# SebastianBitsch/SRGAN-ST

Measured on AMD Instinct MI355X. Metric: HR images/sec (96px x4, B=16/GPU) G+D+ST-loss step, higher is better.
Workload: dtype f32; 1 GPU; srgan_x4_hr96_b16_G+D+ST-loss step: adv+mse+st, D updated every step (train.py:116-164; BASELINE metric); global_batch=16, hr=96, lr=24, parallelism=dp1, hip_graph=True, d_update_interval=1, d_sr_forward=run: all three discriminator forwards of train.py:136,155,158

## Files before the change

### include/srganst.h

```cpp
#ifndef SRGANST_H
#define SRGANST_H
#include <stdint.h>
#ifdef __cplusplus
extern "C" {
#endif

const char* sst_last_error(void);
int sst_version(void);
const char* sst_arch(void);
int sst_clear_error(void);
int sst_reload_env(void);

int sst_st_loss_workspace(int B, int H, int W, int64_t* partial_floats);
int sst_st_loss_fwd(const float* sr, const float* gt, float* loss, float* gS, float* partials,
                    unsigned* counter, int B, int H, int W, float sigma, float rho, int normalize,
                    void* stream);
int sst_st_loss_bwd(const float* sr, const float* gS, float* dsr, const float* scale_dev,
                    float scale_host, int accumulate, int B, int H, int W, float sigma, float rho,
                    void* stream);
int sst_st_maps_workspace(int B, int H, int W, int64_t* tile_floats);
int sst_st_maps(const float* x, const float* gt, float* Sx, float* Sgt, float* Fx, float* Fgt, float* d, float* tile_sums,
                int B, int H, int W, float sigma, float rho, int normalize, void* stream);
int sst_st_pixel_loss_fwd(const float* sr, const float* gt, float* loss, float* gS, float* partials, unsigned* counter,
                          float* pix_loss, float* pix_partials, int pix_mode, int B, int H, int W, float sigma, float rho,
                          int normalize, void* stream);
int sst_st_pixel_loss_bwd(const float* sr, const float* gt, const float* gS, float* dsr, const float* scale_dev, float scale_host,
                          float pix_weight, int pix_mode, int accumulate, int B, int H, int W, float sigma, float rho,
                          void* stream);

int64_t sst_conv_packed_floats(int Cout, int Cin, int ksize);
int sst_conv_pack(const float* w, float* wp, int Cout, int Cin, int ksize, int mode, void* stream);
int sst_conv_pack_multi(const void* jobs, int njobs, int total_blocks, void* stream);
int sst_conv_mtiles(int B, int Ho, int Wo);
int sst_conv_stat_tiles(int B, int H, int W, int Cin, int Cout, int ksize, int stride);
const char* sst_conv_kernel_name(int B, int H, int W, int Cin, int Cout, int ksize, int stride, int out_mode, int fused_in);
const char* sst_conv_wgrad_kernel_name(int B, int H, int W, int Cin, int Cout, int ksize, int stride, int njobs);
long sst_debug_big_tile_launches(void);
long sst_debug_band_launches(void);
long sst_debug_wgrad_band_launches(void);
int sst_debug_mfma_peak(float* out, int blocks, int iters, void* stream);
int sst_debug_bf16x3(const float* A, const float* B, float* C32, float* C3, int K, int mode, int blocks, void* stream);
int sst_debug_stamp(unsigned long long* out, int slot, void* stream);
int sst_conv_fwd(const float* x, const float* wp, float* y, float* y_pre, const float* bias,
                 const float* in_scale, const float* in_shift, const float* in_slope,
                 float in_slope_const, int in_act, const float* residual, float* stats,
                 float* stats_cnt, int out_mode, int B, int H, int W, int Cin, int Cout, int ksize,
                 int stride, void* stream);
int sst_conv_pipe_supported(int B, int H, int W, int Cin, int Cout, int ksize, int stride);
int sst_conv_pipe_stat_tiles(int B, int H, int W, int Cin, int Cout, int ksize, int stride);
int64_t sst_conv_pipe_ws_floats(int B, int H, int W, int Cin, int Cout, int ksize, int stride);
int sst_conv_pipe_groups_ok(int B, int H, int W, int Cin, int Cout, int ksize, int stride, int grp_images);
int sst_conv_pipe_fwd_grp(const float* x, const float* wp, float* y, const float* bias, const float* in_scale,
                          const float* in_shift, const float* in_slope, float in_slope_const, int in_act, float* stats,
                          float* stats_cnt, const float* epi_y, const float* epi_scale, const float* epi_shift,
                          const float* epi_slope, float epi_slope_const, int epi_act, float* epi_partial, float* ws, int B,
                          int H, int W, int Cin, int Cout, int ksize, int stride, int grp_images, void* stream);
int sst_conv_ns_supported(int B, int H, int W, int Cin, int Cout, int ksize, int stride, int out_mode);
int sst_conv_ns_fwd(const float* x, const float* wp, float* y, const float* bias, const float* in_scale,
                    const float* in_shift, const float* in_slope, float in_slope_const, int in_act, float* stats,
                    float* stats_cnt, const float* epi_y, const float* epi_scale, const float* epi_shift,
                    const float* epi_slope, float epi_slope_const, int epi_act, float* epi_partial, int B, int H, int W,
                    int Cin, int Cout, int ksize, int stride, int out_mode, int grp_images, void* stream);
int sst_conv_s2_dgrad_pipe_supported(int B, int H, int W, int Cin, int Cout);
int64_t sst_conv_s2_dgrad_pipe_ws_floats(int B, int H, int W, int Cin, int Cout);
int sst_conv_s2_dgrad_pipe_stat_tiles(int B, int H, int W, int Cin, int Cout);
int sst_conv_s2_dgrad_pipe_groups_ok(int B, int H, int W, int Cin, int Cout, int grp_images);
int sst_conv_s2_dgrad_pipe_bwdstats_grp(const float* dy, const float* wp, float* dx, float* ws, const float* epi_y,
                                    const float* epi_scale, const float* epi_shift, const float* epi_slope,
                                    float epi_slope_const, int epi_act, float* epi_partial, int B, int H, int W, int Cin,
                                    int Cout, int grp_images, void* stream);
int sst_conv_dgrad_bwdstats(const float* x, const float* wp, float* y, const float* residual, const float* epi_y,
                            const float* epi_scale, const float* epi_shift, const float* epi_slope,
                            float epi_slope_const, int epi_act, float* epi_partial, int B, int H, int W, int Cin,
                            int Cout, int ksize, void* stream);
int sst_conv_acc_supported(int B, int H, int W, int Cin, int Cout, int ksize, int stride);
int sst_conv_fwd_acc(const float* x, const float* in2, float* side_out, const float* ones, const float* wp, float* y,
                     const float* bias, const float* in_slope, float in_slope_const, int in_act, const double* in_acc,
                     const float* in_gamma, const float* in_beta, float in_n, float eps, float momentum, float* o_mean,
                     float* o_rstd, float* o_scale, float* o_shift, float* run_mean, float* run_var, double* st_acc,
                     int nrep, int B, int H, int W, int Cin, int Cout, int ksize, void* stream);
int sst_conv_dgrad_fused_acc(const float* g, const float* y2, const float* in_scale, const float* in_shift,
                             const float* in_slope, float in_slope_const, int in_act, float* dy_out, const float* wp,
                             float* out, const float* residual, const float* epi_y, const float* epi_scale,
                             const float* epi_shift, const float* epi_slope, float epi_slope_const, int epi_act,
                             const double* bw_in_acc, const float* mean, const float* rstd, const float* gamma, float n,
                             float* dgamma, float* dbeta, float* dslope, double* bw_st_acc, int nrep, int B, int H,
                             int W, int Cin, int Cout, int ksize, void* stream);
int sst_bn_finalize_acc(const double* acc, int nrep, int C, float n, const float* gamma, const float* beta,
                        float* run_mean, float* run_var, float* mean, float* rstd, float* scale, float* shift,
                        float eps, float momentum, void* stream);
int sst_conv_fwd_resin(const float* x, const float* y2, const float* ones, const float* bn_scale, const float* bn_shift,
                       float* h_out, const float* wp, float* y, const float* bias, float* stats, float* stats_cnt,
                       int B, int H, int W, int Cin, int Cout, int ksize, void* stream);
int sst_conv_dgrad_fused(const float* g, const float* y2, const float* cA, const float* cB, const float* cC,
                         const float* in_scale, const float* in_shift, const float* in_slope, float in_slope_const,
                         int in_act, float* dy_out, const float* wp, float* out, const float* residual,
                         const float* epi_y, const float* epi_scale, const float* epi_shift, const float* epi_slope,
                         float epi_slope_const, int epi_act, float* epi_partial, int B, int H, int W, int Cin, int Cout,
                         int ksize, void* stream);
int sst_conv_wgrad_chunks2(int B, int H, int W, int Cin, int Cout, int ksize, int stride, int njobs);
int sst_conv_wgrad_groups_ok(int B, int H, int W, int Cin, int Cout, int ksize, int stride, int grp_images);
int sst_conv_wgrad_grp(const float* x, const float* dy, float* slab, float* dw, const float* in_scale,
                   const float* in_shift, const float* in_slope, float in_slope_const, int in_act,
                   int B, int H, int W, int Cin, int Cout, int stride, int ksize, int accumulate,
                       int grp_images, void* stream);
int sst_conv_wgrad_pending_reduce(int B, int H, int W, int Cin, int Cout, int ksize, int stride, int has_in_scale, int in_act);
int sst_wgrad_reduce_multi(const void* jobs, int njobs, void* stream);
int sst_wgrad_c3_supported(int C, int ksize);
int64_t sst_wgrad_c3_slab_floats(int B, int H, int W, int C);
int sst_wgrad_c3(const float* big, const float* small, float* slab, float* dw, const float* in_slope,
                 float in_slope_const, int in_act, int kind, int B, int H, int W, int C, int accumulate,
                 void* stream);

int64_t sst_conv9_c3_packed_floats(int Cout_eff);
int sst_conv9_c3_pack(const float* w, float* wp, int Cout, int Cin, int mode, void* stream);
int sst_conv9_c3_fwd(const float* x, const float* wp, float* y, const float* bias, int B, int H, int W,
                     int Cout, void* stream);
int64_t sst_conv9_to3_packed_floats(int C);
int sst_conv9_to3_pack(const float* w, float* wp, int C, void* stream);
int sst_conv9_to3_fwd(const float* x, const float* wp, float* y, float* y_pre, const float* bias,
                      const float* in_slope, float in_slope_const, int in_act, int B, int H, int W, int C,
                      void* stream);

int64_t sst_conv_s2_dgrad_packed_floats(int Cout, int Cin);
int sst_conv_s2_dgrad_pack(const float* w, float* wp, int Cout, int Cin, void* stream);
int sst_conv_s2_dgrad(const float* dy, const float* wp, float* dx, int B, int H, int W, int Cin, int Cout,
                      void* stream);
int sst_conv_s2_dgrad_tiles(int B, int H, int W);
const char* sst_conv_s2_dgrad_kernel_name(int B, int H, int W, int Cin, int Cout, int fused);
int sst_conv_s2_dgrad_fused(const float* g, const float* y2, const float* cA, const float* cB, const float* cC,
                            const float* in_scale, const float* in_shift, const float* in_slope, float in_slope_const,
                            int in_act, float* dy_out, const float* wp, float* dx, const float* epi_y,
                            const float* epi_scale, const float* epi_shift, const float* epi_slope, float epi_slope_const,
                            int epi_act, float* epi_partial, int B, int H, int W, int Cin, int Cout, void* stream);

int sst_conv_wgrad_grouped(const void* jobs, int njobs, int B, int H, int W, int Cin, int Cout, int stride,
                           int ksize, int accumulate, void* stream);

int sst_bn_finalize_grp(const float* stats, const float* cnt, int ntiles, int C, int groups, const float* gamma,
                        const float* beta, float* run_mean, float* run_var, float* mean, float* rstd, float* scale,
                        float* shift, float eps, float momentum, void* stream);
int sst_bn_eval_affine(const float* gamma, const float* beta, const float* run_mean,
                       const float* run_var, float* scale, float* shift, int C, float eps, void* stream);
int sst_bn_residual(const float* y, const float* scale, const float* shift, const float* res,
                    const float* res_slope, float* out, int64_t R, int C, void* stream);
int sst_bwd_reduce_blocks(int64_t R, int C);
int sst_bwd_finalize(const float* partial, int nblk, int C, float n, const float* mean,
                     const float* rstd, const float* gamma, float* dgamma, float* dbeta, float* cA,
                     float* cB, float* cC, float* dslope, int accumulate, void* stream);
int sst_bwd_reduce_grp(const float* g, const float* g2, const float* y, const float* scale, const float* shift,
                       const float* slope, float slope_const, int act, float* partial, int64_t R, int C, int groups,
                       void* stream);
int sst_bwd_finalize_grp(const float* partial, int nblk, int C, float n, int groups, const float* mean, const float* rstd,
                         const float* gamma, float* dgamma, float* dbeta, float* cA, float* cB, float* cC, int accumulate,
                         void* stream);
int sst_bwd_apply_grp(const float* g, const float* g2, const float* y, const float* scale, const float* shift,
                      const float* slope, float slope_const, int act, const float* cA, const float* cB, const float* cC,
                      float* dy, int64_t R, int C, int groups, void* stream);
int sst_bwd_finalize_wide(const float* partial, int nblk, int C, float n, const float* mean, const float* rstd,
                          const float* gamma, float* dgamma, float* dbeta, float* cA, float* cB, float* cC,
                          float* dslope, int accumulate, float* scratch, unsigned* counter, void* stream);
int sst_act_bwd_partial_blocks(int64_t stored_rows);
int sst_act_bwd_partial(const float* g, const float* g2, const float* y, const float* slope, float slope_const,
                        float* dy, float* partial, int64_t R, int C, int unshuffle_H, int unshuffle_W, void* stream);
int sst_bwd_apply(const float* g, const float* g2, const float* y, const float* scale,
                  const float* shift, const float* slope, float slope_const, int act, const float* cA,
                  const float* cB, const float* cC, float* dy, int64_t R, int C, int unshuffle_H,
                  int unshuffle_W, void* stream);
int sst_add(const float* a, const float* b, float* out, int64_t n, void* stream);

int sst_transpose(const float* src, float* dst, int B, int C, int H, int W, int to_nchw, void* stream);
int sst_feat_loss_fwd(const float* x, const float* gt, const float* scale, const float* shift, float slope, int C,
                      float* loss, float* partials, unsigned* counter, int64_t n, int mode, void* stream);
int sst_feat_loss_bwd(const float* x, const float* gt, const float* scale, const float* shift, float slope, int C,
                      float* dx, const float* scale_dev, float scale_host, int accumulate, int64_t n, int mode,
                      void* stream);
int sst_transpose_affine(const float* src, float* dst, int B, int C, int H, int W, int to_nchw,
                         const float* scale, const float* shift, void* stream);
int sst_maxpool_relu_fwd(const float* y, float* out, int B, int H, int W, int C, void* stream);
int sst_maxpool_relu_bwd(const float* g, const float* y, float* dy, int B, int H, int W, int C, void* stream);
int sst_clamp_bwd_blocks(int B, int H, int W);
int sst_clamp_bwd(const float* g, const float* pre, float* out, float* partial, float* dbias,
                  int accumulate, int B, int C, int H, int W, void* stream);
int sst_pixel_loss_blocks(int64_t n);
int sst_pixel_loss_fwd(const float* x, const float* gt, float* loss, float* partials, unsigned* counter,
                       int64_t n, int mode, void* stream);
int sst_pixel_loss_bwd(const float* x, const float* gt, float* dx, const float* scale_dev,
                       float scale_host, int accumulate, int64_t n, int mode, void* stream);
int sst_bce_logits(const float* logits, float target, float* loss, float* dlogits,
                   const float* scale_dev, float scale_host, int n, void* stream);
int sst_bicubic(const float* x, float* y, const float* wy, const int* iy, const float* wx, const int* ix,
                int64_t planes, int H, int W, int oh, int ow, int Ty, int Tx, int round_grid, void* stream);
int sst_gather_batch(const uint8_t* src, int64_t N, const int* idx, int B, int H, int W, const float* lut, float* gt, float* lr,
                     const float* wy, const int* iy, const float* wx, const int* ix, int oh, int ow, int Ty, int Tx,
                     void* stream);
int sst_gather_crops(const uint8_t* arena, int64_t arena_bytes, const int64_t* table, int64_t N, const int* desc, int B, int S,
                     const float* lut, float* gt, float* lr, const float* wy, const int* iy, const float* wx, const int* ix,
                     int oh, int ow, int Ty, int Tx, int span, void* stream);
int sst_image_metrics_workspace(int B, int H, int W, int64_t* partial_doubles);
int sst_image_metrics(const float* sr, const float* hr, int B, int H, int W, double* out, uint8_t* sr_u8, uint8_t* hr_u8,
                      double* workspace, void* stream);
int sst_tile_gather(const uint8_t* src_u8, const float* src_f32, int64_t src_bytes, int H, int W, const int* desc, int B, int th,
                    int tw, int t, const float* lut, float* out, void* stream);
int sst_tile_scatter(const float* tiles, const int* rows, int B, int H, int W, int th, int tw, int scale, int t, float* canvas,
                     int accumulate, void* stream);
int sst_canvas_to_u8(const float* canvas, int H, int W, float scale, uint8_t* out, void* stream);
int sst_bb_blocks(int B, int H, int W);
int sst_bb_feature_dim(int mode);
int sst_bb_patches(const float* img, float* cand, float* cnrm, int B, int H, int W, int ncand_total, int cand_off,
                   int mode, const float* st_mats, void* stream);
int sst_bb_match_dist(const float* sr, const float* cand, const float* cnrm, int* ind, float* dsr, float* partials, int B,
                 int H, int W, int ncand, float alpha, float beta, int criterion_l2, int mode, const float* st_mats, int dist_l1,
                      void* stream);
int sst_bbg_patches(int H, int W, int k, int pad, int stride);
int sst_bbg_blocks(int B, int np);
int sst_bbg_unfold(const float* img, float* table, float* nrm, int B, int H, int W, int k, int pad, int stride, int nrows_total,
                   int row_off, void* stream);
int sst_bbg_match(const float* srf, const float* cand, const float* cnrm, int* ind, float* gfeat, float* partials, int B, int np,
                  int ncand, int D, float alpha, float beta, int criterion_l2, int dist_l1, void* stream);
int sst_bbg_fold(const float* gfeat, float* dsr, int B, int H, int W, int k, int pad, int stride, void* stream);
int sst_weighted_sum(const float* const* terms, const float* weights, int n, float* out, float* weighted,
                     void* stream);

int sst_linear_ksplit(int M, int N, int K);
int sst_linear_fwd(const float* x, const float* w, const float* bias, float* y, float* slab, int M, int N,
                   int K, void* stream);
int sst_linear_dgrad(const float* dy, const float* w, float* dx, int M, int N, int K, int nhwc_C,
                     int nhwc_HW, void* stream);
int sst_linear_wgrad(const float* dy, const float* x, float* dw, float* db, int M, int N, int K,
                     int accumulate, void* stream);
int sst_head_fwd(const float* h, const float* w, const float* b, float* y, int M, int N, int K, float slope,
                 void* stream);
int sst_head_bwd(const float* h, const float* w, const float* dy, float* dh, float* dw, float* db, int M,
                 int N, int K, float slope, int accumulate, void* stream);
int sst_flatten_act_grp(const float* y, const float* scale, const float* shift, float slope, int act,
                        float* flat, int B, int HW, int C, int grp_images, void* stream);

int sst_adam_flat(float* p, const float* g, float* m, float* v, int64_t n, const float* lr, float* steps,
                  int nsteps, double beta1, double beta2, double eps, double weight_decay, void* stream);

int sst_adam_flat_ema(float* p, const float* g, float* m, float* v, float* ema, int64_t n, const float* lr, float* steps,
                      int nsteps, double beta1, double beta2, double eps, double weight_decay, double ema_decay,
                      int ema_warmup, void* stream);

int sst_ema_flat(float* ema, const float* p, int64_t n, const float* steps, double ema_decay, int ema_warmup, void* stream);

#ifdef __cplusplus
}
#endif
#endif
```

### srgan-st_amd/csrc/conv_pipe.hip

```cpp
#include "conv_common.h"
#include <cstdlib>
#include <type_traits>
#include "conv_epilogue.h"

int sst_conv_band_rows(int B, int H, int W, int Cin, int Cout, int ksize, int stride);

namespace {

constexpr int PIPE_RING = 9;

struct PipeArgs {
  const float* x;
  const float* wp;
  float* y;
  const float* bias;
  const float* in_scale; const float* in_shift; const float* in_slope; float in_slope_const; int in_act;
  float* stats; float* stats_cnt;
  const float* epi_y; const float* epi_scale; const float* epi_shift; const float* epi_slope;
  float epi_slope_const; int epi_act; float* epi_partial;
  float* ws;
  int B, H, W, Cin, Cout, Ho, Wo;
  int R;
  int tiles_x, n_mt, nfc, total_tiles, ncb, ksplit, cb_per, units;
#ifdef SST_PIPE_ABLATE
  int dbg;
#endif
  int gB, grows;
};

template <int S, int TW, int MODE>
struct PipeGeom {
  static constexpr int TH = 32 / TW;
  static constexpr int NB = TW == 2 ? 3 : 1;
  static constexpr int KSPAN = MODE ? 2 : 3;
  static constexpr int PW = (TW - 1) * S + KSPAN;
  static constexpr int PR = (TH - 1) * S + KSPAN + NB;
  static constexpr int NP = PW * PR;
  static constexpr int NU = (NP + 15) / 16;
  static constexpr int PS = 20;
  static constexpr int WAVE_FLOATS = NP * PS;
  static constexpr int NACC = MODE ? 4 : 1;
  static constexpr int NPAIR = MODE ? 2 : 1;
  static constexpr int SCRATCH = NPAIR * 4 * 32 * 33;
};
constexpr int S2D_CLS[9] = {0, 1, 1, 2, 2, 3, 3, 3, 3};
constexpr int S2D_TAP[9] = {0, 0, 1, 0, 1, 0, 1, 2, 3};

struct Stage {
  int b0, rem0, ix0, c0;
  int gin;
  const float* w;
};

#define PIPE_GLOAD(dst, voff, sbase) \
  asm volatile("s_nop 4\n\tglobal_load_dwordx4 %0, %1, %2" : "=v"(dst) : "v"(voff), "s"(sbase))
#define PIPE_WAIT(reg, n) asm volatile("s_waitcnt vmcnt(%1)" : "+v"(reg) : "n"(n))

__device__ __forceinline__ float half_sum(float t) {
  auto ror = [](float x, auto ctrl) {
    return __builtin_bit_cast(float, __builtin_amdgcn_update_dpp(0, __builtin_bit_cast(int, x), decltype(ctrl)::value, 0xf, 0xf, false));
  };
  t += ror(t, std::integral_constant<int, 0x128>{});
  t += ror(t, std::integral_constant<int, 0x124>{});
  t += ror(t, std::integral_constant<int, 0x122>{});
  t += ror(t, std::integral_constant<int, 0x121>{});
  t += __shfl_xor(t, 16, 64);
  return t;
}

template <int TW, int MODE = 0>
__device__ __forceinline__ void pipe_epilogue(const PipeArgs& a, float v[4], int r0, int ox0, int c0, int mt, int lane, bool first,
                                              int cls = 0) {
  constexpr int TH = 32 / TW;
  const int px = lane & 31;
  const int r = r0 + px / TW, ox = ox0 + px % TW;
  const bool pix_ok = r < a.R && ox < a.Wo;
  size_t obase;
  if (MODE) {
    obase = ((size_t)(2 * r + (cls >> 1)) * (2 * a.Wo) + 2 * ox + (cls & 1)) * a.Cout + c0;
    if (pix_ok) *reinterpret_cast<f32x4*>(a.y + obase) = f32x4{v[0], v[1], v[2], v[3]};
  }
  if (!MODE && a.bias) {
    const f32x4 bv = *reinterpret_cast<const f32x4*>(a.bias + c0);
#pragma unroll
    for (int j = 0; j < 4; ++j) v[j] += bv[j];
  }
  if (!MODE) {
    obase = ((size_t)r * a.Wo + ox) * a.Cout + c0;
    if (pix_ok) *reinterpret_cast<f32x4*>(a.y + obase) = f32x4{v[0], v[1], v[2], v[3]};
  }
  if (!MODE && a.stats) {
    const int nvalid = min(TH, a.R - r0) * min(TW, a.Wo - ox0);
    f32x4 s1, m2;
#pragma unroll
    for (int j = 0; j < 4; ++j) s1[j] = half_sum(pix_ok ? v[j] : 0.f);
#pragma unroll
    for (int j = 0; j < 4; ++j) {
      const float mean = s1[j] / (float)nvalid;
      const float d = pix_ok ? (v[j] - mean) : 0.f;
      m2[j] = half_sum(d * d);
    }
    if (px == 0) {
      float* st = a.stats + (size_t)mt * 2 * a.Cout;
      *reinterpret_cast<f32x4*>(st + c0) = s1;
      *reinterpret_cast<f32x4*>(st + a.Cout + c0) = m2;
      if (first) a.stats_cnt[mt] = (float)nvalid;
    }
  }
  if (a.epi_partial) {
    const float eslope = a.epi_slope ? a.epi_slope[0] : a.epi_slope_const;
    f32x4 yv = {0.f, 0.f, 0.f, 0.f}, es = {1.f, 1.f, 1.f, 1.f}, eh = {0.f, 0.f, 0.f, 0.f};
    if (pix_ok) yv = *reinterpret_cast<const f32x4*>(a.epi_y + obase);
    if (a.epi_scale) {
      const int ge = a.gB ? (r0 / a.grows) * a.Cout : 0;
      es = *reinterpret_cast<const f32x4*>(a.epi_scale + ge + c0);
      eh = *reinterpret_cast<const f32x4*>(a.epi_shift + ge + c0);
    }
    f32x4 q[3];
#pragma unroll
    for (int j = 0; j < 4; ++j) {
      const float g = pix_ok ? v[j] : 0.f;
      const float z = a.epi_scale ? fmaf(yv[j], es[j], eh[j]) : yv[j];
      float gz = g, q2 = 0.f;
      if (a.epi_act) {
        q2 = g * fminf(z, 0.f);
        gz = z > 0.f ? g : g * eslope;
      }
      q[0][j] = half_sum(gz);
      q[1][j] = half_sum(gz * yv[j]);
      q[2][j] = half_sum(q2);
    }
    if (px == 0) {
      const size_t prow = MODE ? (size_t)mt * 4 + cls : (size_t)mt;
#pragma unroll
      for (int k = 0; k < 3; ++k) *reinterpret_cast<f32x4*>(a.epi_partial + (prow * 3 + k) * a.Cout + c0) = q[k];
    }
  }
}

template <int S, int TW, int MODE, bool MS>
__global__ __launch_bounds__(CONV_NT, (S == 1 && MODE == 0 ? 3 : 2)) void conv_pipe_kernel(PipeArgs a) {
  using G = PipeGeom<S, TW, MODE>;
  constexpr int NACC = G::NACC, NPAIR = G::NPAIR;
  constexpr int PW = G::PW, NP = G::NP, NU = G::NU, NB = G::NB;
  constexpr int PS = G::PS;
  __shared__ __attribute__((aligned(16))) float patch[4 * G::WAVE_FLOATS];
  __shared__ __attribute__((aligned(16))) float scratch[G::SCRATCH];
  const int tid = threadIdx.x, wave = __builtin_amdgcn_readfirstlane(tid >> 6), lane = tid & 63;
  const int li = lane & 31, lh = lane >> 5;
  const int nwg = gridDim.x;
  const int HV = a.H + 1;
  const float slope = a.in_slope ? a.in_slope[0] : a.in_slope_const;
  const int c4 = wave * 16 + (lane & 3) * 4;
  const int p0 = lane >> 2;
  float* const lds = patch + wave * G::WAVE_FLOATS;

  int q = blockIdx.x;
  if (q >= a.units) return;
  int mt, nf, r0, ox0, oy0, cb, cb_end;
  Stage cur, nxt;
  auto decode = [&](int qq, int& mt_, int& nf_, int& ksi_, int& r0_, int& ox0_, int& b0_, int& oy0_) {
    mt_ = qq % a.n_mt;
    const int rest = qq / a.n_mt;
    nf_ = rest % a.nfc;
    ksi_ = rest / a.nfc;
    const int ty = mt_ / a.tiles_x, tx = mt_ - ty * a.tiles_x;
    r0_ = ty * G::TH;
    ox0_ = tx * TW;
    b0_ = r0_ / a.Ho;
    oy0_ = r0_ - b0_ * a.Ho;
  };
  auto make_stage = [&](int b0_, int oy0_, int ox0_, int nf_, int cb_) {
    Stage s;
    s.b0 = b0_;
    s.rem0 = oy0_ * S;
    s.ix0 = ox0_ * S - (MODE ? 0 : 1);
    s.c0 = cb_ * CB;
    s.gin = a.gB ? (b0_ / a.gB) * a.Cin : 0;
    s.w = a.wp + ((size_t)(nf_ * a.ncb + cb_) * 9 * 8) * 256 + wave * 512;
    return s;
  };
  int ksi, b0;
  decode(q, mt, nf, ksi, r0, ox0, b0, oy0);
  cb = ksi * a.cb_per;
  cb_end = cb + a.cb_per;
  cur = make_stage(b0, oy0, ox0, nf, cb);

  constexpr int NS = NU + 2;
  f32x4 sv[NU];
  unsigned okmask = 0;
  f32x4 ssc, ssh;
  const float* sc_base = a.in_scale ? a.in_scale : a.x;
  const float* sh_base = a.in_scale ? a.in_shift : a.x;
  unsigned boffs[MS ? NU : 1];
  auto stage_load = [&](const Stage& s, bool same_tile) {
#ifdef SST_PIPE_ABLATE
    if (a.dbg & 4) return;
#endif
    if (MS && same_tile) {
#pragma unroll
      for (int u = 0; u < NU; ++u) {
        boffs[u] += CB * 4u;
        PIPE_GLOAD(sv[u], boffs[u], a.x);
      }
    } else {
      okmask = 0;
#pragma unroll
      for (int u = 0; u < NU; ++u) {
        const int p = p0 + 16 * u;
        const int pr = p / PW, pc = p - pr * PW;
        int rr = s.rem0 + pr, b = s.b0;
#pragma unroll
        for (int k = 0; k <= NB; ++k) {
          const bool wrap = rr >= HV;
          rr -= wrap ? HV : 0;
          b += wrap ? 1 : 0;
        }
        const int iy = MODE ? rr : rr - 1, ix = s.ix0 + pc;
        const bool ok = p < NP && (MODE ? rr < a.H : rr >= 1) && b < a.B && (unsigned)ix < (unsigned)a.W;
        const int off = ((b * a.H + iy) * a.W + ix) * a.Cin + s.c0 + c4;
        const unsigned boff = (ok ? (unsigned)off : (unsigned)c4) * 4u;
        if (MS) boffs[u] = boff;
        PIPE_GLOAD(sv[u], boff, a.x);
        okmask |= ok ? (1u << u) : 0u;
      }
    }
    const unsigned coff = (unsigned)(a.in_scale ? s.gin + s.c0 + c4 : c4) * 4u;
    PIPE_GLOAD(ssc, coff, sc_base);
    PIPE_GLOAD(ssh, coff, sh_base);
  };
  auto stage_store = [&]() {
#ifdef SST_PIPE_ABLATE
    if (a.dbg & 1) return;
#endif
#pragma unroll
    for (int u = 0; u < NU; ++u) {
      const int p = p0 + 16 * u;
      if (p >= NP) continue;
      f32x4 t = sv[u];
      if (a.in_scale) {
#pragma unroll
        for (int j = 0; j < 4; ++j) t[j] = fmaf(t[j], ssc[j], ssh[j]);
      }
      if (a.in_act == ACT_SLOPE) {
#pragma unroll
        for (int j = 0; j < 4; ++j) t[j] = t[j] > 0.f ? t[j] : t[j] * slope;
      }
      if (!((okmask >> u) & 1u)) t = f32x4{0.f, 0.f, 0.f, 0.f};
      *reinterpret_cast<f32x4*>(&lds[p * PS + (lane & 3) * 4]) = t;
    }
  };

  auto lane_base = [&](int oy0_) {
    const int tr = li / TW, tc = li - tr * TW;
    int cross = 0;
#pragma unroll
    for (int k = 1; k <= NB; ++k) cross += (oy0_ + tr >= k * a.Ho) ? 1 : 0;
    return ((S * tr + cross) * PW + tc * S) * PS + 4 * lh;
  };
  int a_base = lane_base(oy0);

  f32x4 ring[PIPE_RING];
  const unsigned wlane = lane * 16u;
#define PIPE_WCHUNK(dst, w, i) PIPE_GLOAD(dst, wlane, (w) + (((i) >> 1) * 8 + ((i) & 1)) * 256)

#pragma unroll
  for (int i = 0; i < PIPE_RING; ++i) PIPE_WCHUNK(ring[i], cur.w, i);
  stage_load(cur, false);
  asm volatile("s_waitcnt vmcnt(0)" ::: "memory");
  __builtin_amdgcn_sched_barrier(0);
  stage_store();

  f32x16 acc[NACC];
#pragma unroll
  for (int k = 0; k < NACC; ++k)
#pragma unroll
    for (int r = 0; r < 16; ++r) acc[k][r] = 0.f;

  for (;;) {
    const bool unit_end = cb + 1 == cb_end;
    int n_q = q, n_mt = mt, n_nf = nf, n_r0 = r0, n_ox0 = ox0, n_oy0 = oy0, n_cb = cb + 1, n_cb_end = cb_end;
    bool more = true;
    if (unit_end) {
      n_q = q + nwg;
      more = n_q < a.units;
      if (more) {
        int n_ksi, n_b0;
        decode(n_q, n_mt, n_nf, n_ksi, n_r0, n_ox0, n_b0, n_oy0);
        n_cb = n_ksi * a.cb_per;
        n_cb_end = n_cb + a.cb_per;
        nxt = make_stage(n_b0, n_oy0, n_ox0, n_nf, n_cb);
      } else {
        nxt = cur;
      }
    } else {
      nxt = cur;
      nxt.c0 += CB;
      nxt.w += (size_t)9 * 8 * 256;
    }

    {
      const float* ab = lds + a_base;
      f32x4 av = *reinterpret_cast<const f32x4*>(ab);
      __builtin_amdgcn_sched_barrier(0);
#pragma unroll
      for (int i = 0; i < 18; ++i) {
        f32x4 an = av;
        if (i + 1 < 18) {
          const int t = (i + 1) >> 1;
          const int ntx = MODE ? 1 + (S2D_CLS[t] & 1) : 3, tt = MODE ? S2D_TAP[t] : t;
          an = *reinterpret_cast<const f32x4*>(ab + ((tt / ntx) * PW + (tt % ntx)) * PS + ((i + 1) & 1) * 8);
        }
        if (i == 0 || i >= 10) PIPE_WAIT(ring[i % PIPE_RING], 8); else PIPE_WAIT(ring[i % PIPE_RING], 8 + NS);
        const f32x4 bv = ring[i % PIPE_RING];
        constexpr int dummy_ = 0;
        (void)dummy_;
        const int ai = MODE ? S2D_CLS[i >> 1] : 0;
#ifdef SST_PIPE_ABLATE
        if (!(a.dbg & 16))
#endif
#pragma unroll
        for (int j = 0; j < 4; ++j) acc[ai] = __builtin_amdgcn_mfma_f32_32x32x2f32(av[j], bv[j], acc[ai], 0, 0, 0);
#ifdef SST_PIPE_ABLATE
        if (a.dbg & 8) { PIPE_GLOAD(ring[i % PIPE_RING], wlane, a.wp); } else
#endif
        if (i + PIPE_RING < 18) PIPE_WCHUNK(ring[i % PIPE_RING], cur.w, i + PIPE_RING);
        else PIPE_WCHUNK(ring[i % PIPE_RING], nxt.w, i + PIPE_RING - 18);
        if (i == 0) stage_load(nxt, !unit_end);
        av = an;
        __builtin_amdgcn_sched_barrier(0);
      }
    }
#ifdef SST_PIPE_ABLATE
    if (unit_end && (a.dbg & 2)) {
      if (acc[0][0] == 12345.f) a.y[0] = acc[0][0];
      if (!more) return;
      a_base = lane_base(n_oy0);
    } else
#endif
    if (unit_end) {
      const int cl = 8 * wave + 4 * lh;
#pragma unroll
      for (int k0 = 0; k0 < NACC; k0 += NPAIR) {
        __syncthreads();
#pragma unroll
        for (int k = 0; k < NPAIR; ++k)
#pragma unroll
          for (int r = 0; r < 16; ++r) {
            const int row = (r & 3) + 8 * (r >> 2) + 4 * lh;
            scratch[((k * 4 + wave) * 32 + row) * 33 + li] = acc[k0 + k][r];
            acc[k0 + k][r] = 0.f;
          }
        __syncthreads();
#pragma unroll
        for (int k = 0; k < NPAIR; ++k) {
          float v[4];
#pragma unroll
          for (int j = 0; j < 4; ++j) {
            float t = scratch[((k * 4 + 0) * 32 + li) * 33 + cl + j];
            t += scratch[((k * 4 + 1) * 32 + li) * 33 + cl + j];
            t += scratch[((k * 4 + 2) * 32 + li) * 33 + cl + j];
            t += scratch[((k * 4 + 3) * 32 + li) * 33 + cl + j];
            v[j] = t;
          }
          if (a.ksplit > 1) {
            const int tile = nf * a.n_mt + mt;
            const int part = cb / a.cb_per;
            *reinterpret_cast<f32x4*>(a.ws + (((size_t)part * a.total_tiles + tile) * NACC + k0 + k) * 1024 + li * 32 + cl) =
                f32x4{v[0], v[1], v[2], v[3]};
          } else {
            pipe_epilogue<TW, MODE>(a, v, r0, ox0, nf * 32 + cl, mt, lane, nf == 0 && wave == 0, k0 + k);
          }
        }
      }
      if (!more) return;
      a_base = lane_base(n_oy0);
    }
    stage_store();
    q = n_q; mt = n_mt; nf = n_nf; r0 = n_r0; ox0 = n_ox0; oy0 = n_oy0; cb = n_cb; cb_end = n_cb_end;
    cur = nxt;
  }
}

template <int TW, int MODE>
__global__ __launch_bounds__(CONV_NT) void pipe_reduce_kernel(PipeArgs a) {
  constexpr int NACC = MODE ? 4 : 1;
  const int tid = threadIdx.x, wave = tid >> 6, lane = tid & 63;
  const int tile = blockIdx.x / NACC, cls = blockIdx.x - tile * NACC;
  const int nf = tile / a.n_mt, mt = tile - nf * a.n_mt;
  const int ty = mt / a.tiles_x, tx = mt - ty * a.tiles_x;
  const int li = lane & 31, cl = 8 * wave + 4 * (lane >> 5);
  const size_t slab = (size_t)a.total_tiles * NACC * 1024;
  const float* src = a.ws + ((size_t)tile * NACC + cls) * 1024 + li * 32 + cl;
  f32x4 s = *reinterpret_cast<const f32x4*>(src);
  for (int k = 1; k < a.ksplit; ++k) {
    const f32x4 t = *reinterpret_cast<const f32x4*>(src + k * slab);
#pragma unroll
    for (int j = 0; j < 4; ++j) s[j] += t[j];
  }
  float v[4] = {s[0], s[1], s[2], s[3]};
  pipe_epilogue<TW, MODE>(a, v, ty * (32 / TW), tx * TW, nf * 32 + cl, mt, lane, nf == 0 && wave == 0, cls);
}

struct PipePlan {
  int tw;
  int ksplit, n_mt, tiles_x, nfc, ncb;
};

PipePlan pipe_plan(int B, int H, int W, int Cin, int Cout, int ksize, int stride) {
  PipePlan pl{};
  if (ksize != 3 || (stride != 1 && stride != 2) || (Cin % 64) || (Cout % 32) || B <= 0) return pl;
  if (stride == 2 && ((H | W) & 1)) return pl;
  if (Cout <= 64 && sst_conv_band_rows(B, H, W, Cin, Cout, ksize, stride)) return pl;
  const int Ho = (H - 1) / stride + 1, Wo = (W - 1) / stride + 1;
  int tw = 0;
  if (Wo % 8 == 0 && Ho >= 3) tw = 8;
  else if (Wo % 4 == 0 && Ho >= 7) tw = 4;
  else if (Wo % 2 == 0 && Ho >= 5) tw = 2;
  if (!tw) return pl;
  const int th = 32 / tw;
  pl.tiles_x = Wo / tw;
  pl.n_mt = pl.tiles_x * ((B * Ho + th - 1) / th);
  pl.nfc = Cout / 32;
  pl.ncb = Cin / 64;
  const long tiles = (long)pl.n_mt * pl.nfc;
  int maxks = 1;
  while (maxks < 4 && pl.ncb % (maxks * 2) == 0) maxks *= 2;
  if (tiles * maxks < 256) return pl;
  int ks = 1;
  while (tiles * ks < 1024 && ks < maxks) ks *= 2;
  pl.ksplit = ks;
  pl.tw = tw;
  return pl;
}

constexpr int PIPE_CUS = 256;

}

SST_API int sst_conv_pipe_supported(int B, int H, int W, int Cin, int Cout, int ksize, int stride) {
  return pipe_plan(B, H, W, Cin, Cout, ksize, stride).tw;
}
SST_API int sst_conv_pipe_stat_tiles(int B, int H, int W, int Cin, int Cout, int ksize, int stride) {
  return pipe_plan(B, H, W, Cin, Cout, ksize, stride).n_mt;
}
SST_API int64_t sst_conv_pipe_ws_floats(int B, int H, int W, int Cin, int Cout, int ksize, int stride) {
  const PipePlan pl = pipe_plan(B, H, W, Cin, Cout, ksize, stride);
  return (pl.tw && pl.ksplit > 1) ? (int64_t)pl.ksplit * pl.n_mt * pl.nfc * 1024 : 0;
}

SST_API int sst_conv_pipe_groups_ok(int B, int H, int W, int Cin, int Cout, int ksize, int stride, int grp_images) {
  const PipePlan pl = pipe_plan(B, H, W, Cin, Cout, ksize, stride);
  if (!pl.tw || grp_images <= 0 || B % grp_images) return 0;
  const int Ho = (H - 1) / stride + 1;
  return (grp_images * Ho) % (32 / pl.tw) == 0;
}

SST_API int sst_conv_pipe_fwd_grp(const float* x, const float* wp, float* y, const float* bias, const float* in_scale,
                                  const float* in_shift, const float* in_slope, float in_slope_const, int in_act, float* stats,
                                  float* stats_cnt, const float* epi_y, const float* epi_scale, const float* epi_shift,
                                  const float* epi_slope, float epi_slope_const, int epi_act, float* epi_partial, float* ws, int B,
                                  int H, int W, int Cin, int Cout, int ksize, int stride, int grp_images, void* stream) {
  SST_REQUIRE(x && wp && y, "sst_conv_pipe_fwd: null pointer");
  const PipePlan pl = pipe_plan(B, H, W, Cin, Cout, ksize, stride);
  SST_REQUIRE(grp_images == 0 || grp_images == B || sst_conv_pipe_groups_ok(B, H, W, Cin, Cout, ksize, stride, grp_images),
              "sst_conv_pipe_fwd: coefficient groups of %d images do not end on tile boundaries (B=%d H=%d W=%d stride=%d)", grp_images, B,
              H, W, stride);
  SST_REQUIRE(pl.tw, "sst_conv_pipe_fwd: shape B=%d H=%d W=%d Cin=%d Cout=%d k=%d stride=%d is not taken by the pipelined kernel", B,
              H, W, Cin, Cout, ksize, stride);
  SST_REQUIRE((in_scale == nullptr) == (in_shift == nullptr), "sst_conv_pipe_fwd: in_scale/in_shift must come together");
  SST_REQUIRE(!stats || stats_cnt, "sst_conv_pipe_fwd: stats needs stats_cnt");
  SST_REQUIRE(!epi_partial || (epi_y && !stats && ((epi_scale == nullptr) == (epi_shift == nullptr))),
              "sst_conv_pipe_fwd: backward partials need epi_y and exclude forward stats");
  SST_REQUIRE(pl.ksplit == 1 || ws, "sst_conv_pipe_fwd: this shape splits K over workgroups and needs the workspace");
  SST_REQUIRE((int64_t)B * H * W * Cin < (1ll << 29), "sst_conv_pipe_fwd: input too large for 32-bit byte offsets");
  PipeArgs a;
  a.x = x; a.wp = wp; a.y = y; a.bias = bias; a.in_scale = in_scale; a.in_shift = in_shift; a.in_slope = in_slope;
  a.in_slope_const = in_slope_const; a.in_act = in_act; a.stats = stats; a.stats_cnt = stats_cnt;
  a.epi_y = epi_y; a.epi_scale = epi_scale; a.epi_shift = epi_shift; a.epi_slope = epi_slope; a.epi_slope_const = epi_slope_const;
  a.epi_act = epi_act; a.epi_partial = epi_partial; a.ws = ws;
  a.B = B; a.H = H; a.W = W; a.Cin = Cin; a.Cout = Cout;
  a.Ho = (H - 1) / stride + 1; a.Wo = (W - 1) / stride + 1; a.R = B * a.Ho;
  a.tiles_x = pl.tiles_x; a.n_mt = pl.n_mt; a.nfc = pl.nfc; a.total_tiles = pl.n_mt * pl.nfc; a.ncb = pl.ncb;
  a.ksplit = pl.ksplit; a.cb_per = pl.ncb / pl.ksplit; a.units = a.total_tiles * pl.ksplit;
  a.gB = (grp_images > 0 && grp_images < B) ? grp_images : 0;
  a.grows = a.gB * a.Ho;
#ifdef SST_PIPE_ABLATE
  a.dbg = sst_env("SST_PIPE_DBG") ? atoi(sst_env("SST_PIPE_DBG")) : 0;
#endif
  int wg_per_cu = stride == 1 ? 3 : 2;
  if (const char* e = sst_env("SST_PIPE_GPC")) {
    const int v = atoi(e);
    if (v >= 1 && v < wg_per_cu) wg_per_cu = v;
  }
  const int grid = a.units < wg_per_cu * PIPE_CUS ? a.units : wg_per_cu * PIPE_CUS;
  hipStream_t st = sst_stream(stream);
#define SST_PIPE_LAUNCH(S_, TW_)                                                                  \
  do {                                                                                            \
    if (a.cb_per > 1) conv_pipe_kernel<S_, TW_, 0, true><<<grid, CONV_NT, 0, st>>>(a);            \
    else conv_pipe_kernel<S_, TW_, 0, false><<<grid, CONV_NT, 0, st>>>(a);                        \
    SST_LAUNCH_CHECK("conv_pipe_kernel");                                                         \
    if (pl.ksplit > 1) {                                                                          \
      pipe_reduce_kernel<TW_, 0><<<a.total_tiles, CONV_NT, 0, st>>>(a);                           \
      SST_LAUNCH_CHECK("pipe_reduce_kernel");                                                     \
    }                                                                                             \
  } while (0)
  if (stride == 1) {
    if (pl.tw == 8) SST_PIPE_LAUNCH(1, 8); else if (pl.tw == 4) SST_PIPE_LAUNCH(1, 4); else SST_PIPE_LAUNCH(1, 2);
  } else {
    if (pl.tw == 8) SST_PIPE_LAUNCH(2, 8); else if (pl.tw == 4) SST_PIPE_LAUNCH(2, 4); else SST_PIPE_LAUNCH(2, 2);
  }
#undef SST_PIPE_LAUNCH
  return SST_OK;
}

int64_t sst_conv_s2_dgrad_pipe_section(int Cout, int Cin);

namespace {
PipePlan pipe_plan_s2d(int B, int H, int W, int Cin, int Cout) {
  PipePlan pl{};
  if (B <= 0 || H <= 0 || W <= 0 || ((H | W) & 1) || (Cout % 64) || (Cin % 32)) return pl;
  const int Hd = H / 2, Wd = W / 2;
  int tw = 0;
  if (Wd % 8 == 0 && Hd >= 3) tw = 8;
  else if (Wd % 4 == 0 && Hd >= 7) tw = 4;
  else if (Wd % 2 == 0 && Hd >= 5) tw = 2;
  if (!tw) return pl;
  const int th = 32 / tw;
  pl.tiles_x = Wd / tw;
  pl.n_mt = pl.tiles_x * ((B * Hd + th - 1) / th);
  pl.nfc = Cin / 32;
  pl.ncb = Cout / 64;
  const long tiles = (long)pl.n_mt * pl.nfc;
  int maxks = 1;
  while (maxks < 4 && pl.ncb % (maxks * 2) == 0) maxks *= 2;
  if (tiles * maxks < 256) return pl;
  int ks = 1;
  while (tiles * ks < 1024 && ks < maxks) ks *= 2;
  if (tw == 4 && ks > 1) return pl;
  pl.ksplit = ks;
  pl.tw = tw;
  return pl;
}
}

SST_API int sst_conv_s2_dgrad_pipe_supported(int B, int H, int W, int Cin, int Cout) { return pipe_plan_s2d(B, H, W, Cin, Cout).tw; }
SST_API int64_t sst_conv_s2_dgrad_pipe_ws_floats(int B, int H, int W, int Cin, int Cout) {
  const PipePlan pl = pipe_plan_s2d(B, H, W, Cin, Cout);
  return (pl.tw && pl.ksplit > 1) ? (int64_t)pl.ksplit * pl.n_mt * pl.nfc * 4 * 1024 : 0;
}
SST_API int sst_conv_s2_dgrad_pipe_stat_tiles(int B, int H, int W, int Cin, int Cout) { return pipe_plan_s2d(B, H, W, Cin, Cout).n_mt * 4; }
SST_API int sst_conv_s2_dgrad_pipe_groups_ok(int B, int H, int W, int Cin, int Cout, int grp_images) {
  const PipePlan pl = pipe_plan_s2d(B, H, W, Cin, Cout);
  if (!pl.tw || grp_images <= 0 || B % grp_images) return 0;
  return (grp_images * (H / 2)) % (32 / pl.tw) == 0;
}
SST_API int sst_conv_s2_dgrad_pipe_bwdstats_grp(const float* dy, const float* wp, float* dx, float* ws, const float* epi_y,
                                                const float* epi_scale, const float* epi_shift, const float* epi_slope,
                                                float epi_slope_const, int epi_act, float* epi_partial, int B, int H, int W, int Cin,
                                                int Cout, int grp_images, void* stream) {
  SST_REQUIRE(dy && wp && dx, "sst_conv_s2_dgrad_pipe: null pointer");
  SST_REQUIRE(grp_images == 0 || grp_images == B || !epi_partial || sst_conv_s2_dgrad_pipe_groups_ok(B, H, W, Cin, Cout, grp_images),
              "sst_conv_s2_dgrad_pipe: coefficient groups of %d images do not end on tile boundaries", grp_images);
  SST_REQUIRE(!epi_partial || (epi_y && ((epi_scale == nullptr) == (epi_shift == nullptr))), "sst_conv_s2_dgrad_pipe: backward partials need epi_y");
  const PipePlan pl = pipe_plan_s2d(B, H, W, Cin, Cout);
  SST_REQUIRE(pl.tw, "sst_conv_s2_dgrad_pipe: shape B=%d H=%d W=%d Cin=%d Cout=%d is not taken by the pipelined kernel", B, H, W, Cin, Cout);
  SST_REQUIRE(pl.ksplit == 1 || ws, "sst_conv_s2_dgrad_pipe: this shape splits K over workgroups and needs the workspace");
  SST_REQUIRE((int64_t)B * (H / 2) * (W / 2) * Cout < (1ll << 29), "sst_conv_s2_dgrad_pipe: input too large for 32-bit byte offsets");
  PipeArgs a{};
  a.x = dy; a.wp = wp + sst_conv_s2_dgrad_pipe_section(Cout, Cin); a.y = dx; a.ws = ws;
  a.in_act = ACT_NONE;
  a.epi_y = epi_y; a.epi_scale = epi_scale; a.epi_shift = epi_shift; a.epi_slope = epi_slope; a.epi_slope_const = epi_slope_const;
  a.epi_act = epi_act; a.epi_partial = epi_partial;
  a.B = B; a.H = H / 2; a.W = W / 2; a.Cin = Cout; a.Cout = Cin;
  a.Ho = a.H; a.Wo = a.W; a.R = B * a.Ho;
  a.tiles_x = pl.tiles_x; a.n_mt = pl.n_mt; a.nfc = pl.nfc; a.total_tiles = pl.n_mt * pl.nfc; a.ncb = pl.ncb;
  a.ksplit = pl.ksplit; a.cb_per = pl.ncb / pl.ksplit; a.units = a.total_tiles * pl.ksplit;
#ifdef SST_PIPE_ABLATE
  a.dbg = 0;
#endif
  a.gB = (grp_images > 0 && grp_images < B && epi_partial) ? grp_images : 0;
  a.grows = a.gB * a.Ho;
  const int grid = a.units < 2 * PIPE_CUS ? a.units : 2 * PIPE_CUS;
  hipStream_t st = sst_stream(stream);
#define SST_S2D_LAUNCH(TW_)                                                                       \
  do {                                                                                            \
    if (a.cb_per > 1) conv_pipe_kernel<1, TW_, 1, true><<<grid, CONV_NT, 0, st>>>(a);             \
    else conv_pipe_kernel<1, TW_, 1, false><<<grid, CONV_NT, 0, st>>>(a);                         \
    SST_LAUNCH_CHECK("conv_pipe_kernel (stride-2 data-gradient)");                                \
    if (pl.ksplit > 1) {                                                                          \
      pipe_reduce_kernel<TW_, 1><<<a.total_tiles * 4, CONV_NT, 0, st>>>(a);                       \
      SST_LAUNCH_CHECK("pipe_reduce_kernel (stride-2 data-gradient)");                            \
    }                                                                                             \
  } while (0)
  if (pl.tw == 8) SST_S2D_LAUNCH(8); else if (pl.tw == 4) SST_S2D_LAUNCH(4); else SST_S2D_LAUNCH(2);
#undef SST_S2D_LAUNCH
  return SST_OK;
}
```

### srgan-st_amd/csrc/conv_wgrad.hip

```cpp
#include "conv_common.h"
#include <cstring>
#include <cstdlib>

namespace {

constexpr int SUB = 64;
constexpr int WLD = 64 + 4;

struct WgJob {
  const float* x; const float* dy; float* slab; float* dw;
  const float* in_scale; const float* in_shift; const float* in_slope;
  float in_slope_const; int in_act;
};

constexpr int WG_TAB_MAX = 40;
struct WgJobTab { WgJob j[WG_TAB_MAX]; };

struct WgradArgs {
  int grouped;
  int nchunk;
  const float* x;
  const float* dy;
  float* slab;
  const float* in_scale;
// ... 78 lines not shown
            dv = *reinterpret_cast<const f32x4*>(src);
          } else {
#pragma unroll
            for (int j = 0; j < 4; ++j)
              if (co + j < a.Cout) dv[j] = src[j];
          }
        }
      }
      rx[u] = xv;
      rd[u] = dv;
      int ox = sox[u] + adv_x, oy = soy[u] + adv_y;
      if (ox >= a.Wo) { ox -= a.Wo; ++oy; }
      if (oy >= a.Ho) { oy -= a.Ho; ++sb[u]; if (oy >= a.Ho) { sb[u] += oy / a.Ho; oy %= a.Ho; } }
      sox[u] = ox;
      soy[u] = oy;
    }
  };
  f32x4 sc4 = {1.f, 1.f, 1.f, 1.f}, sh4 = {0.f, 0.f, 0.f, 0.f};
  {
    const int c = ci0 + (tid & 15) * 4;
    if (a.in_scale) {
#pragma unroll
      for (int j = 0; j < 4; ++j)
        if (c + j < a.Cin) {
          sc4[j] = a.in_scale[c + j];
          sh4[j] = a.in_shift[c + j];
        }
    }
  }
  auto stage_store = [&]() {
#pragma unroll
    for (int u = 0; u < 4; ++u) {
      const int q = tid + u * CONV_NT;
      const int p = q >> 4, c4 = (q & 15) * 4;
      f32x4 xv = rx[u];
      if ((rvalid >> u) & 1u) {
        const int c = ci0 + c4;
        if (a.in_scale) {
#pragma unroll
          for (int j = 0; j < 4; ++j) xv[j] = fmaf(xv[j], sc4[j], sh4[j]);
        }
        if (a.in_act == ACT_SLOPE) {
#pragma unroll
          for (int j = 0; j < 4; ++j) xv[j] = xv[j] > 0.f ? xv[j] : xv[j] * slope;
        }
        if (!VEC) {
#pragma unroll
          for (int j = 0; j < 4; ++j)
            if (c + j >= a.Cin) xv[j] = 0.f;
        }
      } else {
        xv = f32x4{0.f, 0.f, 0.f, 0.f};
      }
      *reinterpret_cast<f32x4*>(&sX[p * WLD + c4]) = xv;
      *reinterpret_cast<f32x4*>(&sD[p * WLD + c4]) = rd[u];
    }
  };
  if (m_begin < m_end) stage_load(m_begin);
  for (int64_t m0 = m_begin; m0 < m_end; m0 += SUB) {
    __syncthreads();
    stage_store();
    __syncthreads();
    if (m0 + SUB < m_end) stage_load(m0 + SUB);
    if (!(a.dbg & 2)) {
      float av = sD[lh * WLD + wco + li], bv = sX[lh * WLD + wci + li];
#pragma unroll
      for (int kk = 0; kk < SUB / 2; ++kk) {
        const int kn = (kk + 1 < SUB / 2) ? kk + 1 : kk;
        const float an = sD[(2 * kn + lh) * WLD + wco + li];
        const float bn = sX[(2 * kn + lh) * WLD + wci + li];
        acc = __builtin_amdgcn_mfma_f32_32x32x2f32(av, bv, acc, 0, 0, 0);
        av = an;
        bv = bn;
      }
    }
  }
  if (a.dbg & 4) {
    if (acc[0] == 12345.f) a.slab[0] = 1.f;
    return;
  }
  float* out = a.slab + ((size_t)chunk * gridDim.y + tap) * a.Cout * a.Cin;
  const int ci = ci0 + wci + li;
#pragma unroll
  for (int r = 0; r < 16; ++r) {
    const int co = co0 + wco + (r & 3) + 8 * (r >> 2) + 4 * lh;
    if (co < a.Cout && ci < a.Cin) out[(size_t)co * a.Cin + ci] = acc[r];
  }
}

constexpr int WB_XS = 10, WB_DS = 3;

template <int XS>
__global__ __launch_bounds__(CONV_NT, (XS > 7 ? 1 : 2)) void conv_wgrad_band_kernel(WgradArgs a, WgJobTab tab) {
  extern __shared__ __attribute__((aligned(16))) float wlds[];
  int chunk = blockIdx.x;
  if (a.grouped) {
    const int job = blockIdx.x / a.nchunk;
    chunk = blockIdx.x - job * a.nchunk;
    const WgJob jb = tab.j[job];
    a.x = jb.x; a.dy = jb.dy; a.slab = jb.slab; a.in_scale = jb.in_scale; a.in_shift = jb.in_shift;
    a.in_slope = jb.in_slope; a.in_slope_const = jb.in_slope_const; a.in_act = jb.in_act;
  }
  const int tid = threadIdx.x, wave = __builtin_amdgcn_readfirstlane(tid >> 6), lane = tid & 63;
  const int li = lane & 31, lh = lane >> 5;
  const int R = a.R, W = a.W, PW = W + 2, H = a.H;
  const int npx_x = (R + 2) * PW, npx_d = R * W;
  float* sX = wlds;
  float* sD = wlds + npx_x * WLD;
  const int nci = a.Cin >> 6;
  const int cob = blockIdx.y / nci, cib = blockIdx.y - cob * nci;
  const int co0 = cob * 64, ci0 = cib * 64;
  const int wco = (wave & 1) * 32, wci = (wave >> 1) * 32;
  const float slope = a.in_slope ? a.in_slope[0] : a.in_slope_const;
  const int bands_per_img = H / R;
  const int band_begin = chunk * a.bpc, band_end = min(a.nbands, band_begin + a.bpc);

  const int c4 = (tid & 15) * 4;
  f32x4 sc4 = {1.f, 1.f, 1.f, 1.f}, sh4 = {0.f, 0.f, 0.f, 0.f};
  if (a.in_scale) {
    sc4 = *reinterpret_cast<const f32x4*>(a.in_scale + ci0 + c4);
    sh4 = *reinterpret_cast<const f32x4*>(a.in_shift + ci0 + c4);
  }
  int xoff[XS];
  unsigned m_col = 0, m_top = 0, m_bot = 0;
#pragma unroll
  for (int u = 0; u < XS; ++u) {
    const int p = (tid + u * CONV_NT) >> 4;
    const int py = p / PW, px = p - py * PW;
    if (p < npx_x && px >= 1 && px <= W) m_col |= 1u << u;
    if (py == 0) m_top |= 1u << u;
    if (py == R + 1) m_bot |= 1u << u;
    xoff[u] = ((py - 1) * W + (px - 1)) * a.Cin;
  }
  f32x4 rx[XS], rd[WB_DS];
  unsigned rvalid = 0;
  auto stage_load = [&](int band) {
    const int b = band / bands_per_img, y0 = (band - b * bands_per_img) * R;
    const float* xb = a.x + ((size_t)(b * H + y0) * W) * a.Cin + ci0 + c4;
    const float* db = a.dy + ((size_t)(b * H + y0) * W) * a.Cout + co0 + c4;
    rvalid = m_col & ~(y0 == 0 ? m_top : 0u) & ~(y0 + R == H ? m_bot : 0u);
#pragma unroll
    for (int u = 0; u < XS; ++u) {
      const bool ok = (rvalid >> u) & 1u;
      const f32x4 v = *reinterpret_cast<const f32x4*>(xb + (ok ? xoff[u] : 0));
      rx[u] = v;
    }
#pragma unroll
    for (int u = 0; u < WB_DS; ++u) {
      const int p = (tid + u * CONV_NT) >> 4;
      rd[u] = *reinterpret_cast<const f32x4*>(db + (size_t)(p < npx_d ? p : 0) * a.Cout);
    }
  };
  auto stage_store = [&]() {
#pragma unroll
    for (int u = 0; u < XS; ++u) {
      const int p = (tid + u * CONV_NT) >> 4;
      if (p >= npx_x) break;
      f32x4 xv = rx[u];
      if (a.in_scale) {
#pragma unroll
        for (int j = 0; j < 4; ++j) xv[j] = fmaf(xv[j], sc4[j], sh4[j]);
      }
      if (a.in_act == ACT_SLOPE) {
#pragma unroll
        for (int j = 0; j < 4; ++j) xv[j] = xv[j] > 0.f ? xv[j] : xv[j] * slope;
      }
      if (!((rvalid >> u) & 1u)) xv = f32x4{0.f, 0.f, 0.f, 0.f};
      *reinterpret_cast<f32x4*>(&sX[p * WLD + c4]) = xv;
    }
#pragma unroll
    for (int u = 0; u < WB_DS; ++u) {
      const int p = (tid + u * CONV_NT) >> 4;
      if (p < npx_d) *reinterpret_cast<f32x4*>(&sD[p * WLD + c4]) = rd[u];
    }
  };

  f32x16 acc[9];
#pragma unroll
  for (int t = 0; t < 9; ++t)
#pragma unroll
    for (int r = 0; r < 16; ++r) acc[t][r] = 0.f;

  const int la = lh * WLD + wco + li, lb = lh * WLD + wci + li;
  int tofs[9];
#pragma unroll
  for (int t = 0; t < 9; ++t) tofs[t] = ((t / 3) * PW + (t % 3)) * WLD;
  const int halfw = W >> 1, npairs = R * halfw;

  if (band_begin < band_end) stage_load(band_begin);
  for (int band = band_begin; band < band_end; ++band) {
    __syncthreads();
    stage_store();
    __syncthreads();
    if (band + 1 < band_end && !(a.dbg & 1)) stage_load(band + 1);
    if (a.dbg & 2) continue;
    int pa = 0, pb = 0, x2 = 0;
    auto advance = [&]() {
      pa += 2 * WLD;
      pb += 2 * WLD;
      if (++x2 == halfw) { x2 = 0; pb += 2 * WLD; }
    };
    float av0 = sD[pa + la], av1;
    float bv0[9], bv1[9];
#pragma unroll
    for (int t = 0; t < 9; ++t) bv0[t] = sX[pb + tofs[t] + lb];
    for (int i = 0; i < npairs; i += 2) {
      advance();
      av1 = sD[pa + la];
#pragma unroll
      for (int t = 0; t < 9; ++t) bv1[t] = sX[pb + tofs[t] + lb];
#pragma unroll
      for (int t = 0; t < 9; ++t) acc[t] = __builtin_amdgcn_mfma_f32_32x32x2f32(av0, bv0[t], acc[t], 0, 0, 0);
      if (i + 2 < npairs) advance();
      av0 = sD[pa + la];
#pragma unroll
      for (int t = 0; t < 9; ++t) bv0[t] = sX[pb + tofs[t] + lb];
#pragma unroll
      for (int t = 0; t < 9; ++t) acc[t] = __builtin_amdgcn_mfma_f32_32x32x2f32(av1, bv1[t], acc[t], 0, 0, 0);
    }
  }

  if (a.dbg & 4) {
    if (acc[0][0] == 12345.f) a.slab[0] = 1.f;
    return;
  }
  const int ci = ci0 + wci + li;
#pragma unroll
  for (int t = 0; t < 9; ++t) {
    float* out = a.slab + ((size_t)chunk * 9 + t) * a.Cout * a.Cin;
#pragma unroll
    for (int r = 0; r < 16; ++r) {
      const int co = co0 + wco + (r & 3) + 8 * (r >> 2) + 4 * lh;
      out[(size_t)co * a.Cin + ci] = acc[t][r];
    }
  }
}

constexpr int C3_ROWS = 8;
__global__ __launch_bounds__(CONV_NT) void wgrad_k3c3_kernel(const float* __restrict__ x, const float* __restrict__ dy,
                                                             float* __restrict__ slab, int B, int H, int W, int Cout) {
  extern __shared__ __attribute__((aligned(16))) float xs[];
  __shared__ float red[3][64][28];
  const int bands = (H + C3_ROWS - 1) / C3_ROWS;
  const int b = blockIdx.x / bands, y0 = (blockIdx.x - b * bands) * C3_ROWS;
  const int rows = min(C3_ROWS, H - y0);
  const int RS = (W + 2) * 3 + 3;
  for (int i = threadIdx.x; i < (C3_ROWS + 2) * RS; i += CONV_NT) {
    const int r = i / RS, o = i - r * RS;
    const int px = o / 3 - 1, y = y0 - 1 + r;
    float v = 0.f;
    if (o < (W + 2) * 3 && (unsigned)px < (unsigned)W && (unsigned)y < (unsigned)H)
      v = x[(((size_t)b * H + y) * W + px) * 3 + (o - (px + 1) * 3)];
    xs[i] = v;
  }
  __syncthreads();
  const int co = threadIdx.x & 63, pl = threadIdx.x >> 6;
  for (int cob = blockIdx.y * 64; cob < Cout; cob += gridDim.y * 64) {
    float acc[27];
#pragma unroll
    for (int k = 0; k < 27; ++k) acc[k] = 0.f;
    if (cob + co < Cout) {
      constexpr int UNR = 8;
      const int npx = rows * W;
      const float* dyb = dy + ((size_t)b * H + y0) * W * Cout + cob + co;
      for (int p0 = pl; p0 < npx; p0 += UNR * (CONV_NT / 64)) {
        float g[UNR];
#pragma unroll
        for (int u = 0; u < UNR; ++u) {
          const int p = p0 + u * (CONV_NT / 64);
          g[u] = p < npx ? dyb[(size_t)p * Cout] : 0.f;
        }
#pragma unroll
        for (int u = 0; u < UNR; ++u) {
          const int p = min(p0 + u * (CONV_NT / 64), npx - 1);
          const int r = p / W, c = p - r * W;
          const float* w0 = xs + r * RS + c * 3;
#pragma unroll
          for (int ky = 0; ky < 3; ++ky)
#pragma unroll
            for (int q = 0; q < 9; ++q) acc[ky * 9 + q] = fmaf(g[u], w0[ky * RS + q], acc[ky * 9 + q]);
        }
      }
    }
    __syncthreads();
    if (pl > 0) {
#pragma unroll
      for (int k = 0; k < 27; ++k) red[pl - 1][co][k] = acc[k];
    }
    __syncthreads();
    if (pl == 0 && cob + co < Cout) {
      float* out = slab + (size_t)blockIdx.x * 9 * Cout * 3;
#pragma unroll
      for (int k = 0; k < 27; ++k) {
        const float t = ((acc[k] + red[0][co][k]) + red[1][co][k]) + red[2][co][k];
        const int ky = k / 9, kx = (k % 9) / 3, ci = k % 3;
        out[((size_t)(ky * 3 + kx) * Cout + cob + co) * 3 + ci] = t;
      }
    }
  }
}
constexpr int C3M_ROW = 104;
constexpr int C3M_WAVE = 3 * C3M_ROW + 96;
constexpr int C3M_TPW = 4;
__global__ __launch_bounds__(CONV_NT) void wgrad_k3c3_mfma_kernel(const float* __restrict__ x, const float* __restrict__ dy,
                                                                  float* __restrict__ slab, int B, int H, int W, int ntiles) {
  __shared__ float patch[4 * C3M_WAVE];
  __shared__ float scr[4 * 32 * 33];
  const int tid = threadIdx.x, wave = __builtin_amdgcn_readfirstlane(tid >> 6), lane = tid & 63;
  const int li = lane & 31, lh = lane >> 5;
  constexpr int Cout = 64;
  float* const ps = patch + wave * C3M_WAVE;
  const int tpr = W >> 5;
  const int ky = li / 9, kr = li - ky * 9;
  const float* const bl = ps + (li < 27 ? ky * C3M_ROW + kr + 3 * lh : 3 * C3M_ROW);
  f32x16 acc[2];
#pragma unroll
  for (int h = 0; h < 2; ++h)
#pragma unroll
    for (int r = 0; r < 16; ++r) acc[h][r] = 0.f;
  for (int i = lane; i < 96; i += 64) ps[3 * C3M_ROW + i] = 0.f;
  float av[2][16][2], xv[2][5];
  auto issue = [&](int it, float (&a_)[16][2], float (&x_)[5]) {
    const int t = (blockIdx.x * C3M_TPW + it) * 4 + wave;
    const bool live = it < C3M_TPW && t < ntiles;
    const int b = t / (H * tpr), rem = t - b * (H * tpr);
    const int y = rem / tpr, x0 = (rem - y * tpr) << 5;
    const float* dp = dy + (live ? (((size_t)b * H + y) * W + x0 + lh) * Cout + li : 0);
#pragma unroll
    for (int ks = 0; ks < 16; ++ks) {
      a_[ks][0] = live ? dp[(size_t)(2 * ks) * Cout] : 0.f;
      a_[ks][1] = live ? dp[(size_t)(2 * ks) * Cout + 32] : 0.f;
    }
#pragma unroll
    for (int u = 0; u < 5; ++u) {
      const int i = lane + 64 * u;
      const int r = i / 102, c = i - r * 102;
      const int iy = y - 1 + r, fx = (x0 - 1) * 3 + c;
      const bool ok = live && i < 306 && (unsigned)iy < (unsigned)H && (unsigned)fx < (unsigned)(W * 3);
      x_[u] = ok ? x[((size_t)b * H + iy) * W * 3 + fx] : 0.f;
    }
  };
  issue(0, av[0], xv[0]);
#pragma unroll
  for (int it = 0; it < C3M_TPW; ++it) {
#pragma unroll
    for (int u = 0; u < 5; ++u) {
      const int i = lane + 64 * u;
      if (i < 306) ps[(i / 102) * C3M_ROW + i % 102] = xv[it & 1][u];
    }
    if (it + 1 < C3M_TPW) issue(it + 1, av[(it + 1) & 1], xv[(it + 1) & 1]);
#pragma unroll
    for (int ks = 0; ks < 16; ++ks) {
      const float bv = bl[6 * ks];
      acc[0] = __builtin_amdgcn_mfma_f32_32x32x2f32(av[it & 1][ks][0], bv, acc[0], 0, 0, 0);
      acc[1] = __builtin_amdgcn_mfma_f32_32x32x2f32(av[it & 1][ks][1], bv, acc[1], 0, 0, 0);
    }
  }
  float* const out = slab + (size_t)blockIdx.x * 9 * Cout * 3;
#pragma unroll
  for (int h = 0; h < 2; ++h) {
    __syncthreads();
#pragma unroll
    for (int r = 0; r < 16; ++r) scr[(wave * 32 + (r & 3) + 8 * (r >> 2) + 4 * lh) * 33 + li] = acc[h][r];
    __syncthreads();
#pragma unroll
    for (int j = 0; j < 4; ++j) {
      const int row = 8 * wave + 4 * lh + j;
      const float v = ((scr[row * 33 + li] + scr[(32 + row) * 33 + li]) + scr[(64 + row) * 33 + li]) + scr[(96 + row) * 33 + li];
      if (li < 27) out[((size_t)(li / 3) * Cout + 32 * h + row) * 3 + li % 3] = v;
    }
  }
}
constexpr int C3R_OUT = 16, C3R_GRP = 1024 / C3R_OUT;
__global__ __launch_bounds__(1024) void c3m_reduce_kernel(const float* __restrict__ slab, float* __restrict__ dw, int nchunk,
                                                          int accumulate) {
  __shared__ float part[C3R_GRP][C3R_OUT + 1];
  constexpr int TOTAL = 9 * 64 * 3;
  const int o = threadIdx.x & (C3R_OUT - 1), gq = threadIdx.x / C3R_OUT;
  const int i = blockIdx.x * C3R_OUT + o;
  float t = 0.f;
  int c = gq;
  for (; c + 7 * C3R_GRP < nchunk; c += 8 * C3R_GRP) {
    float v[8];
#pragma unroll
    for (int u = 0; u < 8; ++u) v[u] = slab[(size_t)(c + C3R_GRP * u) * TOTAL + i];
#pragma unroll
    for (int u = 0; u < 8; ++u) t += v[u];
  }
  {
    float v[8];
#pragma unroll
    for (int u = 0; u < 8; ++u) v[u] = c + C3R_GRP * u < nchunk ? slab[(size_t)(c + C3R_GRP * u) * TOTAL + i] : 0.f;
#pragma unroll
    for (int u = 0; u < 8; ++u) t += v[u];
  }
  part[gq][o] = t;
  __syncthreads();
  if (threadIdx.x < 64) {
    const int oo = threadIdx.x & (C3R_OUT - 1), q = threadIdx.x / C3R_OUT;
    t = 0.f;
#pragma unroll
    for (int k = 0; k < C3R_GRP / 4; ++k) t += part[q * (C3R_GRP / 4) + k][oo];
    t += __shfl_xor(t, 16, 64);
    t += __shfl_xor(t, 32, 64);
    if (q == 0) {
      const int ii = blockIdx.x * C3R_OUT + oo;
      const int tap = ii / 192, oc = ii - tap * 192;
      float* d = dw + (size_t)oc * 9 + tap;
      *d = accumulate ? *d + t : t;
    }
  }
}
inline bool k3c3_mfma_applies(int W, int Cout) { return (W & 31) == 0 && Cout == 64 && !sst_env("SST_WGRAD_NO_K3C3_MFMA"); }
inline int k3c3_mfma_chunks(int B, int H, int W) { return (B * H * (W >> 5) + 4 * C3M_TPW - 1) / (4 * C3M_TPW); }

inline bool k3c3_applies(int Cin, int ksize, int stride, bool has_in_scale, int in_act) {
  return Cin == 3 && ksize == 3 && stride == 1 && !has_in_scale && in_act == ACT_NONE;
}

struct WgBandPlan { int R, bpc, nchunk, nbands; size_t lds; };
inline WgBandPlan wgrad_band_plan(int B, int H, int W, int Cin, int Cout, int ksize, int stride, int njobs) {
  WgBandPlan best{0, 0, 0, 0, 0};
  if (ksize != 3 || stride != 1 || (Cin & 63) || (Cout & 63) || (W & 3) || W < 4) return best;
  if (const char* e = sst_env("SST_WGRAD_BAND")) {
    if (atoi(e) == 0) return best;
  }
  if (2.0 * B * H * W * Cin * Cout * 9 * njobs < 2.5e9 && !sst_env("SST_WGRAD_BAND")) return best;
  const int nblk = (Cout >> 6) * (Cin >> 6);
  long slots = 512;
  int rmax = 2;
  if (const char* e = sst_env("SST_WGRAD_BAND_SLOTS")) slots = atoi(e);
  if (const char* e = sst_env("SST_WGRAD_BAND_R")) rmax = atoi(e);
  double best_cost = 1e30;
  for (int R = rmax; R >= 1; --R) {
    if (H % R) continue;
    const int npx_x = (R + 2) * (W + 2), npx_d = R * W;
    if ((npx_x * 16 + CONV_NT - 1) / CONV_NT > WB_XS || (npx_d * 16 + CONV_NT - 1) / CONV_NT > WB_DS) continue;
    const size_t lds = (size_t)(npx_x + npx_d) * WLD * sizeof(float);
    if (lds > 78 * 1024) continue;
    const long nbands = (long)B * (H / R);
    const long per = (long)nblk * njobs;
    long bpc = (nbands * per + slots - 1) / slots;
    if (bpc < 1) bpc = 1;
    const long nchunk = (nbands + bpc - 1) / bpc;
    const long rounds = (nchunk * per + slots - 1) / slots;
    const double cost = (double)rounds * ((double)bpc * R + 1.4);
    if (cost < best_cost) {
      best_cost = cost;
      best = WgBandPlan{R, (int)bpc, (int)nchunk, (int)nbands, lds};
    }
  }
  return best;
}

__global__ __launch_bounds__(256) void wgrad_reduce_kernel(const float* __restrict__ slab, float* __restrict__ dw, int nchunk,
                                                           int KK, int Cout, int Cin, int accumulate, int grouped, WgJobTab tab) {
  if (grouped) {
    slab = tab.j[blockIdx.y].slab;
    dw = tab.j[blockIdx.y].dw;
  }
  const int64_t per_tap = (int64_t)Cout * Cin, total = per_tap * KK;
  const bool split = accumulate & 2;
  accumulate &= 1;
  if (split) {
    __shared__ f32x4 part[4][64];
    const int item = threadIdx.x & 63, cg = threadIdx.x >> 6;
    const int64_t i4 = blockIdx.x * 64ll + item, total4 = total >> 2;
    f32x4 t = {0.f, 0.f, 0.f, 0.f};
    if (i4 < total4) {
#pragma unroll 4
      for (int s = cg; s < nchunk; s += 4) t += *reinterpret_cast<const f32x4*>(slab + (size_t)s * total + (i4 << 2));
    }
    part[cg][item] = t;
    __syncthreads();
    if (cg == 0 && i4 < total4) {
      t = part[0][item] + part[1][item];
      t += part[2][item];
      t += part[3][item];
      const int64_t i = i4 << 2;
      const int tap = (int)(i / per_tap);
      const int64_t oc = i - (int64_t)tap * per_tap;
#pragma unroll
      for (int j = 0; j < 4; ++j) {
        float* d = dw + (oc + j) * KK + tap;
        *d = accumulate ? *d + t[j] : t[j];
      }
    }
    return;
  }
  if ((Cin & 3) == 0) {
    const int64_t total4 = total >> 2;
    for (int64_t i4 = blockIdx.x * 256ll + threadIdx.x; i4 < total4; i4 += (int64_t)gridDim.x * 256) {
      const int64_t i = i4 << 2;
      const int tap = (int)(i / per_tap);
      const int64_t oc = i - (int64_t)tap * per_tap;
      f32x4 t = {0.f, 0.f, 0.f, 0.f};
#pragma unroll 4
      for (int s = 0; s < nchunk; ++s) t += *reinterpret_cast<const f32x4*>(slab + (size_t)s * total + i);
#pragma unroll
      for (int j = 0; j < 4; ++j) {
        float* d = dw + (oc + j) * KK + tap;
        *d = accumulate ? *d + t[j] : t[j];
      }
    }
  } else {
    for (int64_t i = blockIdx.x * 256ll + threadIdx.x; i < total; i += (int64_t)gridDim.x * 256) {
      const int tap = (int)(i / per_tap);
      const int64_t oc = i - (int64_t)tap * per_tap;
      float t = 0.f;
#pragma unroll 8
      for (int s = 0; s < nchunk; ++s) t += slab[(size_t)s * total + i];
      float* d = dw + oc * KK + tap;
      *d = accumulate ? *d + t : t;
    }
  }
}

}

static int sst_conv_wgrad_chunks(int B, int Ho, int Wo, int Cin, int Cout, int ksize) {
  const int64_t M = (int64_t)B * Ho * Wo;
  const int nblk = ((Cout + 63) / 64) * ((Cin + 63) / 64);
  int64_t want = (1024 + ksize * ksize * nblk - 1) / (ksize * ksize * nblk);
  int64_t maxc = (M + 159) / 160;
  if (want > maxc) want = maxc;
  if (want < 1) want = 1;
  int64_t chunk_px = ((M + want - 1) / want + SUB - 1) / SUB * SUB;
  return (int)((M + chunk_px - 1) / chunk_px);
}

static void launch_wgrad_reduce(const float* slab, float* dw, int nchunk, int KK, int Cout, int Cin, int accumulate,
                                const WgJobTab* tab, int njobs, hipStream_t st) {
  static const WgJobTab no_tab{};
  const WgJobTab& t = tab ? *tab : no_tab;
  const int grouped = tab != nullptr;
  const int64_t total = (int64_t)KK * Cout * Cin;
  if ((Cin & 3) == 0 && nchunk >= 8) {
    const int blocks = (int)((total / 4 + 63) / 64);
    wgrad_reduce_kernel<<<dim3(blocks, njobs), 256, 0, st>>>(slab, dw, nchunk, KK, Cout, Cin, (accumulate & 1) | 2, grouped, t);
    return;
  }
  const int64_t items = (Cin & 3) == 0 ? total / 4 : total;
  const int rb = (int)((items + 255) / 256 < 1024 ? (items + 255) / 256 : 1024);
  wgrad_reduce_kernel<<<dim3(rb, njobs), 256, 0, st>>>(slab, dw, nchunk, KK, Cout, Cin, accumulate, grouped, t);
}

namespace {
struct WrJob { const float* slab; float* dw; int nchunk, KK, Cout, Cin, accumulate, blocks; };
constexpr int WR_TAB_MAX = 24;
struct WrJobTab { WrJob j[WR_TAB_MAX]; };
__global__ __launch_bounds__(256) void wgrad_reduce_multi_kernel(WrJobTab tab) {
  const WrJob jb = tab.j[blockIdx.y];
  if ((int)blockIdx.x >= jb.blocks) return;
  const float* __restrict__ slab = jb.slab;
  float* __restrict__ dw = jb.dw;
  const int nchunk = jb.nchunk, KK = jb.KK, accumulate = jb.accumulate & 1;
  const int64_t per_tap = (int64_t)jb.Cout * jb.Cin, total = per_tap * KK;
  if ((jb.Cin & 3) == 0 && nchunk >= 8) {
    __shared__ f32x4 part[4][64];
    const int item = threadIdx.x & 63, cg = threadIdx.x >> 6;
    const int64_t i4 = blockIdx.x * 64ll + item, total4 = total >> 2;
    f32x4 t = {0.f, 0.f, 0.f, 0.f};
    if (i4 < total4) {
#pragma unroll 4
      for (int s = cg; s < nchunk; s += 4) t += *reinterpret_cast<const f32x4*>(slab + (size_t)s * total + (i4 << 2));
    }
    part[cg][item] = t;
    __syncthreads();
    if (cg == 0 && i4 < total4) {
      t = ((part[0][item] + part[1][item]) + part[2][item]) + part[3][item];
      const int64_t i = i4 << 2;
      const int tap = (int)(i / per_tap);
      const int64_t oc = i - (int64_t)tap * per_tap;
#pragma unroll
      for (int j = 0; j < 4; ++j) {
        float* d = dw + (oc + j) * KK + tap;
        *d = accumulate ? *d + t[j] : t[j];
      }
    }
    return;
  }
  if ((jb.Cin & 3) == 0) {
    const int64_t total4 = total >> 2;
    for (int64_t i4 = blockIdx.x * 256ll + threadIdx.x; i4 < total4; i4 += (int64_t)jb.blocks * 256) {
      const int64_t i = i4 << 2;
      const int tap = (int)(i / per_tap);
      const int64_t oc = i - (int64_t)tap * per_tap;
      f32x4 t = {0.f, 0.f, 0.f, 0.f};
#pragma unroll 4
      for (int s = 0; s < nchunk; ++s) t += *reinterpret_cast<const f32x4*>(slab + (size_t)s * total + i);
#pragma unroll
      for (int j = 0; j < 4; ++j) {
        float* d = dw + (oc + j) * KK + tap;
        *d = accumulate ? *d + t[j] : t[j];
      }
    }
  } else {
    for (int64_t i = blockIdx.x * 256ll + threadIdx.x; i < total; i += (int64_t)jb.blocks * 256) {
      const int tap = (int)(i / per_tap);
      const int64_t oc = i - (int64_t)tap * per_tap;
      float t = 0.f;
#pragma unroll 8
      for (int s = 0; s < nchunk; ++s) t += slab[(size_t)s * total + i];
      float* d = dw + oc * KK + tap;
      *d = accumulate ? *d + t : t;
    }
  }
}
}

struct WgS2Args {
  const float* x; const float* dy; float* slab;
  const float* in_scale; const float* in_shift; const float* in_slope; float in_slope_const; int in_act;
  int B, H, W, Cin, Cout, Ho, Wo;
  int tiles_x, tiles_img, ntiles, tpc;
  int dbg;
  float* dw; int accumulate;
  int gB;
};

template <int S, int TH, int TW, int S2_NW>
struct WgS2Geom {
  static constexpr int NPIX = TH * TW, PH = S * (TH - 1) + 3, PW = S * (TW - 1) + 3, NPX = PH * PW;
  static constexpr int XQ = (NPX * 8 + 63) / 64;
  static constexpr int DQ = (NPIX * 8 + 63) / 64;
  static constexpr int WAVE_FLOATS = (XQ * 8 + DQ * 8) * 32;
  static constexpr size_t LDS_BYTES = (size_t)S2_NW * WAVE_FLOATS * sizeof(float);
  static_assert(NPIX % 2 == 0 && TW % 2 == 0, "pixel pairs of one tile row");
  static_assert((size_t)2 * S2_NW * 32 * 33 * sizeof(float) <= LDS_BYTES, "exchange scratch (double-buffered) fits the staging area");
};

template <int S, int TH, int TW, int S2_NW>
__global__ __launch_bounds__(S2_NW * 64, 1) void conv_wgrad_tile_kernel(WgS2Args a) {
  using G = WgS2Geom<S, TH, TW, S2_NW>;
  constexpr int NPIX = G::NPIX, PW = G::PW, NPX = G::NPX, XQ = G::XQ, DQ = G::DQ;
  extern __shared__ __attribute__((aligned(16))) float wlds[];
  const int tid = threadIdx.x, wave = __builtin_amdgcn_readfirstlane(tid >> 6), lane = tid & 63;
  const int li = lane & 31, lh = lane >> 5;
  float* const xs = wlds + wave * G::WAVE_FLOATS;
  float* const ds = xs + XQ * 8 * 32;
  const int nci = a.Cin >> 5;
  const int co0 = (blockIdx.y / nci) * 32, ci0 = (blockIdx.y % nci) * 32;
  const int t0 = blockIdx.x * a.tpc, t1 = min(a.ntiles, t0 + a.tpc);
  const float slope = a.in_slope ? a.in_slope[0] : a.in_slope_const;
  const int q4 = (lane & 7) * 4;

  f32x16 acc[9];
#pragma unroll
  for (int t = 0; t < 9; ++t)
#pragma unroll
    for (int r = 0; r < 16; ++r) acc[t][r] = 0.f;

  f32x4 xr[XQ], dr[DQ];
  unsigned okm = 0;
  bool edge = false;
  int goff = 0;
  const bool lmax = a.in_act == ACT_SLOPE && slope >= 0.f && slope <= 1.f;
  auto issue = [&](int t, auto edge_) {
    constexpr bool EDGE = decltype(edge_)::value;
    const int b = t / a.tiles_img, rem = t - b * a.tiles_img;
    const int ty = rem / a.tiles_x, tx = rem - ty * a.tiles_x;
    const int oy0 = ty * TH, ox0 = tx * TW;
    const int xo = ((b * a.H + S * oy0 - 1) * a.W + S * ox0 - 1) * a.Cin + ci0 + q4;
    const bool last_y = oy0 + TH == a.Ho, last_x = ox0 + TW == a.Wo;
    const float* db = a.dy + ((size_t)(b * a.Ho + oy0) * a.Wo + ox0) * a.Cout + co0 + q4;
    okm = 0;
#pragma unroll
    for (int u = 0; u < XQ; ++u) {
      const int p = (lane >> 3) + 8 * u;
      const int pr = p / PW, pc = p - pr * PW;
      bool ok = 8 * u + 7 < NPX || p < NPX;
      if (EDGE) ok = ok && (pr > 0 || oy0 > 0) && (pc > 0 || ox0 > 0);
      if (EDGE && S == 1) ok = ok && (pr < G::PH - 1 || !last_y) && (pc < PW - 1 || !last_x);
      const int off = xo + (pr * a.W + pc) * a.Cin;
      xr[u] = *reinterpret_cast<const f32x4*>(a.x + ((EDGE || 8 * u + 7 >= NPX) ? (ok ? off : ci0 + q4) : off));
      if (EDGE) okm |= ok ? (1u << u) : 0u;
    }
#pragma unroll
    for (int u = 0; u < DQ; ++u) {
      const int p = (lane >> 3) + 8 * u;
      const int py = p / TW, px = p - py * TW;
      dr[u] = *reinterpret_cast<const f32x4*>(db + ((8 * u + 7 < NPIX || p < NPIX) ? (py * a.Wo + px) * a.Cout : 0));
    }
  };
  auto is_edge = [&](int t) {
    const int rem = t % a.tiles_img, tx = rem % a.tiles_x;
    bool e = rem < a.tiles_x || tx == 0;
    if (S == 1) e = e || rem >= a.tiles_img - a.tiles_x || tx == a.tiles_x - 1;
    return e;
  };
  auto issue_any = [&](int t) {
    goff = a.gB ? (t / a.tiles_img / a.gB) * a.Cin : 0;
    edge = is_edge(t);
    if (edge) issue(t, std::true_type{}); else issue(t, std::false_type{});
  };
  auto store = [&](auto edge_) {
    constexpr bool EDGE = decltype(edge_)::value;
    f32x4 sc = {1.f, 1.f, 1.f, 1.f}, sh = {0.f, 0.f, 0.f, 0.f};
    if (a.in_scale) {
      sc = *reinterpret_cast<const f32x4*>(a.in_scale + goff + ci0 + q4);
      sh = *reinterpret_cast<const f32x4*>(a.in_shift + goff + ci0 + q4);
    }
#pragma unroll
    for (int u = 0; u < XQ; ++u) {
      const int p = (lane >> 3) + 8 * u;
      f32x4 v = xr[u];
      if (a.in_scale) {
#pragma unroll
        for (int j = 0; j < 4; ++j) v[j] = fmaf(v[j], sc[j], sh[j]);
      }
      if (lmax) {
#pragma unroll
        for (int j = 0; j < 4; ++j) v[j] = fmaxf(v[j], v[j] * slope);
      } else if (a.in_act == ACT_SLOPE) {
#pragma unroll
        for (int j = 0; j < 4; ++j) v[j] = v[j] > 0.f ? v[j] : v[j] * slope;
      }
      if (EDGE && !((okm >> u) & 1u)) v = f32x4{0.f, 0.f, 0.f, 0.f};
      *reinterpret_cast<f32x4*>(xs + p * 32 + q4) = v;
    }
#pragma unroll
    for (int u = 0; u < DQ; ++u) *reinterpret_cast<f32x4*>(ds + ((lane >> 3) + 8 * u) * 32 + q4) = dr[u];
  };

  int t = t0 + wave;
  if (t < t1 && !(a.dbg & 2)) issue_any(t);
  const float* const dl = ds + lh * 32 + li;
  const float* const xl = xs + S * lh * 32 + li;
  for (; t < t1; t += S2_NW) {
    if (!(a.dbg & 1)) {
      if (edge) store(std::true_type{}); else store(std::false_type{});
    }
    if (t + S2_NW < t1 && !(a.dbg & 2)) issue_any(t + S2_NW);
    if (a.dbg & 4) continue;
    float av, bv[9];
    auto fetch = [&](int ks, float& a_, float (&b_)[9]) {
      const int py = (2 * ks) / TW, px = (2 * ks) % TW;
      a_ = dl[2 * ks * 32];
#pragma unroll
      for (int tap = 0; tap < 9; ++tap) b_[tap] = xl[((S * py + tap / 3) * PW + S * px + tap % 3) * 32];
    };
    fetch(0, av, bv);
    __builtin_amdgcn_sched_barrier(0);
#pragma unroll
    for (int ks = 0; ks < NPIX / 2; ++ks) {
      float an = 0.f, bn[9] = {0.f, 0.f, 0.f, 0.f, 0.f, 0.f, 0.f, 0.f, 0.f};
      if (ks + 1 < NPIX / 2) fetch(ks + 1, an, bn);
      __builtin_amdgcn_sched_barrier(0);
#pragma unroll
      for (int tap = 0; tap < 9; ++tap) acc[tap] = __builtin_amdgcn_mfma_f32_32x32x2f32(av, bv[tap], acc[tap], 0, 0, 0);
      __builtin_amdgcn_sched_barrier(0);
      av = an;
#pragma unroll
      for (int tap = 0; tap < 9; ++tap) bv[tap] = bn[tap];
    }
  }

  if (a.dbg & 8) {
    if (acc[0][0] == 12345.f) a.slab[0] = 1.f;
    return;
  }
  float* const scr = wlds;
  float* const out = a.slab + (size_t)blockIdx.x * 9 * a.Cout * a.Cin;
  __syncthreads();
#pragma unroll
  for (int tap = 0; tap < 9; ++tap) {
    float* const sb = scr + (tap & 1) * (S2_NW * 32 * 33);
#pragma unroll
    for (int r = 0; r < 16; ++r) {
      const int row = (r & 3) + 8 * (r >> 2) + 4 * lh;
      sb[(wave * 32 + row) * 33 + li] = acc[tap][r];
    }
    __syncthreads();
    constexpr int RPW = 32 / S2_NW;
#pragma unroll
    for (int j = 0; j < RPW / 2; ++j) {
      const int row = RPW * wave + (RPW / 2) * lh + j;
      float v = sb[row * 33 + li];
#pragma unroll
      for (int w = 1; w < S2_NW; ++w) v += sb[(w * 32 + row) * 33 + li];
      if (a.dw) {
        float* d = a.dw + ((size_t)(co0 + row) * a.Cin + ci0 + li) * 9 + tap;
        *d = a.accumulate ? *d + v : v;
      } else {
        out[((size_t)tap * a.Cout + co0 + row) * a.Cin + ci0 + li] = v;
      }
    }
  }
}

struct WgS2Plan { int th, tw, nw, nchunk, tpc, ntiles; };
inline WgS2Plan wgrad_s2_plan(int B, int H, int W, int Cin, int Cout, int ksize, int stride) {
  WgS2Plan pl{0, 0, 0, 0, 0, 0};
  if (ksize != 3 || (stride != 1 && stride != 2) || (Cin & 31) || (Cout & 31) || B <= 0) return pl;
  if (stride == 2 && ((H | W) & 1)) return pl;
  bool force = false;
  if (const char* e = sst_env(stride == 2 ? "SST_WGRAD_S2" : "SST_WGRAD_S1T")) {
    if (atoi(e) == 0) return pl;
    force = true;
  }
  const int Ho = H / stride, Wo = W / stride;
  constexpr int NW = 8;
  int th = 0, tw = 0;
  if (stride == 2) {
    if (Wo % 8 == 0 && Ho % 2 == 0) { th = 2; tw = 8; }
    else if (Wo % 6 == 0 && Ho % 2 == 0) { th = 2; tw = 6; }
  } else {
    if (2.0 * B * H * W * Cin * Cout * 9 < 2.5e9 && !force) return pl;
    if (Wo % 8 == 0 && Ho % 4 == 0) { th = 4; tw = 8; }
    else if (Wo % 6 == 0 && Ho % 4 == 0) { th = 4; tw = 6; }
  }
  if (!th || (int64_t)B * H * W * Cin >= (1ll << 31)) return pl;
  const int ntiles = B * (Ho / th) * (Wo / tw);
  const int nblk = (Cout >> 5) * (Cin >> 5);
  int nchunk = 256 / nblk;
  if (nchunk < 1) nchunk = 1;
  int tpc = ((ntiles + nchunk - 1) / nchunk + NW - 1) / NW * NW;
  if (tpc < NW) tpc = NW;
  nchunk = (ntiles + tpc - 1) / tpc;
  pl = WgS2Plan{th, tw, NW, nchunk, tpc, ntiles};
  return pl;
}

template <int S, int TH, int TW, int S2_NW>
static int launch_wgrad_s2_t(const WgS2Args& a, const WgS2Plan& pl, hipStream_t st) {
  using G = WgS2Geom<S, TH, TW, S2_NW>;
  static bool lds_ok = false;
  if (!lds_ok) {
    if (hipFuncSetAttribute(reinterpret_cast<const void*>(&conv_wgrad_tile_kernel<S, TH, TW, S2_NW>),
                            hipFuncAttributeMaxDynamicSharedMemorySize, (int)G::LDS_BYTES) != hipSuccess)
      return sst_set_error(SST_ERR_HIP, "conv_wgrad_tile: cannot raise the LDS limit");
    lds_ok = true;
  }
  conv_wgrad_tile_kernel<S, TH, TW, S2_NW><<<dim3(pl.nchunk, (a.Cout >> 5) * (a.Cin >> 5)), S2_NW * 64, G::LDS_BYTES, st>>>(a);
  return SST_OK;
}

static long g_wgrad_band_launches = 0;
SST_API long sst_debug_wgrad_band_launches(void) { return g_wgrad_band_launches; }

static int launch_wgrad_band(WgradArgs& a, const WgBandPlan& pl, int njobs, hipStream_t st, const WgJobTab& tab) {
  ++g_wgrad_band_launches;
  static bool big_lds_enabled = false;
  if (!big_lds_enabled) {
    if (hipFuncSetAttribute(reinterpret_cast<const void*>(&conv_wgrad_band_kernel<7>), hipFuncAttributeMaxDynamicSharedMemorySize,
                            80 * 1024) != hipSuccess ||
        hipFuncSetAttribute(reinterpret_cast<const void*>(&conv_wgrad_band_kernel<WB_XS>),
                            hipFuncAttributeMaxDynamicSharedMemorySize, 80 * 1024) != hipSuccess)
      return sst_set_error(SST_ERR_HIP, "conv_wgrad_band: cannot raise the LDS limit");
    big_lds_enabled = true;
  }
  a.R = pl.R; a.bpc = pl.bpc; a.nbands = pl.nbands; a.nchunk = pl.nchunk;
  dim3 grid((unsigned)pl.nchunk * njobs, (a.Cout >> 6) * (a.Cin >> 6));
  const int xslots = ((pl.R + 2) * (a.W + 2) * 16 + CONV_NT - 1) / CONV_NT;
  if (xslots <= 7)
    conv_wgrad_band_kernel<7><<<grid, CONV_NT, pl.lds, st>>>(a, tab);
  else
    conv_wgrad_band_kernel<WB_XS><<<grid, CONV_NT, pl.lds, st>>>(a, tab);
  SST_LAUNCH_CHECK("conv_wgrad_band_kernel");
  return SST_OK;
}

namespace {
enum class WgKind { TILE, BAND, K3C3_MFMA, K3C3, GENERAL_VEC, GENERAL_SCALAR };
struct WgradPlan {
  WgKind kind;
  int nchunk;
  int pending;
  int slab_chunks;
  int chunk_px;
  WgS2Plan tile;
  WgBandPlan band;
  const char* name;
};

WgradPlan wgrad_plan(int B, int H, int W, int Cin, int Cout, int ksize, int stride, int njobs, bool has_in_scale, int in_act,
                     bool grouped) {
  WgradPlan p{};
  if (!grouped) p.tile = wgrad_s2_plan(B, H, W, Cin, Cout, ksize, stride);
  if (p.tile.th) {
    static const char* const names[2][2] = {{"conv_wgrad_tile_kernel<1, 4, 8, 8>", "conv_wgrad_tile_kernel<1, 4, 6, 8>"},
                                            {"conv_wgrad_tile_kernel<2, 2, 8, 8>", "conv_wgrad_tile_kernel<2, 2, 6, 8>"}};
    const bool direct = p.tile.nchunk == 1 && !sst_env("SST_WGRAD_TILE_NO_DIRECT");
    p.kind = WgKind::TILE;
    p.nchunk = p.slab_chunks = p.tile.nchunk;
    p.pending = direct ? 0 : p.nchunk;
    p.name = names[stride == 2][p.tile.tw == 6];
    return p;
  }
  p.band = wgrad_band_plan(B, H, W, Cin, Cout, ksize, stride, njobs);
  if (p.band.R) {
    p.kind = WgKind::BAND;
    p.nchunk = p.slab_chunks = p.band.nchunk;
    p.pending = grouped ? 0 : p.nchunk;
    p.name = ((p.band.R + 2) * (W + 2) * 16 + CONV_NT - 1) / CONV_NT <= 7 ? "conv_wgrad_band_kernel<7>" : "conv_wgrad_band_kernel<10>";
    return p;
  }
  const int pad = ksize / 2, Ho = (H + 2 * pad - ksize) / stride + 1, Wo = (W + 2 * pad - ksize) / stride + 1;
  const int64_t M = (int64_t)B * Ho * Wo;
  int nchunk = sst_conv_wgrad_chunks(B, Ho, Wo, Cin, Cout, ksize);
  p.slab_chunks = nchunk;
  if (Cin == 3 && ksize == 3 && stride == 1) {
    const int rows = B * ((H + C3_ROWS - 1) / C3_ROWS);
    const bool mfma = k3c3_mfma_applies(W, Cout);
    if (rows > p.slab_chunks) p.slab_chunks = rows;
    if (mfma && k3c3_mfma_chunks(B, H, W) > p.slab_chunks) p.slab_chunks = k3c3_mfma_chunks(B, H, W);
    if (!grouped && k3c3_applies(Cin, ksize, stride, has_in_scale, in_act)) {
      if (mfma) {
        p.kind = WgKind::K3C3_MFMA;
        p.nchunk = k3c3_mfma_chunks(B, H, W);
        p.name = "wgrad_k3c3_mfma_kernel";
        return p;
      }
      if (!sst_env("SST_WGRAD_NO_K3C3")) {
        p.kind = WgKind::K3C3;
        p.nchunk = p.pending = rows;
        p.name = "wgrad_k3c3_kernel";
        return p;
      }
    }
  }
  if (grouped) {
    int target = 2048;
    if (const char* e = sst_env("SST_WGRAD_GROUP_WGS")) target = atoi(e);
    const int nblk = ((Cout + 63) / 64) * ((Cin + 63) / 64);
    int want = (target + ksize * ksize * nblk * njobs - 1) / (ksize * ksize * nblk * njobs);
    if (want < 1) want = 1;
    if (target > 0 && want < nchunk) {
      const int64_t cpx = ((M + want - 1) / want + SUB - 1) / SUB * SUB;
      nchunk = (int)((M + cpx - 1) / cpx);
    }
  }
  const bool vec = (Cin & 3) == 0 && (Cout & 3) == 0;
  p.kind = vec ? WgKind::GENERAL_VEC : WgKind::GENERAL_SCALAR;
  p.nchunk = nchunk;
  p.pending = grouped ? 0 : nchunk;
  p.chunk_px = (int)(((M + nchunk - 1) / nchunk + SUB - 1) / SUB * SUB);
  p.name = vec ? "conv_wgrad_kernel<true>" : "conv_wgrad_kernel<false>";
  return p;
}

void wgrad_shape_args(WgradArgs& a, const WgradPlan& pl, int B, int H, int W, int Cin, int Cout, int ksize, int stride) {
  a.B = B; a.H = H; a.W = W; a.Cin = Cin; a.Cout = Cout; a.stride = stride; a.KS = ksize; a.pad = ksize / 2;
  a.Ho = (H + 2 * a.pad - ksize) / stride + 1;
  a.Wo = (W + 2 * a.pad - ksize) / stride + 1;
  a.chunk_px = pl.chunk_px;
}
}

SST_API int sst_conv_wgrad_chunks2(int B, int H, int W, int Cin, int Cout, int ksize, int stride, int njobs) {
  return wgrad_plan(B, H, W, Cin, Cout, ksize, stride, njobs, false, ACT_NONE, njobs > 1).slab_chunks;
}

SST_API const char* sst_conv_wgrad_kernel_name(int B, int H, int W, int Cin, int Cout, int ksize, int stride, int njobs) {
  return wgrad_plan(B, H, W, Cin, Cout, ksize, stride, njobs, false, ACT_NONE, njobs > 1).name;
}

SST_API int sst_conv_wgrad_groups_ok(int B, int H, int W, int Cin, int Cout, int ksize, int stride, int grp_images) {
  return grp_images > 0 && B > 0 && B % grp_images == 0 &&
         wgrad_plan(B, H, W, Cin, Cout, ksize, stride, 1, true, ACT_NONE, false).kind == WgKind::TILE;
}

SST_API int sst_conv_wgrad_pending_reduce(int B, int H, int W, int Cin, int Cout, int ksize, int stride, int has_in_scale, int in_act) {
  return wgrad_plan(B, H, W, Cin, Cout, ksize, stride, 1, has_in_scale != 0, in_act, false).pending;
}

SST_API int sst_conv_wgrad_grp(const float* x, const float* dy, float* slab, float* dw, const float* in_scale,
                               const float* in_shift, const float* in_slope, float in_slope_const, int in_act, int B, int H,
                               int W, int Cin, int Cout, int stride, int ksize, int accumulate, int grp_images, void* stream) {
  SST_REQUIRE(x && dy && slab && dw, "sst_conv_wgrad: null pointer");
  SST_REQUIRE(B > 0 && H > 0 && W > 0 && Cin > 0 && Cout > 0 && (stride == 1 || stride == 2) && (ksize & 1) && ksize <= 9,
              "sst_conv_wgrad: bad shape");
  const WgradPlan pl = wgrad_plan(B, H, W, Cin, Cout, ksize, stride, 1, in_scale != nullptr, in_act, false);
  const bool grouped = grp_images > 0 && grp_images < B && in_scale;
  SST_REQUIRE(!grouped || (B % grp_images == 0 && pl.kind == WgKind::TILE),
              "sst_conv_wgrad: coefficient groups are only taken by the all-taps tile kernel (B=%d H=%d W=%d Cin=%d Cout=%d stride=%d)", B, H, W,
              Cin, Cout, stride);
  WgradArgs a;
  a.grouped = 0; a.nchunk = 0;
  static const WgJobTab no_tab{};
  a.x = x; a.dy = dy; a.slab = slab; a.in_scale = in_scale; a.in_shift = in_shift; a.in_slope = in_slope;
  a.in_slope_const = in_slope_const; a.in_act = in_act;
  wgrad_shape_args(a, pl, B, H, W, Cin, Cout, ksize, stride);
  SST_REQUIRE((int64_t)B * a.Ho * a.Wo < (1ll << 31), "sst_conv_wgrad: too many pixels");
  {
    const char* e = sst_env("SST_WGRAD_DBG");
    a.dbg = e ? atoi(e) : 0;
  }
  const int KK = ksize * ksize;
  const dim3 grid(pl.nchunk, KK, ((Cout + 63) / 64) * ((Cin + 63) / 64));
  hipStream_t st = sst_stream(stream);
  switch (pl.kind) {
    case WgKind::BAND: {
      const int rc = launch_wgrad_band(a, pl.band, 1, st, no_tab);
      if (rc != SST_OK) return rc;
      break;
    }
    case WgKind::TILE: {
      const WgS2Plan& p2 = pl.tile;
      WgS2Args s2;
      s2.x = x; s2.dy = dy; s2.slab = slab; s2.in_scale = in_scale; s2.in_shift = in_shift; s2.in_slope = in_slope;
      s2.in_slope_const = in_slope_const; s2.in_act = in_act;
      s2.B = B; s2.H = H; s2.W = W; s2.Cin = Cin; s2.Cout = Cout; s2.Ho = a.Ho; s2.Wo = a.Wo;
      s2.dbg = sst_env("SST_WGRAD_S2_DBG") ? atoi(sst_env("SST_WGRAD_S2_DBG")) : 0;
      s2.dw = pl.pending ? nullptr : dw;
      s2.accumulate = accumulate & 1;
      s2.gB = grouped ? grp_images : 0;
      s2.tiles_x = a.Wo / p2.tw; s2.tiles_img = (a.Ho / p2.th) * s2.tiles_x; s2.ntiles = p2.ntiles; s2.tpc = p2.tpc;
      int rc;
      if (stride == 2) rc = p2.tw == 8 ? launch_wgrad_s2_t<2, 2, 8, 8>(s2, p2, st) : launch_wgrad_s2_t<2, 2, 6, 8>(s2, p2, st);
      else rc = p2.tw == 8 ? launch_wgrad_s2_t<1, 4, 8, 8>(s2, p2, st) : launch_wgrad_s2_t<1, 4, 6, 8>(s2, p2, st);
      if (rc != SST_OK) return rc;
      break;
    }
    case WgKind::K3C3_MFMA:
      wgrad_k3c3_mfma_kernel<<<pl.nchunk, CONV_NT, 0, st>>>(x, dy, slab, B, H, W, B * H * (W >> 5));
      SST_LAUNCH_CHECK("wgrad_k3c3_mfma_kernel");
      c3m_reduce_kernel<<<9 * 64 * 3 / C3R_OUT, 1024, 0, st>>>(slab, dw, pl.nchunk, accumulate & 1);
      SST_LAUNCH_CHECK("c3m_reduce_kernel");
      return SST_OK;
    case WgKind::K3C3: {
      const size_t lds = (size_t)(C3_ROWS + 2) * ((W + 2) * 3 + 3) * sizeof(float);
      SST_REQUIRE(lds <= 48 * 1024, "sst_conv_wgrad: image too wide for the 3-channel-input kernel (W=%d)", W);
      wgrad_k3c3_kernel<<<dim3(pl.nchunk, 1), CONV_NT, lds, st>>>(x, dy, slab, B, H, W, Cout);
      break;
    }
    case WgKind::GENERAL_VEC: conv_wgrad_kernel<true><<<grid, CONV_NT, 0, st>>>(a, no_tab); break;
    case WgKind::GENERAL_SCALAR: conv_wgrad_kernel<false><<<grid, CONV_NT, 0, st>>>(a, no_tab); break;
  }
  SST_LAUNCH_CHECK(pl.name);
  if (pl.pending == 0 || (accumulate & 4)) return SST_OK;
  launch_wgrad_reduce(slab, dw, pl.nchunk, KK, Cout, Cin, accumulate, nullptr, 1, st);
  SST_LAUNCH_CHECK("wgrad_reduce_kernel");
  return SST_OK;
}

SST_API int sst_wgrad_reduce_multi(const void* jobs, int njobs, void* stream) {
  static_assert(sizeof(WrJob) == 40, "WrJob layout");
  SST_REQUIRE(jobs && njobs > 0 && njobs <= WR_TAB_MAX, "sst_wgrad_reduce_multi: 1..%d jobs", WR_TAB_MAX);
  WrJobTab tab{};
  memcpy(tab.j, jobs, (size_t)njobs * sizeof(WrJob));
  int maxb = 0;
  for (int i = 0; i < njobs; ++i) {
    WrJob& j = tab.j[i];
    SST_REQUIRE(j.slab && j.dw && j.nchunk > 0 && j.KK > 0 && j.Cout > 0 && j.Cin > 0, "sst_wgrad_reduce_multi: bad job %d", i);
    const int64_t total = (int64_t)j.KK * j.Cout * j.Cin;
    if ((j.Cin & 3) == 0 && j.nchunk >= 8) {
      j.blocks = (int)((total / 4 + 63) / 64);
    } else {
      const int64_t items = (j.Cin & 3) == 0 ? total / 4 : total;
      j.blocks = (int)((items + 255) / 256 < 1024 ? (items + 255) / 256 : 1024);
    }
    if (j.blocks > maxb) maxb = j.blocks;
  }
  wgrad_reduce_multi_kernel<<<dim3(maxb, njobs), 256, 0, sst_stream(stream)>>>(tab);
  SST_LAUNCH_CHECK("wgrad_reduce_multi_kernel");
  return SST_OK;
}

SST_API int sst_conv_wgrad_grouped(const void* jobs, int njobs, int B, int H, int W, int Cin, int Cout, int stride, int ksize,
                                   int accumulate, void* stream) {
  static_assert(sizeof(WgJob) == 64, "WgJob layout");
  SST_REQUIRE(jobs && njobs > 0 && njobs <= WG_TAB_MAX && B > 0 && H > 0 && W > 0 && Cin > 0 && Cout > 0 && (stride == 1 || stride == 2) &&
                  (ksize & 1) && ksize <= 9, "sst_conv_wgrad_grouped: bad argument (at most %d jobs per call)", WG_TAB_MAX);
  WgJobTab tab{};
  memcpy(tab.j, jobs, (size_t)njobs * sizeof(WgJob));
  const WgradPlan pl = wgrad_plan(B, H, W, Cin, Cout, ksize, stride, njobs, true, ACT_NONE, true);
  WgradArgs a;
  a.grouped = 1;
  a.x = a.dy = nullptr; a.slab = nullptr; a.in_scale = a.in_shift = a.in_slope = nullptr; a.in_slope_const = 0.f; a.in_act = 0;
  wgrad_shape_args(a, pl, B, H, W, Cin, Cout, ksize, stride);
  SST_REQUIRE((int64_t)B * a.Ho * a.Wo < (1ll << 31), "sst_conv_wgrad_grouped: too many pixels");
  a.nchunk = pl.nchunk;
  a.dbg = 0;
  const int KK = ksize * ksize;
  const dim3 grid((unsigned)pl.nchunk * njobs, KK, ((Cout + 63) / 64) * ((Cin + 63) / 64));
  hipStream_t st = sst_stream(stream);
  if (pl.kind == WgKind::BAND) {
    const int rc = launch_wgrad_band(a, pl.band, njobs, st, tab);
    if (rc != SST_OK) return rc;
  } else if (pl.kind == WgKind::GENERAL_VEC)
    conv_wgrad_kernel<true><<<grid, CONV_NT, 0, st>>>(a, tab);
  else
    conv_wgrad_kernel<false><<<grid, CONV_NT, 0, st>>>(a, tab);
  SST_LAUNCH_CHECK("conv_wgrad_kernel (grouped)");
  launch_wgrad_reduce(nullptr, nullptr, pl.nchunk, KK, Cout, Cin, accumulate, &tab, njobs, st);
  SST_LAUNCH_CHECK("wgrad_reduce_kernel (grouped)");
  return SST_OK;
}
```

### srgan-st_amd/srganst/_abi.py

```python
from __future__ import annotations

import ctypes
import os
from ctypes import c_char_p, c_float, c_int, c_int64, c_void_p, POINTER

_HERE = os.path.dirname(os.path.abspath(__file__))
LIB_PATH = os.environ.get("SST_LIB_PATH") or os.path.join(_HERE, "lib", "libsrganst.so")

P = c_void_p

SIGNATURES = {
    "sst_last_error": (c_char_p, []),
    "sst_version": (c_int, []),
    "sst_arch": (c_char_p, []),
    "sst_clear_error": (c_int, []),
    "sst_reload_env": (c_int, []),
    "sst_st_loss_workspace": (c_int, [c_int, c_int, c_int, POINTER(c_int64)]),
    "sst_st_loss_fwd": (c_int, [P, P, P, P, P, P, c_int, c_int, c_int, c_float, c_float, c_int, P]),
    "sst_st_loss_bwd": (c_int, [P, P, P, P, c_float, c_int, c_int, c_int, c_int, c_float, c_float, P]),
    "sst_st_pixel_loss_fwd": (c_int, [P, P, P, P, P, P, P, P, c_int, c_int, c_int, c_int, c_float, c_float, c_int, P]),
    "sst_st_pixel_loss_bwd": (c_int, [P, P, P, P, P, c_float, c_float, c_int, c_int, c_int, c_int, c_int, c_float, c_float, P]),
    "sst_st_maps_workspace": (c_int, [c_int, c_int, c_int, POINTER(c_int64)]),
    "sst_st_maps": (c_int, [P, P, P, P, P, P, P, P, c_int, c_int, c_int, c_float, c_float, c_int, P]),
    "sst_conv_packed_floats": (c_int64, [c_int, c_int, c_int]),
    "sst_conv_pack": (c_int, [P, P, c_int, c_int, c_int, c_int, P]),
    "sst_conv_pack_multi": (c_int, [P, c_int, c_int, P]),
    "sst_conv_kernel_name": (c_char_p, [c_int, c_int, c_int, c_int, c_int, c_int, c_int, c_int, c_int]),
    "sst_conv_wgrad_kernel_name": (c_char_p, [c_int, c_int, c_int, c_int, c_int, c_int, c_int, c_int]),
    "sst_debug_big_tile_launches": (ctypes.c_long, []),
    "sst_adam_flat": (c_int, [P, P, P, P, c_int64, P, P, c_int, ctypes.c_double, ctypes.c_double, ctypes.c_double,
                            ctypes.c_double, P]),
    "sst_adam_flat_ema": (c_int, [P, P, P, P, P, c_int64, P, P, c_int, ctypes.c_double, ctypes.c_double, ctypes.c_double,
                                ctypes.c_double, ctypes.c_double, c_int, P]),
    "sst_ema_flat": (c_int, [P, P, c_int64, P, ctypes.c_double, c_int, P]),
    "sst_debug_band_launches": (ctypes.c_long, []),
    "sst_debug_wgrad_band_launches": (ctypes.c_long, []),
    "sst_debug_mfma_peak": (c_int, [P, c_int, c_int, P]),
    "sst_debug_bf16x3": (c_int, [P, P, P, P, c_int, c_int, c_int, P]),
    "sst_debug_stamp": (c_int, [P, c_int, P]),
    "sst_conv_mtiles": (c_int, [c_int, c_int, c_int]),
    "sst_conv_stat_tiles": (c_int, [c_int, c_int, c_int, c_int, c_int, c_int, c_int]),
    "sst_conv_fwd": (c_int, [P, P, P, P, P, P, P, P, c_float, c_int, P, P, P, c_int,
                             c_int, c_int, c_int, c_int, c_int, c_int, c_int, P]),
    "sst_conv_pipe_supported": (c_int, [c_int, c_int, c_int, c_int, c_int, c_int, c_int]),
    "sst_conv_pipe_stat_tiles": (c_int, [c_int, c_int, c_int, c_int, c_int, c_int, c_int]),
    "sst_conv_pipe_ws_floats": (c_int64, [c_int, c_int, c_int, c_int, c_int, c_int, c_int]),
    "sst_conv_pipe_groups_ok": (c_int, [c_int, c_int, c_int, c_int, c_int, c_int, c_int, c_int]),
    "sst_conv_pipe_fwd_grp": (c_int, [P, P, P, P, P, P, P, c_float, c_int, P, P, P, P, P, P, c_float, c_int, P, P,
                                      c_int, c_int, c_int, c_int, c_int, c_int, c_int, c_int, P]),
    "sst_conv_ns_supported": (c_int, [c_int, c_int, c_int, c_int, c_int, c_int, c_int, c_int]),
    "sst_conv_ns_fwd": (c_int, [P, P, P, P, P, P, P, c_float, c_int, P, P, P, P, P, P, c_float, c_int, P,
                                c_int, c_int, c_int, c_int, c_int, c_int, c_int, c_int, c_int, P]),
    "sst_conv_s2_dgrad_pipe_supported": (c_int, [c_int, c_int, c_int, c_int, c_int]),
    "sst_conv_s2_dgrad_pipe_ws_floats": (c_int64, [c_int, c_int, c_int, c_int, c_int]),
    "sst_conv_s2_dgrad_pipe_stat_tiles": (c_int, [c_int, c_int, c_int, c_int, c_int]),
    "sst_conv_s2_dgrad_pipe_groups_ok": (c_int, [c_int, c_int, c_int, c_int, c_int, c_int]),
    "sst_conv_s2_dgrad_pipe_bwdstats_grp": (c_int, [P, P, P, P, P, P, P, P, c_float, c_int, P, c_int, c_int, c_int, c_int, c_int, c_int, P]),
    "sst_conv_acc_supported": (c_int, [c_int, c_int, c_int, c_int, c_int, c_int, c_int]),
    "sst_conv_fwd_acc": (c_int, [P, P, P, P, P, P, P, P, c_float, c_int, P, P, P, c_float, c_float, c_float, P, P, P, P, P, P, P,
                                 c_int, c_int, c_int, c_int, c_int, c_int, c_int, P]),
    "sst_conv_dgrad_fused_acc": (c_int, [P, P, P, P, P, c_float, c_int, P, P, P, P, P, P, P, P, c_float, c_int, P, P, P, P, c_float, P, P, P,
                                         P, c_int, c_int, c_int, c_int, c_int, c_int, c_int, P]),
    "sst_bn_finalize_acc": (c_int, [P, c_int, c_int, c_float, P, P, P, P, P, P, P, P, c_float, c_float, P]),
    "sst_conv_fwd_resin": (c_int, [P, P, P, P, P, P, P, P, P, P, P, c_int, c_int, c_int, c_int, c_int, c_int, P]),
    "sst_conv_dgrad_bwdstats": (c_int, [P, P, P, P, P, P, P, P, c_float, c_int, P, c_int, c_int, c_int, c_int, c_int, c_int, P]),
    "sst_conv_dgrad_fused": (c_int, [P, P, P, P, P, P, P, P, c_float, c_int, P, P, P, P, P, P, P, P, c_float, c_int, P,
                                     c_int, c_int, c_int, c_int, c_int, c_int, P]),
    "sst_conv_wgrad_chunks2": (c_int, [c_int, c_int, c_int, c_int, c_int, c_int, c_int, c_int]),
    "sst_conv_wgrad_groups_ok": (c_int, [c_int, c_int, c_int, c_int, c_int, c_int, c_int, c_int]),
    "sst_conv_wgrad_grp": (c_int, [P, P, P, P, P, P, P, c_float, c_int, c_int, c_int, c_int, c_int, c_int,
                                   c_int, c_int, c_int, c_int, P]),
    "sst_conv_wgrad_grouped": (c_int, [P, c_int, c_int, c_int, c_int, c_int, c_int, c_int, c_int, c_int, P]),
    "sst_conv_wgrad_pending_reduce": (c_int, [c_int, c_int, c_int, c_int, c_int, c_int, c_int, c_int, c_int]),
    "sst_wgrad_reduce_multi": (c_int, [P, c_int, P]),
    "sst_bn_finalize_grp": (c_int, [P, P, c_int, c_int, c_int, P, P, P, P, P, P, P, P, c_float, c_float, P]),
    "sst_bn_eval_affine": (c_int, [P, P, P, P, P, P, c_int, c_float, P]),
    "sst_bn_residual": (c_int, [P, P, P, P, P, P, c_int64, c_int, P]),
    "sst_bwd_reduce_blocks": (c_int, [c_int64, c_int]),
    "sst_bwd_finalize": (c_int, [P, c_int, c_int, c_float, P, P, P, P, P, P, P, P, P, c_int, P]),
    "sst_bwd_reduce_grp": (c_int, [P, P, P, P, P, P, c_float, c_int, P, c_int64, c_int, c_int, P]),
    "sst_bwd_finalize_grp": (c_int, [P, c_int, c_int, c_float, c_int, P, P, P, P, P, P, P, P, c_int, P]),
    "sst_bwd_apply_grp": (c_int, [P, P, P, P, P, P, c_float, c_int, P, P, P, P, c_int64, c_int, c_int, P]),
    "sst_bwd_finalize_wide": (c_int, [P, c_int, c_int, c_float, P, P, P, P, P, P, P, P, P, c_int, P, P, P]),
    "sst_act_bwd_partial_blocks": (c_int, [c_int64]),
    "sst_act_bwd_partial": (c_int, [P, P, P, P, c_float, P, P, c_int64, c_int, c_int, c_int, P]),
    "sst_bwd_apply": (c_int, [P, P, P, P, P, P, c_float, c_int, P, P, P, P, c_int64, c_int, c_int, c_int, P]),
    "sst_add": (c_int, [P, P, P, c_int64, P]),
    "sst_transpose": (c_int, [P, P, c_int, c_int, c_int, c_int, c_int, P]),
    "sst_transpose_affine": (c_int, [P, P, c_int, c_int, c_int, c_int, c_int, P, P, P]),
    "sst_maxpool_relu_fwd": (c_int, [P, P, c_int, c_int, c_int, c_int, P]),
    "sst_maxpool_relu_bwd": (c_int, [P, P, P, c_int, c_int, c_int, c_int, P]),
    "sst_clamp_bwd_blocks": (c_int, [c_int, c_int, c_int]),
    "sst_clamp_bwd": (c_int, [P, P, P, P, P, c_int, c_int, c_int, c_int, c_int, P]),
    "sst_pixel_loss_blocks": (c_int, [c_int64]),
    "sst_pixel_loss_fwd": (c_int, [P, P, P, P, P, c_int64, c_int, P]),
    "sst_pixel_loss_bwd": (c_int, [P, P, P, P, c_float, c_int, c_int64, c_int, P]),
    "sst_bce_logits": (c_int, [P, c_float, P, P, P, c_float, c_int, P]),
    "sst_bicubic": (c_int, [P, P, P, P, P, P, c_int64, c_int, c_int, c_int, c_int, c_int, c_int, c_int, P]),
    "sst_gather_batch": (c_int, [P, c_int64, P, c_int, c_int, c_int, P, P, P, P, P, P, P, c_int, c_int, c_int, c_int, P]),
    "sst_gather_crops": (c_int, [P, c_int64, P, c_int64, P, c_int, c_int, P, P, P, P, P, P, P, c_int, c_int, c_int, c_int, c_int, P]),
    "sst_image_metrics_workspace": (c_int, [c_int, c_int, c_int, POINTER(c_int64)]),
    "sst_image_metrics": (c_int, [P, P, c_int, c_int, c_int, P, P, P, P, P]),
    "sst_tile_gather": (c_int, [P, P, c_int64, c_int, c_int, P, c_int, c_int, c_int, c_int, P, P, P]),
    "sst_tile_scatter": (c_int, [P, P, c_int, c_int, c_int, c_int, c_int, c_int, c_int, P, c_int, P]),
    "sst_canvas_to_u8": (c_int, [P, c_int, c_int, c_float, P, P]),
    "sst_feat_loss_fwd": (c_int, [P, P, P, P, c_float, c_int, P, P, P, c_int64, c_int, P]),
    "sst_feat_loss_bwd": (c_int, [P, P, P, P, c_float, c_int, P, P, c_float, c_int, c_int64, c_int, P]),
    "sst_bb_blocks": (c_int, [c_int, c_int, c_int]),
    "sst_bb_feature_dim": (c_int, [c_int]),
    "sst_bb_patches": (c_int, [P, P, P, c_int, c_int, c_int, c_int, c_int, c_int, P, P]),
    "sst_bb_match_dist": (c_int, [P, P, P, P, P, P, c_int, c_int, c_int, c_int, c_float, c_float, c_int, c_int, P, c_int, P]),
    "sst_bbg_patches": (c_int, [c_int, c_int, c_int, c_int, c_int]),
    "sst_bbg_blocks": (c_int, [c_int, c_int]),
    "sst_bbg_unfold": (c_int, [P, P, P, c_int, c_int, c_int, c_int, c_int, c_int, c_int, c_int, P]),
    "sst_bbg_match": (c_int, [P, P, P, P, P, P, c_int, c_int, c_int, c_int, c_float, c_float, c_int, c_int, P]),
    "sst_bbg_fold": (c_int, [P, P, c_int, c_int, c_int, c_int, c_int, c_int, P]),
    "sst_weighted_sum": (c_int, [POINTER(c_void_p), POINTER(c_float), c_int, P, P, P]),
    "sst_wgrad_c3_supported": (c_int, [c_int, c_int]),
    "sst_wgrad_c3_slab_floats": (c_int64, [c_int, c_int, c_int, c_int]),
    "sst_wgrad_c3": (c_int, [P, P, P, P, P, c_float, c_int, c_int, c_int, c_int, c_int, c_int, c_int, P]),
    "sst_conv9_c3_packed_floats": (c_int64, [c_int]),
    "sst_conv9_c3_pack": (c_int, [P, P, c_int, c_int, c_int, P]),
    "sst_conv9_c3_fwd": (c_int, [P, P, P, P, c_int, c_int, c_int, c_int, P]),
    "sst_conv9_to3_packed_floats": (c_int64, [c_int]),
    "sst_conv9_to3_pack": (c_int, [P, P, c_int, P]),
    "sst_conv9_to3_fwd": (c_int, [P, P, P, P, P, P, c_float, c_int, c_int, c_int, c_int, c_int, P]),
    "sst_conv_s2_dgrad_tiles": (c_int, [c_int, c_int, c_int]),
    "sst_conv_s2_dgrad_kernel_name": (c_char_p, [c_int, c_int, c_int, c_int, c_int, c_int]),
    "sst_conv_s2_dgrad_fused": (c_int, [P, P, P, P, P, P, P, P, c_float, c_int, P, P, P, P, P, P, P, c_float, c_int, P,
                                        c_int, c_int, c_int, c_int, c_int, P]),
    "sst_conv_s2_dgrad_packed_floats": (c_int64, [c_int, c_int]),
    "sst_conv_s2_dgrad_pack": (c_int, [P, P, c_int, c_int, P]),
    "sst_conv_s2_dgrad": (c_int, [P, P, P, c_int, c_int, c_int, c_int, c_int, P]),
    "sst_linear_ksplit": (c_int, [c_int, c_int, c_int]),
    "sst_linear_fwd": (c_int, [P, P, P, P, P, c_int, c_int, c_int, P]),
    "sst_linear_dgrad": (c_int, [P, P, P, c_int, c_int, c_int, c_int, c_int, P]),
    "sst_linear_wgrad": (c_int, [P, P, P, P, c_int, c_int, c_int, c_int, P]),
    "sst_head_fwd": (c_int, [P, P, P, P, c_int, c_int, c_int, c_float, P]),
    "sst_head_bwd": (c_int, [P, P, P, P, P, P, c_int, c_int, c_int, c_float, c_int, P]),
    "sst_flatten_act_grp": (c_int, [P, P, P, c_float, c_int, P, c_int, c_int, c_int, c_int, P]),
}

_lib = None


class HipPathError(RuntimeError):
    pass


def lib() -> ctypes.CDLL:
    global _lib
    if _lib is None:
        if not os.path.exists(LIB_PATH):
            raise HipPathError(
                f"{LIB_PATH} is missing - build it with `python -c 'import __graft_entry__ as g; g.build()'` "
                "(make -C srgan-st_amd/csrc).  There is no CPU fallback for the HIP path.")
        import torch
        l = ctypes.CDLL(LIB_PATH)
        for name, (res, args) in SIGNATURES.items():
            fn = getattr(l, name)
            fn.restype = res
            fn.argtypes = args
        _lib = l
    return _lib


def reload_env() -> None:
    if _lib is not None:
        _lib.sst_reload_env()


def check(rc: int, what: str) -> None:
    if rc != 0:
        msg = lib().sst_last_error().decode(errors="replace")
        raise HipPathError(f"{what} failed (code {rc}): {msg}")


def ptr(t) -> int:
    if t is None:
        return None
    if not t.is_cuda:
        raise HipPathError("HIP path needs tensors on a ROCm device (no CPU fallback)")
    if not t.is_contiguous():
        raise HipPathError("HIP path needs contiguous tensors")
    return t.data_ptr()


def stream_ptr() -> int:
    import torch
    return torch.cuda.current_stream().cuda_stream
```

### srgan-st_amd/srganst/disc_graph.py

```python
from __future__ import annotations

from collections import namedtuple
from dataclasses import dataclass

import torch

from . import ops
from ._state import KeptPass, state
from .ops import ACT_SLOPE

LRELU = 0.2

PLAN = [(0, None, 1), (2, 3, 2), (5, 6, 1), (8, 9, 2), (11, 12, 1), (14, 15, 2), (17, 18, 1), (20, 21, 2)]


class _Layer:
    __slots__ = ("ci", "bi", "stride", "y", "mean", "rstd", "scale", "shift", "st", "cnt")

    def __init__(self, ci, bi, stride, y, mean=None, rstd=None, scale=None, shift=None):
        self.ci, self.bi, self.stride, self.y = ci, bi, stride, y
        self.mean, self.rstd, self.scale, self.shift, self.st, self.cnt = mean, rstd, scale, shift, None, None

    def epi(self, prefix=""):
        return {prefix + "y": self.y, prefix + "scale": self.scale, prefix + "shift": self.shift, prefix + "slope_const": LRELU,
                prefix + "act": 1}


@dataclass
class _Saved:
    x3: torch.Tensor
    layers: list
    flat: torch.Tensor | None
    h1: torch.Tensor | None
    groups: int
    gB: int
    wd: dict | None
    ws2: dict | None

    def input_of(self, li):
        if li == 0:
            return self.x3, dict(in_scale=None, in_shift=None, in_slope_const=LRELU, in_act=0)
        r = self.layers[li - 1]
        return r.y, dict(in_scale=r.scale, in_shift=r.shift, in_slope_const=LRELU, in_act=ACT_SLOPE)


_Packs = namedtuple("_Packs", "sig wp wd ws2")


class _GradSink:
    __slots__ = ("views", "acc", "taken", "g")

    def __init__(self, module, p, need_param_grads):
        names = list(p.keys())
        hs = state(module)
        scope = hs.grad_accum if need_param_grads else None
        self.acc = scope is not None and scope.flat is not None
        if self.acc:
            plist = [p[n] for n in names]
            offs, _ = ops.flat_layout(plist)
            self.views = {n: scope.flat[o:o + t.numel()].view(t.shape) for n, t, o in zip(names, plist, offs)}
        else:
            self.views = ops.flat_grads(module, names, [p[n] for n in names]) if need_param_grads else {}
            if scope is not None:
                scope.flat = hs.flat_grads[-1]
        self.taken, self.g = {}, None

    def take(self, name):
        t = self.taken[name] = self.views[name]
        return t

    def grads(self):
        return {} if self.acc else self.taken


def param_dict(module):
    names = [n for n, _ in module.named_parameters()]
    return names, dict(zip(names, [t.detach() for t in module.parameters()]))


def packs(module, p, with_dgrad, counter_add=0):
    hs = state(module)
    cache = hs.cache
    names = [f"features.{ci}.weight" for ci, _, _ in PLAN]
    n1, n2 = ([n for n, (_, _, s) in zip(names, PLAN) if s == stride] for stride in (1, 2))
    sig = tuple((p[n].data_ptr(), p[n]._version) for n in names)
    st = cache.get("pack_state")
    if hs.owner is not None and hs.packs_fresh and st is not None and st.sig == sig and (st.wd is not None or not with_dgrad):
        assert not counter_add, "the packs are fresh: nothing to ride along with"
        return st.wp, st.wd, st.ws2
    ws = [p[n] for n in names] + ([p[n] for n in n1] if with_dgrad else [])
    modes = [ops.PACK_FWD] * len(names) + ([ops.PACK_DGRAD] * len(n1) if with_dgrad else [])
    extras = (("add", ops.flatten_bn_counters(module), int(counter_add)),) if counter_add else ()
    out = ops.packed_weights(cache, ("pack", bool(with_dgrad), int(counter_add)), ws, modes, extras)
    wp = dict(zip(names, out[:len(names)]))
    wd = ws2 = None
    if with_dgrad:
        wd = dict(zip(n1, out[len(names):]))
        ws2 = {n: ops.pack_conv_s2_dgrad(p[n], out=cache.get(("s2", n))) for n in n2}
        for n in n2:
            cache[("s2", n)] = ws2[n]
    cache["pack_state"] = _Packs(sig, wp, wd, ws2)
    hs.packs_fresh = True
    return wp, wd, ws2


def groups_supported(module, p, gB, groups, H, W):
    B = gB * groups
    h, w = H, W
    for li, (ci, bi, stride) in enumerate(PLAN):
        wt = p[f"features.{ci}.weight"]
        cout, cin = wt.shape[0], wt.shape[1]
        if li > 0 and not (ops.conv_pipe_groups_ok(B, h, w, cin, cout, 3, stride, gB)
                           and (stride != 1 or ops.conv_pipe_groups_ok(B, h, w, cout, cin, 3, 1, gB))
                           and ops.conv_wgrad_groups_ok(B, h, w, cin, cout, 3, stride, gB)):
            return False
        h, w = ops.conv_out_hw(h, w, 3, stride)
    return B <= 64


class PassArena:

    def __init__(self, slots):
        self.slots, self.B, self.filled = slots, None, set()
        self.x3 = self.flat = self.h1 = None
        self.y, self.bn = [None] * len(PLAN), [None] * len(PLAN)

    def part(self, slot, name, li, shape, like):
        if name != "bn":
            self.B = self.B or shape[0]
            assert shape[0] == self.B, "every pass of an arena has the same batch size"
        held, key = (self.__dict__, name) if li is None else (getattr(self, name), li)
        if held[key] is None:
            full = (4, self.slots, *shape) if name == "bn" else (self.slots * shape[0], *shape[1:])
            held[key] = torch.empty(full, device=like.device, dtype=torch.float32)
        return tuple(held[key][:, slot]) if name == "bn" else held[key][slot * self.B:(slot + 1) * self.B]

    def all_slots(self, sv):
        assert len(self.filled) == self.slots, "not every pass of the arena has run"
        layers = [_Layer(ci, bi, stride, self.y[li], *(self.bn[li] if bi is not None else ())) for li, (ci, bi, stride) in enumerate(PLAN)]
        return _Saved(self.x3, layers, self.flat, self.h1, self.slots, self.B, sv.wd, sv.ws2)


def forward(module, x, p, training, need_grad=False, arena=None):
    groups, gB = 1, 0
    ar, slot = arena if arena is not None else (None, 0)
    assert ar is None or (training and not isinstance(x, (list, tuple)))
    if isinstance(x, (list, tuple)):
        groups, gB = len(x), x[0].shape[0]
        if groups == 1:
            x, gB = x[0], 0
        elif not training:
            raise NotImplementedError("batched passes are a train-mode schedule (eval mode has no per-pass statistics to keep apart)")
    wp, wd, ws2 = packs(module, p, need_grad)
    if training and not state(module).counters_external:
        ops.flatten_bn_counters(module).add_(groups)
    if groups > 1:
        _, c3, hh, ww = x[0].shape
        x3 = torch.empty(groups * gB, hh, ww, c3, device=x[0].device, dtype=torch.float32)
        for gi, xi in enumerate(x):
            assert xi.shape == x[0].shape
            ops.transpose(xi.contiguous(), to_nchw=False, out=x3[gi * gB:(gi + 1) * gB])
    else:
        Bq, c3, hh, ww = x.shape
        x3 = ops.transpose(x.contiguous(), to_nchw=False, out=ar and ar.part(slot, "x3", None, (Bq, hh, ww, c3), x))
    sv = _Saved(x3, [], None, None, groups, gB, wd, ws2)
    for li, (ci, bi, stride) in enumerate(PLAN):
        h, in_kw = sv.input_of(li)
        cout = p[f"features.{ci}.weight"].shape[0]
        ho, wo = ops.conv_out_hw(h.shape[1], h.shape[2], 3, stride)
        y, _, st, cnt = ops.conv_fwd(h, wp[f"features.{ci}.weight"], cout, 3, stride, bias=p.get(f"features.{ci}.bias"), **in_kw,
                                     want_stats=(bi is not None and training), grp=gB,
                                     out=ar and ar.part(slot, "y", li, (h.shape[0], ho, wo, cout), h))
        rec = _Layer(ci, bi, stride, y)
        if bi is not None:
            bn = module.features[bi]
            g, b = p[f"features.{bi}.weight"], p[f"features.{bi}.bias"]
            if training:
                rec.mean, rec.rstd, rec.scale, rec.shift = ops.bn_finalize(st, cnt, g, b, bn.running_mean, bn.running_var, groups=groups,
                                                                           out=ar and ar.part(slot, "bn", li, (cout,), h))
                rec.st, rec.cnt = st, cnt
            else:
                rec.scale, rec.shift = ops.bn_eval_affine(g, b, bn.running_mean, bn.running_var)
        sv.layers.append(rec)
    h, w0 = rec.y, p["classifier.0.weight"]
    sv.flat = ops.flatten_act(h, rec.scale, rec.shift, LRELU, 1, grp=gB,
                              out=ar and ar.part(slot, "flat", None, (h.shape[0], h[0].numel()), h))
    sv.h1 = ops.linear_fwd(sv.flat, w0, p["classifier.0.bias"], out=ar and ar.part(slot, "h1", None, (h.shape[0], w0.shape[0]), h))
    if ar is not None:
        ar.filled.add(slot)
    return ops.head_fwd(sv.h1, p["classifier.2.weight"], p["classifier.2.bias"], LRELU), sv


def replay_running_stats(module, p, sv):
    if not state(module).counters_external:
        ops.flatten_bn_counters(module).add_(sv.groups)
    for rec in sv.layers:
        if rec.bi is None:
            continue
        bn = module.features[rec.bi]
        ops.bn_finalize(rec.st, rec.cnt, p[f"features.{rec.bi}.weight"], p[f"features.{rec.bi}.bias"],
                        bn.running_mean, bn.running_var, groups=sv.groups)


def backward_classifier(module, p, sv, dout, need_param_grads):
    sink = _GradSink(module, p, need_param_grads)
    wg, acc = need_param_grads, sink.acc
    dh1 = ops.head_bwd(sv.h1, p["classifier.2.weight"], dout.contiguous(), LRELU, dw=sink.take("classifier.2.weight") if wg else None,
                       db=sink.take("classifier.2.bias") if wg else None, accumulate=acc)
    if wg:
        dw0, db0 = sink.take("classifier.0.weight"), sink.take("classifier.0.bias")
        with ops.SideStream(dh1, sv.flat, dw0, db0):
            ops.linear_wgrad(dh1, sv.flat, dw0, db0, accumulate=acc)
    B, H, W, C = sv.layers[-1].y.shape
    sink.g = ops.linear_dgrad(dh1, p["classifier.0.weight"], nhwc=(C, H * W)).view(B, H, W, C)
    return sink


def _bn_act_bwd(part, g, n, **kw):
    return ops.bwd_finalize_apply(part, g, n=n, **kw) if part is not None else ops.bwd_reduce_apply(g, n=n, **kw)


def backward_features(module, p, sv, sink, need_param_grads, need_dx, defer_wgrad=None, defer_below=None):
    wg, acc, g = need_param_grads, sink.acc, sink.g
    groups, gB = sv.groups, sv.gB
    dx = part = None
    reduces = [] if ops.WGRAD_REDUCE_MULTI else None
    for li in reversed(range(len(sv.layers))):
        r, below = sv.layers[li], sv.layers[li - 1] if li > 0 else None
        x, in_kw = sv.input_of(li)
        n = r.y.numel() // r.y.shape[-1] // groups
        wname = f"features.{r.ci}.weight"
        cin = p[wname].shape[1]
        if r.bi is not None:
            gam = p[f"features.{r.bi}.weight"]
            dg = sink.take(f"features.{r.bi}.weight") if wg else torch.empty_like(gam)
            db = sink.take(f"features.{r.bi}.bias") if wg else torch.empty_like(gam)
            dy = _bn_act_bwd(part, g, n, **r.epi(), mean=r.mean, rstd=r.rstd, gamma=gam, dgamma=dg, dbeta=db, accumulate=acc and wg,
                             groups=groups)
        elif wg:
            dy = _bn_act_bwd(part, g, n, **r.epi(), dbeta=sink.take(f"features.{r.ci}.bias"), accumulate=acc, groups=groups)
        else:
            dy = ops.bwd_apply(g, **r.epi(), groups=groups)
        part = None
        if wg:
            dwc = sink.take(wname)

            def launch(x=x, dy=dy, dwc=dwc, stride=r.stride, in_kw=in_kw, red=None):
                ops.conv_wgrad(x, dy, dwc, 3, stride, **in_kw, accumulate=acc, grp=gB, defer_reduce=red)
            if defer_wgrad is not None and (defer_below is None or li < defer_below):
                ev = torch.cuda.Event()
                ev.record()
                defer_wgrad.append((ev, launch, (x, dy, dwc, in_kw["in_scale"], in_kw["in_shift"])))
            else:
                with ops.SideStream(x, dy, dwc):
                    launch(red=reduces)
        if li == 0 and not need_dx:
            break
        if r.stride == 1:
            if below is not None:
                g, part = ops.conv_dgrad_bwdstats(dy, sv.wd[wname], cin, 3, **below.epi("epi_"), grp=gB)
            else:
                g = ops.conv_fwd(dy, sv.wd[wname], cin, 3, 1)[0]
        else:
            epi = below.epi() if below is not None and (below.bi is not None or wg) else None
            out = ops.conv_s2_dgrad(dy, sv.ws2[wname], x.shape[1], x.shape[2], cin, epi=epi, grp=gB)
            g, part = out if epi is not None else (out, None)
        if li == 0:
            dx = ops.transpose(g, to_nchw=True)
    if reduces:
        with ops.SideStream(*[t for j in reduces for t in j[:2]]):
            ops.wgrad_reduce_flush(reduces)
    ops.join_side()
    return sink.grads(), dx


def backward(module, p, sv, dout, need_param_grads, need_dx):
    sink = backward_classifier(module, p, sv, dout, need_param_grads)
    return backward_features(module, p, sv, sink, need_param_grads, need_dx)


class DiscriminatorFn(torch.autograd.Function):
    @staticmethod
    def forward(ctx, x, module, grad_mode, *params):
        names, p = param_dict(module)
        need_param = grad_mode and any(ctx.needs_input_grad[3:])
        need_dx = grad_mode and ctx.needs_input_grad[0]
        need_grad = need_param or need_dx
        if need_grad and not module.training:
            raise NotImplementedError("Discriminator backward in eval() mode is not on the reference's path (train.py:110)")
        hs = state(module)
        keep = hs.keep_pass and need_grad and module.training
        req = hs.arena_request if keep else None
        arena = (PassArena(req[0]), req[1]) if req is not None else None
        out, sv = forward(module, x, p, module.training, need_grad, arena=arena)
        if keep:
            hs.last_pass = KeptPass(x.data_ptr(), tuple(x.shape), out, sv, p, arena[0] if arena is not None else None)
        if need_grad:
            ctx.module, ctx.sv, ctx.p, ctx.names = module, sv, p, names
            ctx.need_param, ctx.need_dx = need_param, need_dx
        return out

    @staticmethod
    def backward(ctx, dout):
        grads, dx = backward(ctx.module, ctx.p, ctx.sv, dout, ctx.need_param, ctx.need_dx)
        ctx.sv = None
        return (dx, None, None, *[grads.get(n) for n in ctx.names])
```

### srgan-st_amd/srganst/ops.py

```python
from __future__ import annotations

import os

import torch

from . import _abi
from ._abi import check, ptr, stream_ptr
from ._state import state

OUT_NHWC, OUT_SHUFFLE, OUT_NCHW_CLAMP, OUT_UNSHUFFLE = 0, 1, 2, 3
ACT_NONE, ACT_SLOPE = 0, 1
BN_EPS, BN_MOMENTUM = 1e-5, 0.1


TRACE = None

TRACE_HBM = None


def _launch(fn, args, what, flops, name_fn, keep):
    check(fn(*args, stream_ptr()), what)
    if TRACE is not None:
        TRACE.setdefault(name_fn(), []).append((lambda: fn(*args, stream_ptr()), flops, keep))


def _launch_hbm(fn, args, what, name, nbytes, keep):
    check(fn(*args, stream_ptr()), what)
    if TRACE_HBM is not None:
        TRACE_HBM.setdefault(name, []).append((lambda: fn(*args, stream_ptr()), float(nbytes), keep))


def _in_args(scale=None, shift=None, slope=None, slope_const=0.0, act=ACT_NONE):
    return (ptr(scale), ptr(shift), ptr(slope), float(slope_const), int(act)), (scale, shift, slope)


def _epi_args(y=None, scale=None, shift=None, slope=None, slope_const=0.0, act=0):
    return (ptr(y), ptr(scale), ptr(shift), ptr(slope), float(slope_const), int(act)), (y, scale, shift, slope)


def _conv_name(B, H, W, cin, cout, ksize, stride, out_mode=0, fused_in=0):
    return _abi.lib().sst_conv_kernel_name(B, H, W, cin, cout, ksize, stride, int(out_mode) & 0xff, int(fused_in)).decode()


def _wgrad_name(B, H, W, cin, cout, ksize, stride, njobs):
    return _abi.lib().sst_conv_wgrad_kernel_name(B, H, W, cin, cout, ksize, stride, njobs).decode()


def _f32(*shape, like):
    return torch.empty(*shape, device=like.device, dtype=torch.float32)


def pack_conv(w: torch.Tensor, mode: int = 0, out: torch.Tensor | None = None) -> torch.Tensor:
    cout, cin, k, _ = w.shape
    o, i = (cin, cout) if mode else (cout, cin)
    n = _abi.lib().sst_conv_packed_floats(o, i, k)
    if out is None:
        out = _f32(n, like=w)
    assert out.numel() == n
    check(_abi.lib().sst_conv_pack(ptr(w), ptr(out), cout, cin, k, mode, stream_ptr()), "sst_conv_pack")
    return out


def conv_out_hw(h, w, k, stride):
    p = k // 2
    return (h + 2 * p - k) // stride + 1, (w + 2 * p - k) // stride + 1


CONV_NS = os.environ.get("SST_CONV_NS", "1") != "0"


def _pipe_on():
    return os.environ.get("SST_CONV_PIPE", "1") != "0"


class _ConvRoute:

    def __init__(self, shp, out_mode=OUT_NHWC, plain=True, want_stats=False):
        L = _abi.lib()
        self.shp, self.out_mode = shp, int(out_mode)
        pipe_tw = L.sst_conv_pipe_supported(*shp) if plain and out_mode == OUT_NHWC and _pipe_on() else 0
        shuffle = plain and out_mode == OUT_SHUFFLE and not want_stats
        ns_tw = L.sst_conv_ns_supported(*shp, self.out_mode) if CONV_NS and (pipe_tw or shuffle) else 0
        self.kind, self.tw = ("ns", ns_tw) if ns_tw else ("pipe", pipe_tw) if pipe_tw else ("general", 0)

    def rows(self):
        return (_abi.lib().sst_conv_stat_tiles if self.kind == "general" else _abi.lib().sst_conv_pipe_stat_tiles)(*self.shp)

    def ws_floats(self):
        return _abi.lib().sst_conv_pipe_ws_floats(*self.shp) if self.kind == "pipe" else 0

    def name(self):
        stride = self.shp[6]
        if self.kind == "general":
            return _conv_name(*self.shp, self.out_mode)
        return f"conv_ns_kernel<{stride}, {self.tw}>" if self.kind == "ns" else f"conv_pipe_kernel<{stride}, {self.tw}, 0>"

    def groups_ok(self, grp):
        return self.kind != "general" and self.out_mode == OUT_NHWC and bool(_abi.lib().sst_conv_pipe_groups_ok(*self.shp, int(grp)))


def conv_fwd(x, wp, cout, ksize=3, stride=1, bias=None, in_scale=None, in_shift=None, in_slope=None,
             in_slope_const=0.0, in_act=ACT_NONE, residual=None, want_stats=False, out_mode=OUT_NHWC,
             want_pre=False, grp=0, out=None):
    B, H, W, cin = x.shape
    route = _ConvRoute((B, H, W, cin, cout, ksize, stride), out_mode, residual is None and not want_pre, want_stats)
    if grp and grp < B and in_scale is not None and not route.groups_ok(grp):
        raise _abi.HipPathError(f"conv_fwd: coefficient groups of {grp} images are not supported for this shape")
    ho, wo = conv_out_hw(H, W, ksize, stride)
    if out is not None:
        assert out_mode == OUT_NHWC and tuple(out.shape) == (B, ho, wo, cout) and out.is_contiguous()
        y = out
    elif out_mode == OUT_NHWC:
        y = _f32(B, ho, wo, cout, like=x)
    elif out_mode == OUT_SHUFFLE:
        y = _f32(B, 2 * ho, 2 * wo, cout // 4, like=x)
    elif out_mode == OUT_NCHW_CLAMP:
        y = _f32(B, cout, ho, wo, like=x)
    else:
        y = _f32(B, ho // 2, wo // 2, cout * 4, like=x)
    inp, ikeep = _in_args(in_scale, in_shift, in_slope, in_slope_const, in_act)
    if route.kind != "general":
        stats, cnt, _ = _conv_tile(route, x, wp, y, bias, (inp, ikeep), want_stats, grp=grp if out_mode == OUT_NHWC else 0)
        return y, None, stats, cnt
    y_pre = torch.empty_like(y) if want_pre else None
    stats = cnt = None
    if want_stats:
        mt = route.rows()
        stats = _f32(mt, 2, cout, like=x)
        cnt = _f32(mt, like=x)
    args = (ptr(x), ptr(wp), ptr(y), ptr(y_pre), ptr(bias), *inp, ptr(residual), ptr(stats), ptr(cnt), int(out_mode), *route.shp)
    _launch(_abi.lib().sst_conv_fwd, args, "sst_conv_fwd", 2.0 * B * ho * wo * cout * cin * ksize * ksize, route.name,
            (x, wp, y, y_pre, bias, *ikeep, residual, stats, cnt))
    return y, y_pre, stats, cnt


def conv_pipe_groups_ok(B, H, W, cin, cout, ksize, stride, grp):
    return _ConvRoute((B, H, W, cin, cout, ksize, stride)).groups_ok(grp)


def conv_wgrad_groups_ok(B, H, W, cin, cout, ksize, stride, grp):
    return bool(_abi.lib().sst_conv_wgrad_groups_ok(B, H, W, cin, cout, ksize, stride, int(grp)))


def _conv_tile(route, x, wp, y, bias, inp, want_stats=False, epi=None, grp=0):
    L = _abi.lib()
    B, H, W, cin, cout, ksize, stride = route.shp
    stats = cnt = partial = None
    if want_stats:
        mt = route.rows()
        stats, cnt = _f32(mt, 2, cout, like=x), _f32(mt, like=x)
    if epi is not None:
        partial = _f32(route.rows(), 3, cout, like=x)
    nws = route.ws_floats()
    ws = _f32(nws, like=x) if nws else None
    (ia, ikeep), (ea, ekeep) = inp, epi or _epi_args()
    ho, wo = conv_out_hw(H, W, ksize, stride)
    ns = route.kind == "ns"
    args = (ptr(x), ptr(wp), ptr(y), ptr(bias), *ia, ptr(stats), ptr(cnt), *ea, ptr(partial), *(() if ns else (ptr(ws),)), *route.shp,
            *((route.out_mode,) if ns else ()), int(grp))
    _launch(L.sst_conv_ns_fwd if ns else L.sst_conv_pipe_fwd_grp, args, "sst_conv_ns_fwd" if ns else "sst_conv_pipe_fwd",
            2.0 * B * ho * wo * cout * cin * ksize * ksize, route.name, (x, wp, y, bias, *ikeep, stats, cnt, partial, ws, *ekeep))
    return stats, cnt, partial


_ONES = {}


def _ones(x, cin):
    key = (x.device, cin)
    if key not in _ONES:
        _ONES[key] = torch.ones(cin, device=x.device, dtype=torch.float32)
    return _ONES[key]


def conv_fwd_resin(x, y2, bn_scale, bn_shift, wp, cout, ksize=3, bias=None, want_stats=False):
    B, H, W, cin = x.shape
    ones = _ones(x, cin)
    y = _f32(B, H, W, cout, like=x)
    h = torch.empty_like(x)
    stats = cnt = None
    if want_stats:
        mt = _abi.lib().sst_conv_stat_tiles(B, H, W, cin, cout, ksize, 1)
        stats = _f32(mt, 2, cout, like=x)
        cnt = _f32(mt, like=x)
    args = (ptr(x), ptr(y2), ptr(ones), ptr(bn_scale), ptr(bn_shift), ptr(h), ptr(wp), ptr(y), ptr(bias), ptr(stats), ptr(cnt),
            B, H, W, cin, cout, ksize)
    _launch(_abi.lib().sst_conv_fwd_resin, args, "sst_conv_fwd_resin", 2.0 * B * H * W * cout * cin * ksize * ksize,
            lambda: _conv_name(B, H, W, cin, cout, ksize, 1, 0, 1), (x, y2, ones, bn_scale, bn_shift, h, wp, y, bias, stats, cnt))
    return y, h, stats, cnt


ACC_NREP = int(os.environ.get("SST_ACC_NREP", "16"))


def conv_acc_supported(B, H, W, cin, cout, ksize=3, stride=1):
    return bool(_abi.lib().sst_conv_acc_supported(B, H, W, cin, cout, ksize, stride)) and os.environ.get("SST_ATOMIC_STATS", "1") != "0"


def conv_fwd_acc(x, wp, cout, ksize=3, in2=None, bias=None, in_slope=None, in_slope_const=0.0, in_act=ACT_NONE, in_acc=None,
                 in_bn=None, n=0.0, out_stats=None, run_stats=None, st_acc=None):
    B, H, W, cin = x.shape
    y = _f32(B, H, W, cout, like=x)
    h = torch.empty_like(x) if in2 is not None else None
    ones = _ones(x, cin) if in2 is not None else None
    g, bta = in_bn if in_bn is not None else (None, None)
    om, orr, osc, osh = out_stats if out_stats is not None else (None, None, None, None)
    rm, rv = run_stats if run_stats is not None else (None, None)
    args = (ptr(x), ptr(in2), ptr(h), ptr(ones), ptr(wp), ptr(y), ptr(bias), ptr(in_slope), float(in_slope_const), int(in_act),
            _dptr(in_acc), ptr(g), ptr(bta), float(n), float(BN_EPS), float(BN_MOMENTUM), ptr(om), ptr(orr), ptr(osc), ptr(osh),
            ptr(rm), ptr(rv), _dptr(st_acc), ACC_NREP, B, H, W, cin, cout, ksize)
    _launch(_abi.lib().sst_conv_fwd_acc, args, "sst_conv_fwd_acc", 2.0 * B * H * W * cout * cin * ksize * ksize,
            lambda: _conv_name(B, H, W, cin, cout, ksize, 1, 0, 1),
            (x, in2, h, ones, wp, y, bias, in_slope, in_acc, g, bta, om, orr, osc, osh, rm, rv, st_acc))
    return y, h


def conv_dgrad_fused_acc(g, wd, cout, ksize=3, y2=None, in_scale=None, in_shift=None, in_slope=None, in_slope_const=0.0, in_act=0,
                         residual=None, epi_y=None, epi_scale=None, epi_shift=None, epi_slope=None, epi_slope_const=0.0, epi_act=0,
                         bw_in_acc=None, bn=None, n=0.0, dgamma=None, dbeta=None, dslope=None, bw_st_acc=None):
    B, H, W, cin = g.shape
    out = _f32(B, H, W, cout, like=g)
    dy = torch.empty_like(g) if y2 is not None else None
    mean, rstd, gamma = bn if bn is not None else (None, None, None)
    inp, ikeep = _in_args(in_scale, in_shift, in_slope, in_slope_const, in_act)
    epi, ekeep = _epi_args(epi_y, epi_scale, epi_shift, epi_slope, epi_slope_const, epi_act)
    args = (ptr(g), ptr(y2), *inp, ptr(dy), ptr(wd), ptr(out), ptr(residual), *epi, _dptr(bw_in_acc), ptr(mean), ptr(rstd), ptr(gamma),
            float(n), ptr(dgamma), ptr(dbeta), ptr(dslope), _dptr(bw_st_acc), ACC_NREP, B, H, W, cin, cout, ksize)
    _launch(_abi.lib().sst_conv_dgrad_fused_acc, args, "sst_conv_dgrad_fused_acc", 2.0 * B * H * W * cout * cin * ksize * ksize,
            lambda: _conv_name(B, H, W, cin, cout, ksize, 1, 0, 1),
            (g, y2, *ikeep, dy, wd, out, residual, *ekeep, bw_in_acc, mean, rstd, gamma, dgamma, dbeta, dslope, bw_st_acc))
    return out, dy


def _dptr(t):
    if t is None:
        return None
    assert t.is_cuda and t.is_contiguous() and t.dtype == torch.float64
    return t.data_ptr()


def bn_finalize_acc(acc, n, gamma, beta, run_mean=None, run_var=None):
    C = gamma.numel()
    mean, rstd, scale, shift = (_f32(C, like=gamma) for _ in range(4))
    check(_abi.lib().sst_bn_finalize_acc(_dptr(acc), acc.shape[0], C, float(n), ptr(gamma), ptr(beta), ptr(run_mean), ptr(run_var),
                                         ptr(mean), ptr(rstd), ptr(scale), ptr(shift), float(BN_EPS), float(BN_MOMENTUM), stream_ptr()),
          "sst_bn_finalize_acc")
    return mean, rstd, scale, shift


def conv_wgrad(x, dy, dw_out, ksize=3, stride=1, in_scale=None, in_shift=None, in_slope=None, in_slope_const=0.0,
               in_act=ACT_NONE, accumulate=False, grp=0, defer_reduce=None):
    B, H, W, cin = x.shape
    cout = dy.shape[-1]
    ho, wo = conv_out_hw(H, W, ksize, stride)
    assert tuple(dy.shape) == (B, ho, wo, cout) and tuple(dw_out.shape) == (cout, cin, ksize, ksize)
    nch = _abi.lib().sst_conv_wgrad_chunks2(B, H, W, cin, cout, ksize, stride, 1)
    slab = _f32(nch * ksize * ksize * cout * cin, like=x)
    pend = 0
    if defer_reduce is not None and TRACE is None:
        pend = _abi.lib().sst_conv_wgrad_pending_reduce(B, H, W, cin, cout, ksize, stride, int(in_scale is not None), int(in_act))
        if pend:
            assert dw_out.is_contiguous()
            defer_reduce.append((slab, dw_out, pend, ksize * ksize, cout, cin, int(bool(accumulate))))
    inp, ikeep = _in_args(in_scale, in_shift, in_slope, in_slope_const, in_act)
    args = (ptr(x), ptr(dy), ptr(slab), ptr(dw_out), *inp, B, H, W, cin, cout, stride, ksize, int(bool(accumulate)) | (4 if pend else 0),
            int(grp))

    def name():
        n = _wgrad_name(B, H, W, cin, cout, ksize, stride, 1)
        return n + ("+c3m_reduce_kernel" if n == "wgrad_k3c3_mfma_kernel" else "+wgrad_reduce_kernel")
    _launch(_abi.lib().sst_conv_wgrad_grp, args, "sst_conv_wgrad", 2.0 * B * ho * wo * cout * cin * ksize * ksize, name,
            (x, dy, slab, dw_out, *ikeep))
    return dw_out


WGRAD_REDUCE_MULTI = os.environ.get("SST_WGRAD_REDUCE_MULTI", "1") != "0"


def wgrad_reduce_flush(jobs):
    import ctypes
    import struct
    while jobs:
        js, jobs[:] = jobs[:24], jobs[24:]
        buf = b"".join(struct.pack("<QQiiiiii", slab.data_ptr(), dw.data_ptr(), nch, kk, cout, cin, acc, 0)
                       for slab, dw, nch, kk, cout, cin, acc in js)
        check(_abi.lib().sst_wgrad_reduce_multi(ctypes.c_char_p(buf), len(js), stream_ptr()), "sst_wgrad_reduce_multi")


def bn_finalize(stats, cnt, gamma, beta, run_mean=None, run_var=None, eps=BN_EPS, momentum=BN_MOMENTUM, groups=1, out=None):
    C = gamma.numel()
    shape = (C,) if groups == 1 else (groups, C)
    if out is not None:
        mean, rstd, scale, shift = out
        assert all(tuple(t.shape) == shape and t.is_contiguous() for t in out)
    else:
        mean, rstd, scale, shift = (_f32(*shape, like=gamma) for _ in range(4))
    check(_abi.lib().sst_bn_finalize_grp(ptr(stats), ptr(cnt), stats.shape[0], C, int(groups), ptr(gamma), ptr(beta), ptr(run_mean),
                                         ptr(run_var), ptr(mean), ptr(rstd), ptr(scale), ptr(shift), eps, momentum,
                                         stream_ptr()), "sst_bn_finalize")
    return mean, rstd, scale, shift


def bn_eval_affine(gamma, beta, run_mean, run_var, eps=BN_EPS):
    C = gamma.numel()
    scale, shift = _f32(C, like=gamma), _f32(C, like=gamma)
    check(_abi.lib().sst_bn_eval_affine(ptr(gamma), ptr(beta), ptr(run_mean), ptr(run_var), ptr(scale), ptr(shift), C, eps,
                                        stream_ptr()), "sst_bn_eval_affine")
    return scale, shift


def bn_residual(y, scale, shift, res, res_slope=None):
    C = y.shape[-1]
    out = torch.empty_like(y)
    check(_abi.lib().sst_bn_residual(ptr(y), ptr(scale), ptr(shift), ptr(res), ptr(res_slope), ptr(out), y.numel() // C, C,
                                     stream_ptr()), "sst_bn_residual")
    return out


def bwd_reduce(g, y, g2=None, scale=None, shift=None, slope=None, slope_const=0.0, act=0, groups=1):
    C = y.shape[-1]
    R = y.numel() // C // groups
    nblk = _abi.lib().sst_bwd_reduce_blocks(R, C)
    partial = _f32(groups * nblk, 3, C, like=y)
    check(_abi.lib().sst_bwd_reduce_grp(ptr(g), ptr(g2), ptr(y), ptr(scale), ptr(shift), ptr(slope), float(slope_const), int(act),
                                        ptr(partial), R, C, int(groups), stream_ptr()), "sst_bwd_reduce")
    return partial


def bwd_finalize(partial, n, mean=None, rstd=None, gamma=None, dgamma=None, dbeta=None, dslope=None, accumulate=False, groups=1):
    nblk, _, C = partial.shape
    cA = cB = cC = None
    if groups > 1:
        assert dslope is None and nblk % groups == 0
        if mean is not None:
            cA, cB, cC = (_f32(groups, C, like=partial) for _ in range(3))
        check(_abi.lib().sst_bwd_finalize_grp(ptr(partial), nblk // groups, C, float(n), int(groups), ptr(mean), ptr(rstd), ptr(gamma),
                                              ptr(dgamma), ptr(dbeta), ptr(cA), ptr(cB), ptr(cC), int(accumulate), stream_ptr()),
              "sst_bwd_finalize_grp")
        return cA, cB, cC
    if mean is not None:
        cA, cB, cC = (_f32(C, like=partial) for _ in range(3))
    if dslope is not None and C > 64:
        scratch = _f32((C + 63) // 64, like=partial)
        check(_abi.lib().sst_bwd_finalize_wide(ptr(partial), nblk, C, float(n), ptr(mean), ptr(rstd), ptr(gamma), ptr(dgamma),
                                               ptr(dbeta), ptr(cA), ptr(cB), ptr(cC), ptr(dslope), int(accumulate), ptr(scratch),
                                               _next_counter(partial.device), stream_ptr()), "sst_bwd_finalize_wide")
        return cA, cB, cC
    check(_abi.lib().sst_bwd_finalize(ptr(partial), nblk, C, float(n), ptr(mean), ptr(rstd), ptr(gamma), ptr(dgamma), ptr(dbeta),
                                      ptr(cA), ptr(cB), ptr(cC), ptr(dslope), int(accumulate), stream_ptr()),
          "sst_bwd_finalize")
    return cA, cB, cC


def act_bwd(g, y, g2=None, slope=None, slope_const=0.0, dbias=None, dslope=None, accumulate=False, unshuffle=False):
    C = y.shape[-1]
    R = y.numel() // C
    uh = uw = 0
    if unshuffle:
        B, uh, uw, _ = y.shape
        dy = _f32(B, uh // 2, uw // 2, 4 * C, like=y)
    else:
        dy = torch.empty_like(y)
    Cs = dy.shape[-1]
    nblk = _abi.lib().sst_act_bwd_partial_blocks(dy.numel() // Cs)
    partial = _f32(nblk, 3, Cs, like=y)
    check(_abi.lib().sst_act_bwd_partial(ptr(g), ptr(g2), ptr(y), ptr(slope), float(slope_const), ptr(dy), ptr(partial), R, C, uh, uw,
                                         stream_ptr()), "sst_act_bwd_partial")
    if dbias is not None or dslope is not None:
        bwd_finalize(partial, R, dbeta=dbias, dslope=dslope, accumulate=accumulate)
    return dy


def bwd_apply(g, y, g2=None, scale=None, shift=None, slope=None, slope_const=0.0, act=0, cA=None, cB=None, cC=None,
              unshuffle=False, groups=1):
    C = y.shape[-1]
    if groups > 1:
        assert not unshuffle
        dy = torch.empty_like(y)
        check(_abi.lib().sst_bwd_apply_grp(ptr(g), ptr(g2), ptr(y), ptr(scale), ptr(shift), ptr(slope), float(slope_const), int(act),
                                           ptr(cA), ptr(cB), ptr(cC), ptr(dy), y.numel() // C // groups, C, int(groups), stream_ptr()),
              "sst_bwd_apply_grp")
        return dy
    uh = uw = 0
    if unshuffle:
        B, uh, uw, _ = y.shape
        dy = _f32(B, uh // 2, uw // 2, 4 * C, like=y)
    else:
        dy = torch.empty_like(y)
    check(_abi.lib().sst_bwd_apply(ptr(g), ptr(g2), ptr(y), ptr(scale), ptr(shift), ptr(slope), float(slope_const), int(act),
                                   ptr(cA), ptr(cB), ptr(cC), ptr(dy), y.numel() // C, C, uh, uw, stream_ptr()),
          "sst_bwd_apply")
    return dy


def add(a, b):
    out = torch.empty_like(a)
    check(_abi.lib().sst_add(ptr(a), ptr(b), ptr(out), a.numel(), stream_ptr()), "sst_add")
    return out


def transpose(x, to_nchw: bool, out=None):
    if to_nchw:
        B, H, W, C = x.shape
        shape = (B, C, H, W)
    else:
        B, C, H, W = x.shape
        shape = (B, H, W, C)
    if out is None:
        out = _f32(*shape, like=x)
    assert tuple(out.shape) == shape and out.is_contiguous()
    check(_abi.lib().sst_transpose(ptr(x), ptr(out), B, C, H, W, int(to_nchw), stream_ptr()), "sst_transpose")
    return out


def clamp_bwd(g, pre, dbias=None, accumulate=False):
    B, C, H, W = g.shape
    out = _f32(B, H, W, C, like=g)
    partial = _f32(_abi.lib().sst_clamp_bwd_blocks(B, H, W) * C, like=g)
    check(_abi.lib().sst_clamp_bwd(ptr(g), ptr(pre), ptr(out), ptr(partial), ptr(dbias), int(accumulate), B, C, H, W,
                                   stream_ptr()), "sst_clamp_bwd")
    return out


def pixel_loss_fwd(x, gt, mode, ws):
    n = x.numel()
    key = (x.device, n)
    if ws.get("key") != key:
        ws["key"] = key
        ws["partials"] = _f32(_abi.lib().sst_pixel_loss_blocks(n), like=x)
        ws["counter"] = torch.zeros(1, device=x.device, dtype=torch.int32)
    loss = _f32((), like=x)
    check(_abi.lib().sst_pixel_loss_fwd(ptr(x), ptr(gt), ptr(loss), ptr(ws["partials"]), ptr(ws["counter"]), n, mode,
                                        stream_ptr()), "sst_pixel_loss_fwd")
    return loss


def pixel_loss_bwd(x, gt, mode, scale_dev=None, scale_host=1.0, out=None, accumulate=False):
    if out is None:
        out = torch.empty_like(x)
        accumulate = False
    check(_abi.lib().sst_pixel_loss_bwd(ptr(x), ptr(gt), ptr(out), ptr(scale_dev), float(scale_host), int(accumulate), x.numel(),
                                        mode, stream_ptr()), "sst_pixel_loss_bwd")
    return out


def bce_logits(logits, target, want_loss=True, want_grad=False, scale_dev=None, scale_host=1.0, grad_out=None):
    loss = _f32((), like=logits) if want_loss else None
    dl = (grad_out if grad_out is not None else torch.empty_like(logits)) if want_grad else None
    check(_abi.lib().sst_bce_logits(ptr(logits), float(target), ptr(loss), ptr(dl), ptr(scale_dev), float(scale_host),
                                    logits.numel(), stream_ptr()), "sst_bce_logits")
    return loss, dl


def pack_conv_s2_dgrad(w, out=None):
    cout, cin, k, _ = w.shape
    assert k == 3
    n = _abi.lib().sst_conv_s2_dgrad_packed_floats(cout, cin)
    wp = out if out is not None and out.numel() == n and out.device == w.device else _f32(n, like=w)
    check(_abi.lib().sst_conv_s2_dgrad_pack(ptr(w), ptr(wp), cout, cin, stream_ptr()), "sst_conv_s2_dgrad_pack")
    return wp


S2D_EPI = os.environ.get("SST_S2D_EPI", "0") != "0"
S2D_EPI_GRP = os.environ.get("SST_S2D_EPI_GRP", "0") != "0"


def _s2_dgrad_route(B, H, W, cin, cout, want_epi, grp):
    L = _abi.lib()
    shp = (B, H, W, cin, cout)
    tw = L.sst_conv_s2_dgrad_pipe_supported(*shp) if _pipe_on() else 0
    if not tw:
        return 0, 0, 0, lambda: L.sst_conv_s2_dgrad_kernel_name(*shp, 0).decode()
    grouped = bool(grp) and grp < B
    epi = want_epi and (S2D_EPI_GRP and bool(L.sst_conv_s2_dgrad_pipe_groups_ok(*shp, int(grp))) if grouped else S2D_EPI)
    return (tw, L.sst_conv_s2_dgrad_pipe_ws_floats(*shp), L.sst_conv_s2_dgrad_pipe_stat_tiles(*shp) if epi else 0,
            lambda: f"conv_pipe_kernel<1, {tw}, 1>")


def conv_s2_dgrad(dy, wp, H, W, cin, epi=None, grp=0):
    B, ho, wo, cout = dy.shape
    dx = _f32(B, H, W, cin, like=dy)
    L = _abi.lib()
    tw, nws, rows, name = _s2_dgrad_route(B, H, W, cin, cout, epi is not None, grp)
    flops, partial = 2.0 * B * ho * wo * cout * cin * 9, None
    if tw:
        ws = _f32(nws, like=dy) if nws else None
        ea, ekeep = _epi_args(**(epi or {}))
        if rows:
            partial = _f32(rows, 3, cin, like=dy)
        else:
            ea, grp = (None,) * 4 + ea[4:], 0
        _launch(L.sst_conv_s2_dgrad_pipe_bwdstats_grp, (ptr(dy), ptr(wp), ptr(dx), ptr(ws), *ea, ptr(partial), B, H, W, cin, cout, int(grp)),
                "sst_conv_s2_dgrad_pipe", flops, name, (dy, wp, dx, ws, partial, *ekeep))
    else:
        _launch(L.sst_conv_s2_dgrad, (ptr(dy), ptr(wp), ptr(dx), B, H, W, cin, cout), "sst_conv_s2_dgrad", flops, name, (dy, wp, dx))
    return (dx, partial) if epi is not None else dx


def conv_s2_dgrad_fused(g, y2, wp, H, W, cin, cA=None, cB=None, cC=None, in_scale=None, in_shift=None, in_slope=None,
                        in_slope_const=0.0, in_act=0, epi_y=None, epi_scale=None, epi_shift=None, epi_slope=None, epi_slope_const=0.0,
                        epi_act=0):
    B, ho, wo, cout = g.shape
    dx = _f32(B, H, W, cin, like=g)
    dy = torch.empty_like(g)
    partial = _f32(_abi.lib().sst_conv_s2_dgrad_tiles(B, H, W), 3, cin, like=g) if epi_y is not None else None
    inp, ikeep = _in_args(in_scale, in_shift, in_slope, in_slope_const, in_act)
    epi, ekeep = _epi_args(epi_y, epi_scale, epi_shift, epi_slope, epi_slope_const, epi_act)
    args = (ptr(g), ptr(y2), ptr(cA), ptr(cB), ptr(cC), *inp, ptr(dy), ptr(wp), ptr(dx), *epi, ptr(partial), B, H, W, cin, cout)
    _launch(_abi.lib().sst_conv_s2_dgrad_fused, args, "sst_conv_s2_dgrad_fused", 2.0 * B * ho * wo * cout * cin * 9,
            lambda: _abi.lib().sst_conv_s2_dgrad_kernel_name(B, H, W, cin, cout, 1).decode(),
            (g, y2, cA, cB, cC, *ikeep, dy, wp, dx, *ekeep, partial))
    return dx, dy, partial


def linear_fwd(x, w, bias, out=None):
    M, K = x.shape
    N = w.shape[0]
    y = out if out is not None else _f32(M, N, like=x)
    assert tuple(y.shape) == (M, N) and y.is_contiguous()
    slab = _f32(_abi.lib().sst_linear_ksplit(M, N, K) * M * N, like=x)
    _launch_hbm(_abi.lib().sst_linear_fwd, (ptr(x), ptr(w), ptr(bias), ptr(y), ptr(slab), M, N, K), "sst_linear_fwd", "linear_fwd_kernel",
                4.0 * (N * K + M * K + M * N), (x, w, bias, y, slab))
    return y


def linear_dgrad(dy, w, nhwc=None):
    M, N = dy.shape
    K = w.shape[1]
    dx = _f32(M, K, like=dy)
    c, hw = nhwc if nhwc else (0, 0)
    _launch_hbm(_abi.lib().sst_linear_dgrad, (ptr(dy), ptr(w), ptr(dx), M, N, K, c, hw), "sst_linear_dgrad", "linear_dgrad_kernel",
                4.0 * (N * K + M * K + M * N), (dy, w, dx))
    return dx


def linear_wgrad(dy, x, dw, db=None, accumulate=False):
    M, N = dy.shape
    K = x.shape[1]
    _launch_hbm(_abi.lib().sst_linear_wgrad, (ptr(dy), ptr(x), ptr(dw), ptr(db), M, N, K, int(accumulate)), "sst_linear_wgrad",
                "linear_wgrad_kernel", 4.0 * (N * K * (2 if accumulate else 1) + M * K + M * N), (dy, x, dw, db))


def head_fwd(h, w, b, slope):
    M, K = h.shape
    N = w.shape[0]
    y = _f32(M, N, like=h)
    check(_abi.lib().sst_head_fwd(ptr(h), ptr(w), ptr(b), ptr(y), M, N, K, float(slope), stream_ptr()), "sst_head_fwd")
    return y


def head_bwd(h, w, dy, slope, dw=None, db=None, accumulate=False):
    M, K = h.shape
    N = w.shape[0]
    dh = torch.empty_like(h)
    check(_abi.lib().sst_head_bwd(ptr(h), ptr(w), ptr(dy), ptr(dh), ptr(dw), ptr(db), M, N, K, float(slope), int(accumulate),
                                  stream_ptr()), "sst_head_bwd")
    return dh


def flatten_act(y, scale, shift, slope, act=1, grp=0, out=None):
    B, H, W, C = y.shape
    flat = out if out is not None else _f32(B, C * H * W, like=y)
    assert tuple(flat.shape) == (B, C * H * W) and flat.is_contiguous()
    check(_abi.lib().sst_flatten_act_grp(ptr(y), ptr(scale), ptr(shift), float(slope), int(act), ptr(flat), B, H * W, C, int(grp),
                                         stream_ptr()), "sst_flatten_act")
    return flat


def wgrad_c3(big, small, dw_out, kind, in_slope=None, in_slope_const=0.0, in_act=ACT_NONE, accumulate=False):
    B, H, W, C = big.shape
    assert tuple(small.shape) == (B, H, W, 3)
    assert tuple(dw_out.shape) == ((3, C, 9, 9) if kind == 0 else (C, 3, 9, 9))
    slab = _f32(_abi.lib().sst_wgrad_c3_slab_floats(B, H, W, C), like=big)
    check(_abi.lib().sst_wgrad_c3(ptr(big), ptr(small), ptr(slab), ptr(dw_out), ptr(in_slope), float(in_slope_const), int(in_act),
                                  kind, B, H, W, C, int(accumulate), stream_ptr()), "sst_wgrad_c3")
    return dw_out


def wgrad_c3_supported(C, ksize=9):
    return bool(_abi.lib().sst_wgrad_c3_supported(C, ksize))


PACK_FWD, PACK_DGRAD, PACK_C3_FWD, PACK_C3_DGRAD, PACK_TO3 = 0, 1, 2, 3, 4


class PackPlan:

    def __init__(self, weights, modes, extras=()):
        dev = weights[0].device
        self.ptrs = tuple(w.data_ptr() for w in weights) + self._extras_sig(extras)
        self.out, rows, blk = [], [], 0
        for w, m in zip(weights, modes):
            cout, cin, k, _ = w.shape
            if m == PACK_C3_FWD or m == PACK_C3_DGRAD:
                n = _abi.lib().sst_conv9_c3_packed_floats(cin if m == PACK_C3_DGRAD else cout)
            elif m == PACK_TO3:
                n = _abi.lib().sst_conv9_to3_packed_floats(cin)
            else:
                o, i = (cin, cout) if m else (cout, cin)
                n = _abi.lib().sst_conv_packed_floats(o, i, k)
            assert n < 2 ** 31
            wp = torch.empty(n, device=dev, dtype=torch.float32)
            self.out.append(wp)
            rows.append([w.data_ptr(), wp.data_ptr(), cout | (cin << 32), (k * k) | (int(m) << 32), n, blk])
            blk += (n + 1023) // 1024
        for e in extras:
            if e[0] == "zero":
                t = e[1]
                assert t.is_contiguous() and t.element_size() % 4 == 0
                n = t.numel() * (t.element_size() // 4)
                rows.append([0, t.data_ptr(), 0, 5 << 32, n, blk])
            else:
                t, k = e[1], int(e[2])
                assert e[0] == "add" and t.dtype == torch.int64 and t.is_contiguous() and 0 <= k < 2 ** 31
                n = t.numel()
                rows.append([0, t.data_ptr(), k, 6 << 32, n, blk])
            blk += (n + 1023) // 1024
        self.njobs = len(rows)
        self.blocks = blk
        self.table = torch.tensor(rows, dtype=torch.int64).to(dev)

    @staticmethod
    def _extras_sig(extras):
        return tuple((e[0], e[1].data_ptr(), e[1].numel(), int(e[2]) if len(e) > 2 else 0) for e in extras)

    def matches(self, weights, extras=()):
        return self.ptrs == tuple(w.data_ptr() for w in weights) + self._extras_sig(extras)

    def run(self):
        check(_abi.lib().sst_conv_pack_multi(ptr(self.table), self.njobs, self.blocks, stream_ptr()), "sst_conv_pack_multi")
        return self.out


def packed_weights(cache: dict, key, weights, modes, extras=()):
    plan = cache.get(key)
    if plan is None or not plan.matches(weights, extras):
        plan = PackPlan(weights, modes, extras)
        cache[key] = plan
    return plan.run()


_COUNTERS = {}


def _next_counter(device):
    st = _COUNTERS.get(device)
    if st is None:
        st = [torch.zeros(8192, device=device, dtype=torch.int32), 0]
        _COUNTERS[device] = st
    i = st[1]
    st[1] = (i + 1) % 8192
    return st[0].data_ptr() + 4 * i


def flatten_bn_counters(module):
    bns = [m for m in module.modules() if isinstance(m, torch.nn.BatchNorm2d)]
    if not bns:
        return None
    flat = state(module).nbt_flat
    ok = flat is not None and flat.device == bns[0].num_batches_tracked.device and all(
        bn.num_batches_tracked.data_ptr() == flat.data_ptr() + 8 * i for i, bn in enumerate(bns))
    if not ok:
        flat = torch.stack([bn.num_batches_tracked.detach().to(torch.int64) for bn in bns])
        for i, bn in enumerate(bns):
            bn._buffers["num_batches_tracked"] = flat[i]
        state(module).nbt_flat = flat
    return flat


OVERLAP = False
_SIDE = {}

CAPTURE_ORIGIN = None
TOPOLOGY_ERROR = None


class CaptureTopologyError(RuntimeError):
    pass


def check_capture_join(dst_stream):
    global TOPOLOGY_ERROR
    if CAPTURE_ORIGIN is not None and torch.cuda.is_current_stream_capturing() and dst_stream != CAPTURE_ORIGIN:
        TOPOLOGY_ERROR = (
            "a stream forked from a side branch of an open hipGraph capture may only be joined into the capture's origin stream: "
            "joining it into the side branch makes hipStreamEndCapture fault on ROCm 7.2 (ops.CAPTURE_ORIGIN, tools/capture_probe.py). "
            "Run this schedule outside the merged iteration (KERNEL.OVERLAP_GD = False) or without the helper stream.")
        raise CaptureTopologyError(TOPOLOGY_ERROR)


class SideStream:

    def __init__(self, *tensors):
        self.tensors = [t for t in tensors if t is not None]

    def __enter__(self):
        if not OVERLAP:
            return self
        main = torch.cuda.current_stream()
        side = _SIDE.get(main.device)
        if side is None:
            side = torch.cuda.Stream(device=main.device)
            _SIDE[main.device] = side
        side.wait_stream(main)
        for t in self.tensors:
            t.record_stream(side)
        self.ctx = torch.cuda.stream(side)
        self.ctx.__enter__()
        return self

    def __exit__(self, *exc):
        if OVERLAP:
            self.ctx.__exit__(*exc)
        return False


def join_side():
    if OVERLAP:
        main = torch.cuda.current_stream()
        side = _SIDE.get(main.device)
        if side is not None:
            check_capture_join(main)
            main.wait_stream(side)


def conv9_c3_fwd(x3, w, mode, bias=None, wp=None):
    B, H, W, _ = x3.shape
    cout = w.shape[1] if mode else w.shape[0]
    if wp is None:
        wp = _f32(_abi.lib().sst_conv9_c3_packed_floats(cout), like=w)
        check(_abi.lib().sst_conv9_c3_pack(ptr(w), ptr(wp), w.shape[0], w.shape[1], mode, stream_ptr()), "sst_conv9_c3_pack")
    y = _f32(B, H, W, cout, like=x3)
    check(_abi.lib().sst_conv9_c3_fwd(ptr(x3), ptr(wp), ptr(y), ptr(bias), B, H, W, cout, stream_ptr()), "sst_conv9_c3_fwd")
    return y


def conv9_to3_fwd(x, w, bias=None, in_slope=None, in_slope_const=0.0, in_act=ACT_NONE, want_pre=False, wp=None):
    B, H, W, C = x.shape
    assert tuple(w.shape) == (3, C, 9, 9)
    if wp is None:
        wp = _f32(_abi.lib().sst_conv9_to3_packed_floats(C), like=w)
        check(_abi.lib().sst_conv9_to3_pack(ptr(w), ptr(wp), C, stream_ptr()), "sst_conv9_to3_pack")
    y = _f32(B, 3, H, W, like=x)
    y_pre = torch.empty_like(y) if want_pre else None
    check(_abi.lib().sst_conv9_to3_fwd(ptr(x), ptr(wp), ptr(y), ptr(y_pre), ptr(bias), ptr(in_slope), float(in_slope_const),
                                       int(in_act), B, H, W, C, stream_ptr()), "sst_conv9_to3_fwd")
    return y, y_pre


def bwd_reduce_apply(g, y, n, g2=None, scale=None, shift=None, slope=None, slope_const=0.0, act=0, mean=None, rstd=None,
                     gamma=None, dgamma=None, dbeta=None, dslope=None, accumulate=False, unshuffle=False, groups=1):
    part = bwd_reduce(g, y, g2=g2, scale=scale, shift=shift, slope=slope, slope_const=slope_const, act=act, groups=groups)
    cA, cB, cC = bwd_finalize(part, n, mean, rstd, gamma, dgamma, dbeta, dslope, accumulate, groups=groups)
    return bwd_apply(g, y, g2=g2, scale=scale, shift=shift, slope=slope, slope_const=slope_const, act=act, cA=cA, cB=cB, cC=cC,
                     unshuffle=unshuffle, groups=groups)


def transpose_affine(x, to_nchw: bool, scale, shift=None):
    if to_nchw:
        B, H, W, C = x.shape
        out = _f32(B, C, H, W, like=x)
    else:
        B, C, H, W = x.shape
        out = _f32(B, H, W, C, like=x)
    check(_abi.lib().sst_transpose_affine(ptr(x), ptr(out), B, C, H, W, int(to_nchw), ptr(scale), ptr(shift), stream_ptr()),
          "sst_transpose_affine")
    return out


def maxpool_relu_fwd(y):
    B, H, W, C = y.shape
    out = _f32(B, H // 2, W // 2, C, like=y)
    check(_abi.lib().sst_maxpool_relu_fwd(ptr(y), ptr(out), B, H, W, C, stream_ptr()), "sst_maxpool_relu_fwd")
    return out


def maxpool_relu_bwd(g, y):
    B, H, W, C = y.shape
    dy = torch.empty_like(y)
    check(_abi.lib().sst_maxpool_relu_bwd(ptr(g), ptr(y), ptr(dy), B, H, W, C, stream_ptr()), "sst_maxpool_relu_bwd")
    return dy


# ... 175 lines not shown
```

Before: 3258 HR images/s.

## Fuse LeakyReLU backward into stride-2 dgrad and bias grad into first-layer wgrad

For the discriminator's first conv layer (no BN, stride 1, followed by a stride-2 conv), the stride-2 data-gradient pipe kernel gets a new mode that applies the LeakyReLU derivative in its epilogue, reading the forward activation. This replaces the separate epilogue/stats path and the apply pass. The first layer's 3-channel wgrad MFMA kernel also computes the bias gradient through a constant-ones row, with extra reduce blocks summing it in double. Both remove extra elementwise and reduction passes over the largest activation, at the cost of more template variants and extra loads in the epilogue.

```diff
diff --git a/include/srganst.h b/include/srganst.h
--- a/include/srganst.h
+++ b/include/srganst.h
@@ -69,6 +69,9 @@
                                     const float* epi_scale, const float* epi_shift, const float* epi_slope,
                                     float epi_slope_const, int epi_act, float* epi_partial, int B, int H, int W, int Cin,
                                     int Cout, int grp_images, void* stream);
+int sst_conv_s2_dgrad_pipe_act_supported(int B, int H, int W, int Cin, int Cout);
+int sst_conv_s2_dgrad_pipe_act(const float* dy, const float* wp, float* dx, float* ws, const float* act_y, float act_slope, int B,
+                               int H, int W, int Cin, int Cout, void* stream);
 int sst_conv_dgrad_bwdstats(const float* x, const float* wp, float* y, const float* residual, const float* epi_y,
                             const float* epi_scale, const float* epi_shift, const float* epi_slope,
                             float epi_slope_const, int epi_act, float* epi_partial, int B, int H, int W, int Cin,
@@ -104,6 +107,9 @@
                    const float* in_shift, const float* in_slope, float in_slope_const, int in_act,
                    int B, int H, int W, int Cin, int Cout, int stride, int ksize, int accumulate,
                        int grp_images, void* stream);
+int sst_conv_wgrad_db_supported(int B, int H, int W, int Cin, int Cout, int ksize, int stride);
+int sst_conv_wgrad_db(const float* x, const float* dy, float* slab, float* dw, float* dbslab, float* db, int B, int H, int W,
+                      int Cin, int Cout, int accumulate, void* stream);
 int sst_conv_wgrad_pending_reduce(int B, int H, int W, int Cin, int Cout, int ksize, int stride, int has_in_scale, int in_act);
 int sst_wgrad_reduce_multi(const void* jobs, int njobs, void* stream);
 int sst_wgrad_c3_supported(int C, int ksize);
diff --git a/srgan-st_amd/csrc/conv_pipe.hip b/srgan-st_amd/csrc/conv_pipe.hip
--- a/srgan-st_amd/csrc/conv_pipe.hip
+++ b/srgan-st_amd/csrc/conv_pipe.hip
@@ -26,6 +26,8 @@
   int dbg;
 #endif
   int gB, grows;
+  const float* act_y;
+  float act_slope;
 };
 
 template <int S, int TW, int MODE>
@@ -68,9 +70,19 @@
   return t;
 }
 
+template <int TW>
+__device__ __forceinline__ f32x4 pipe_act_load(const PipeArgs& a, int r0, int ox0, int c0, int lane, int cls) {
+  const int px = lane & 31;
+  const int r = r0 + px / TW, ox = ox0 + px % TW;
+  f32x4 z = {0.f, 0.f, 0.f, 0.f};
+  if (r < a.R && ox < a.Wo)
+    z = *reinterpret_cast<const f32x4*>(a.act_y + ((size_t)(2 * r + (cls >> 1)) * (2 * a.Wo) + 2 * ox + (cls & 1)) * a.Cout + c0);
+  return z;
+}
+
 template <int TW, int MODE = 0>
 __device__ __forceinline__ void pipe_epilogue(const PipeArgs& a, float v[4], int r0, int ox0, int c0, int mt, int lane, bool first,
-                                              int cls = 0) {
+                                              int cls = 0, f32x4 zq = f32x4{0.f, 0.f, 0.f, 0.f}) {
   constexpr int TH = 32 / TW;
   const int px = lane & 31;
   const int r = r0 + px / TW, ox = ox0 + px % TW;
@@ -78,6 +90,10 @@
   size_t obase;
   if (MODE) {
     obase = ((size_t)(2 * r + (cls >> 1)) * (2 * a.Wo) + 2 * ox + (cls & 1)) * a.Cout + c0;
+    if (MODE == 2) {
+#pragma unroll
+      for (int j = 0; j < 4; ++j) v[j] = zq[j] > 0.f ? v[j] : v[j] * a.act_slope;
+    }
     if (pix_ok) *reinterpret_cast<f32x4*>(a.y + obase) = f32x4{v[0], v[1], v[2], v[3]};
   }
   if (!MODE && a.bias) {
@@ -342,6 +358,11 @@
       const int cl = 8 * wave + 4 * lh;
 #pragma unroll
       for (int k0 = 0; k0 < NACC; k0 += NPAIR) {
+        f32x4 zq[NPAIR];
+        if (MODE == 2 && a.ksplit == 1) {
+#pragma unroll
+          for (int k = 0; k < NPAIR; ++k) zq[k] = pipe_act_load<TW>(a, r0, ox0, nf * 32 + cl, lane, k0 + k);
+        }
         __syncthreads();
 #pragma unroll
         for (int k = 0; k < NPAIR; ++k)
@@ -369,7 +390,7 @@
             *reinterpret_cast<f32x4*>(a.ws + (((size_t)part * a.total_tiles + tile) * NACC + k0 + k) * 1024 + li * 32 + cl) =
                 f32x4{v[0], v[1], v[2], v[3]};
           } else {
-            pipe_epilogue<TW, MODE>(a, v, r0, ox0, nf * 32 + cl, mt, lane, nf == 0 && wave == 0, k0 + k);
+            pipe_epilogue<TW, MODE>(a, v, r0, ox0, nf * 32 + cl, mt, lane, nf == 0 && wave == 0, k0 + k, zq[k]);
           }
         }
       }
@@ -392,6 +413,8 @@
   const int li = lane & 31, cl = 8 * wave + 4 * (lane >> 5);
   const size_t slab = (size_t)a.total_tiles * NACC * 1024;
   const float* src = a.ws + ((size_t)tile * NACC + cls) * 1024 + li * 32 + cl;
+  f32x4 zq = {0.f, 0.f, 0.f, 0.f};
+  if (MODE == 2) zq = pipe_act_load<TW>(a, ty * (32 / TW), tx * TW, nf * 32 + cl, lane, cls);
   f32x4 s = *reinterpret_cast<const f32x4*>(src);
   for (int k = 1; k < a.ksplit; ++k) {
     const f32x4 t = *reinterpret_cast<const f32x4*>(src + k * slab);
@@ -399,7 +422,7 @@
     for (int j = 0; j < 4; ++j) s[j] += t[j];
   }
   float v[4] = {s[0], s[1], s[2], s[3]};
-  pipe_epilogue<TW, MODE>(a, v, ty * (32 / TW), tx * TW, nf * 32 + cl, mt, lane, nf == 0 && wave == 0, cls);
+  pipe_epilogue<TW, MODE>(a, v, ty * (32 / TW), tx * TW, nf * 32 + cl, mt, lane, nf == 0 && wave == 0, cls, zq);
 }
 
 struct PipePlan {
@@ -485,6 +508,7 @@
   a.ksplit = pl.ksplit; a.cb_per = pl.ncb / pl.ksplit; a.units = a.total_tiles * pl.ksplit;
   a.gB = (grp_images > 0 && grp_images < B) ? grp_images : 0;
   a.grows = a.gB * a.Ho;
+  a.act_y = nullptr; a.act_slope = 0.f;
 #ifdef SST_PIPE_ABLATE
   a.dbg = sst_env("SST_PIPE_DBG") ? atoi(sst_env("SST_PIPE_DBG")) : 0;
 #endif
@@ -555,10 +579,10 @@
   if (!pl.tw || grp_images <= 0 || B % grp_images) return 0;
   return (grp_images * (H / 2)) % (32 / pl.tw) == 0;
 }
-SST_API int sst_conv_s2_dgrad_pipe_bwdstats_grp(const float* dy, const float* wp, float* dx, float* ws, const float* epi_y,
-                                                const float* epi_scale, const float* epi_shift, const float* epi_slope,
-                                                float epi_slope_const, int epi_act, float* epi_partial, int B, int H, int W, int Cin,
-                                                int Cout, int grp_images, void* stream) {
+namespace {
+int s2d_pipe_launch(const float* dy, const float* wp, float* dx, float* ws, const float* epi_y, const float* epi_scale,
+                    const float* epi_shift, const float* epi_slope, float epi_slope_const, int epi_act, float* epi_partial,
+                    const float* act_y, float act_slope, int B, int H, int W, int Cin, int Cout, int grp_images, void* stream) {
   SST_REQUIRE(dy && wp && dx, "sst_conv_s2_dgrad_pipe: null pointer");
   SST_REQUIRE(grp_images == 0 || grp_images == B || !epi_partial || sst_conv_s2_dgrad_pipe_groups_ok(B, H, W, Cin, Cout, grp_images),
               "sst_conv_s2_dgrad_pipe: coefficient groups of %d images do not end on tile boundaries", grp_images);
@@ -581,19 +605,44 @@
 #endif
   a.gB = (grp_images > 0 && grp_images < B && epi_partial) ? grp_images : 0;
   a.grows = a.gB * a.Ho;
+  a.act_y = act_y; a.act_slope = act_slope;
   const int grid = a.units < 2 * PIPE_CUS ? a.units : 2 * PIPE_CUS;
   hipStream_t st = sst_stream(stream);
-#define SST_S2D_LAUNCH(TW_)                                                                       \
+#define SST_S2D_LAUNCH(TW_, MODE_)                                                                \
   do {                                                                                            \
-    if (a.cb_per > 1) conv_pipe_kernel<1, TW_, 1, true><<<grid, CONV_NT, 0, st>>>(a);             \
-    else conv_pipe_kernel<1, TW_, 1, false><<<grid, CONV_NT, 0, st>>>(a);                         \
+    if (a.cb_per > 1) conv_pipe_kernel<1, TW_, MODE_, true><<<grid, CONV_NT, 0, st>>>(a);         \
+    else conv_pipe_kernel<1, TW_, MODE_, false><<<grid, CONV_NT, 0, st>>>(a);                     \
     SST_LAUNCH_CHECK("conv_pipe_kernel (stride-2 data-gradient)");                                \
     if (pl.ksplit > 1) {                                                                          \
-      pipe_reduce_kernel<TW_, 1><<<a.total_tiles * 4, CONV_NT, 0, st>>>(a);                       \
+      pipe_reduce_kernel<TW_, MODE_><<<a.total_tiles * 4, CONV_NT, 0, st>>>(a);                   \
       SST_LAUNCH_CHECK("pipe_reduce_kernel (stride-2 data-gradient)");                            \
     }                                                                                             \
   } while (0)
-  if (pl.tw == 8) SST_S2D_LAUNCH(8); else if (pl.tw == 4) SST_S2D_LAUNCH(4); else SST_S2D_LAUNCH(2);
+  if (act_y) {
+    if (pl.tw == 8) SST_S2D_LAUNCH(8, 2); else if (pl.tw == 4) SST_S2D_LAUNCH(4, 2); else SST_S2D_LAUNCH(2, 2);
+  } else {
+    if (pl.tw == 8) SST_S2D_LAUNCH(8, 1); else if (pl.tw == 4) SST_S2D_LAUNCH(4, 1); else SST_S2D_LAUNCH(2, 1);
+  }
 #undef SST_S2D_LAUNCH
   return SST_OK;
 }
+}
+
+SST_API int sst_conv_s2_dgrad_pipe_bwdstats_grp(const float* dy, const float* wp, float* dx, float* ws, const float* epi_y,
+                                                const float* epi_scale, const float* epi_shift, const float* epi_slope,
+                                                float epi_slope_const, int epi_act, float* epi_partial, int B, int H, int W, int Cin,
+                                                int Cout, int grp_images, void* stream) {
+  return s2d_pipe_launch(dy, wp, dx, ws, epi_y, epi_scale, epi_shift, epi_slope, epi_slope_const, epi_act, epi_partial, nullptr, 0.f, B, H,
+                         W, Cin, Cout, grp_images, stream);
+}
+
+SST_API int sst_conv_s2_dgrad_pipe_act_supported(int B, int H, int W, int Cin, int Cout) {
+  const char* e = sst_env("SST_D0_FUSE");
+  return (e && atoi(e) < 1) ? 0 : pipe_plan_s2d(B, H, W, Cin, Cout).tw;
+}
+SST_API int sst_conv_s2_dgrad_pipe_act(const float* dy, const float* wp, float* dx, float* ws, const float* act_y, float act_slope, int B,
+                                       int H, int W, int Cin, int Cout, void* stream) {
+  SST_REQUIRE(act_y, "sst_conv_s2_dgrad_pipe_act: null act_y");
+  return s2d_pipe_launch(dy, wp, dx, ws, nullptr, nullptr, nullptr, nullptr, 0.f, 0, nullptr, act_y, act_slope, B, H, W, Cin, Cout, 0,
+                         stream);
+}
diff --git a/srgan-st_amd/csrc/conv_wgrad.hip b/srgan-st_amd/csrc/conv_wgrad.hip
--- a/srgan-st_amd/csrc/conv_wgrad.hip
+++ b/srgan-st_amd/csrc/conv_wgrad.hip
@@ -404,23 +404,28 @@
 constexpr int C3M_ROW = 104;
 constexpr int C3M_WAVE = 3 * C3M_ROW + 96;
 constexpr int C3M_TPW = 4;
-__global__ __launch_bounds__(CONV_NT) void wgrad_k3c3_mfma_kernel(const float* __restrict__ x, const float* __restrict__ dy,
-                                                                  float* __restrict__ slab, int B, int H, int W, int ntiles) {
-  __shared__ float patch[4 * C3M_WAVE];
+template <bool DB>
+__device__ __forceinline__ void k3c3_mfma_body(const float* __restrict__ x, const float* __restrict__ dy, float* __restrict__ slab,
+                                               float* __restrict__ dbslab, int B, int H, int W, int ntiles) {
+  constexpr int WAVE_F = C3M_WAVE + (DB ? 96 : 0);
+  __shared__ float patch[4 * WAVE_F];
   __shared__ float scr[4 * 32 * 33];
   const int tid = threadIdx.x, wave = __builtin_amdgcn_readfirstlane(tid >> 6), lane = tid & 63;
   const int li = lane & 31, lh = lane >> 5;
   constexpr int Cout = 64;
-  float* const ps = patch + wave * C3M_WAVE;
+  float* const ps = patch + wave * WAVE_F;
   const int tpr = W >> 5;
   const int ky = li / 9, kr = li - ky * 9;
-  const float* const bl = ps + (li < 27 ? ky * C3M_ROW + kr + 3 * lh : 3 * C3M_ROW);
+  const float* const bl = ps + (li < 27 ? ky * C3M_ROW + kr + 3 * lh : DB && li == 27 ? 3 * C3M_ROW + 96 : 3 * C3M_ROW);
   f32x16 acc[2];
 #pragma unroll
   for (int h = 0; h < 2; ++h)
 #pragma unroll
     for (int r = 0; r < 16; ++r) acc[h][r] = 0.f;
   for (int i = lane; i < 96; i += 64) ps[3 * C3M_ROW + i] = 0.f;
+  if (DB) {
+    for (int i = lane; i < 96; i += 64) ps[3 * C3M_ROW + 96 + i] = 1.f;
+  }
   float av[2][16][2], xv[2][5];
   auto issue = [&](int it, float (&a_)[16][2], float (&x_)[5]) {
     const int t = (blockIdx.x * C3M_TPW + it) * 4 + wave;
@@ -470,15 +475,40 @@
       const int row = 8 * wave + 4 * lh + j;
       const float v = ((scr[row * 33 + li] + scr[(32 + row) * 33 + li]) + scr[(64 + row) * 33 + li]) + scr[(96 + row) * 33 + li];
       if (li < 27) out[((size_t)(li / 3) * Cout + 32 * h + row) * 3 + li % 3] = v;
-    }
-  }
+      if (DB && li == 27) dbslab[(size_t)blockIdx.x * Cout + 32 * h + row] = v;
+    }
+  }
+}
+__global__ __launch_bounds__(CONV_NT) void wgrad_k3c3_mfma_kernel(const float* __restrict__ x, const float* __restrict__ dy,
+                                                                  float* __restrict__ slab, int B, int H, int W, int ntiles) {
+  k3c3_mfma_body<false>(x, dy, slab, nullptr, B, H, W, ntiles);
+}
+__global__ __launch_bounds__(CONV_NT) void wgrad_k3c3_mfma_db_kernel(const float* __restrict__ x, const float* __restrict__ dy,
+                                                                     float* __restrict__ slab, float* __restrict__ dbslab, int B, int H,
+                                                                     int W, int ntiles) {
+  k3c3_mfma_body<true>(x, dy, slab, dbslab, B, H, W, ntiles);
 }
 constexpr int C3R_OUT = 16, C3R_GRP = 1024 / C3R_OUT;
 __global__ __launch_bounds__(1024) void c3m_reduce_kernel(const float* __restrict__ slab, float* __restrict__ dw, int nchunk,
-                                                          int accumulate) {
+                                                          int accumulate, const float* __restrict__ dbslab, float* __restrict__ db) {
   __shared__ float part[C3R_GRP][C3R_OUT + 1];
   constexpr int TOTAL = 9 * 64 * 3;
   const int o = threadIdx.x & (C3R_OUT - 1), gq = threadIdx.x / C3R_OUT;
+  if (blockIdx.x >= TOTAL / C3R_OUT) {
+    __shared__ double dpart[C3R_GRP][C3R_OUT + 1];
+    const int co = (blockIdx.x - TOTAL / C3R_OUT) * C3R_OUT + o;
+    double td = 0.0;
+    for (int c = gq; c < nchunk; c += C3R_GRP) td += (double)dbslab[(size_t)c * 64 + co];
+    dpart[gq][o] = td;
+    __syncthreads();
+    if (threadIdx.x < C3R_OUT) {
+      td = 0.0;
+      for (int k = 0; k < C3R_GRP; ++k) td += dpart[k][o];
+      const float t = (float)td;
+      db[co] = accumulate ? db[co] + t : t;
+    }
+    return;
+  }
   const int i = blockIdx.x * C3R_OUT + o;
   float t = 0.f;
   int c = gq;
@@ -514,6 +544,10 @@
   }
 }
 inline bool k3c3_mfma_applies(int W, int Cout) { return (W & 31) == 0 && Cout == 64 && !sst_env("SST_WGRAD_NO_K3C3_MFMA"); }
+inline bool k3c3_db_on() {
+  const char* e = sst_env("SST_D0_FUSE");
+  return e && atoi(e) >= 2;
+}
 inline int k3c3_mfma_chunks(int B, int H, int W) { return (B * H * (W >> 5) + 4 * C3M_TPW - 1) / (4 * C3M_TPW); }
 
 inline bool k3c3_applies(int Cin, int ksize, int stride, bool has_in_scale, int in_act) {
@@ -1118,7 +1152,7 @@
     case WgKind::K3C3_MFMA:
       wgrad_k3c3_mfma_kernel<<<pl.nchunk, CONV_NT, 0, st>>>(x, dy, slab, B, H, W, B * H * (W >> 5));
       SST_LAUNCH_CHECK("wgrad_k3c3_mfma_kernel");
-      c3m_reduce_kernel<<<9 * 64 * 3 / C3R_OUT, 1024, 0, st>>>(slab, dw, pl.nchunk, accumulate & 1);
+      c3m_reduce_kernel<<<9 * 64 * 3 / C3R_OUT, 1024, 0, st>>>(slab, dw, pl.nchunk, accumulate & 1, nullptr, nullptr);
       SST_LAUNCH_CHECK("c3m_reduce_kernel");
       return SST_OK;
     case WgKind::K3C3: {
@@ -1134,6 +1168,25 @@
   if (pl.pending == 0 || (accumulate & 4)) return SST_OK;
   launch_wgrad_reduce(slab, dw, pl.nchunk, KK, Cout, Cin, accumulate, nullptr, 1, st);
   SST_LAUNCH_CHECK("wgrad_reduce_kernel");
+  return SST_OK;
+}
+
+SST_API int sst_conv_wgrad_db_supported(int B, int H, int W, int Cin, int Cout, int ksize, int stride) {
+  if (B <= 0 || H <= 0 || W <= 0 || !k3c3_db_on()) return 0;
+  return wgrad_plan(B, H, W, Cin, Cout, ksize, stride, 1, false, ACT_NONE, false).kind == WgKind::K3C3_MFMA;
+}
+SST_API int sst_conv_wgrad_db(const float* x, const float* dy, float* slab, float* dw, float* dbslab, float* db, int B, int H, int W,
+                              int Cin, int Cout, int accumulate, void* stream) {
+  SST_REQUIRE(x && dy && slab && dw && dbslab && db, "sst_conv_wgrad_db: null pointer");
+  SST_REQUIRE(sst_conv_wgrad_db_supported(B, H, W, Cin, Cout, 3, 1), "sst_conv_wgrad_db: shape B=%d H=%d W=%d Cin=%d Cout=%d is not taken", B,
+              H, W, Cin, Cout);
+  SST_REQUIRE((int64_t)B * H * W < (1ll << 31), "sst_conv_wgrad_db: too many pixels");
+  const int nchunk = k3c3_mfma_chunks(B, H, W);
+  hipStream_t st = sst_stream(stream);
+  wgrad_k3c3_mfma_db_kernel<<<nchunk, CONV_NT, 0, st>>>(x, dy, slab, dbslab, B, H, W, B * H * (W >> 5));
+  SST_LAUNCH_CHECK("wgrad_k3c3_mfma_db_kernel");
+  c3m_reduce_kernel<<<9 * 64 * 3 / C3R_OUT + 64 / C3R_OUT, 1024, 0, st>>>(slab, dw, nchunk, accumulate & 1, dbslab, db);
+  SST_LAUNCH_CHECK("c3m_reduce_kernel");
   return SST_OK;
 }
 
diff --git a/srgan-st_amd/srganst/_abi.py b/srgan-st_amd/srganst/_abi.py
--- a/srgan-st_amd/srganst/_abi.py
+++ b/srgan-st_amd/srganst/_abi.py
@@ -56,6 +56,8 @@
     "sst_conv_s2_dgrad_pipe_stat_tiles": (c_int, [c_int, c_int, c_int, c_int, c_int]),
     "sst_conv_s2_dgrad_pipe_groups_ok": (c_int, [c_int, c_int, c_int, c_int, c_int, c_int]),
     "sst_conv_s2_dgrad_pipe_bwdstats_grp": (c_int, [P, P, P, P, P, P, P, P, c_float, c_int, P, c_int, c_int, c_int, c_int, c_int, c_int, P]),
+    "sst_conv_s2_dgrad_pipe_act_supported": (c_int, [c_int, c_int, c_int, c_int, c_int]),
+    "sst_conv_s2_dgrad_pipe_act": (c_int, [P, P, P, P, P, c_float, c_int, c_int, c_int, c_int, c_int, P]),
     "sst_conv_acc_supported": (c_int, [c_int, c_int, c_int, c_int, c_int, c_int, c_int]),
     "sst_conv_fwd_acc": (c_int, [P, P, P, P, P, P, P, P, c_float, c_int, P, P, P, c_float, c_float, c_float, P, P, P, P, P, P, P,
                                  c_int, c_int, c_int, c_int, c_int, c_int, c_int, P]),
@@ -70,6 +72,8 @@
     "sst_conv_wgrad_groups_ok": (c_int, [c_int, c_int, c_int, c_int, c_int, c_int, c_int, c_int]),
     "sst_conv_wgrad_grp": (c_int, [P, P, P, P, P, P, P, c_float, c_int, c_int, c_int, c_int, c_int, c_int,
                                    c_int, c_int, c_int, c_int, P]),
+    "sst_conv_wgrad_db_supported": (c_int, [c_int, c_int, c_int, c_int, c_int, c_int, c_int]),
+    "sst_conv_wgrad_db": (c_int, [P, P, P, P, P, P, c_int, c_int, c_int, c_int, c_int, c_int, P]),
     "sst_conv_wgrad_grouped": (c_int, [P, c_int, c_int, c_int, c_int, c_int, c_int, c_int, c_int, c_int, P]),
     "sst_conv_wgrad_pending_reduce": (c_int, [c_int, c_int, c_int, c_int, c_int, c_int, c_int, c_int, c_int]),
     "sst_wgrad_reduce_multi": (c_int, [P, c_int, P]),
diff --git a/srgan-st_amd/srganst/disc_graph.py b/srgan-st_amd/srganst/disc_graph.py
--- a/srgan-st_amd/srganst/disc_graph.py
+++ b/srgan-st_amd/srganst/disc_graph.py
@@ -220,18 +220,37 @@
     return ops.bwd_finalize_apply(part, g, n=n, **kw) if part is not None else ops.bwd_reduce_apply(g, n=n, **kw)
 
 
+def _first_layer_fused(p, sv):
+    if len(sv.layers) < 2 or sv.layers[0].bi is not None or sv.layers[0].stride != 1 or sv.layers[1].stride != 2:
+        return 0
+    B, H, W, c0 = sv.layers[0].y.shape
+    c1 = p[f"features.{sv.layers[1].ci}.weight"].shape[0]
+    if not ops.conv_s2_dgrad_act_supported(B, H, W, c0, c1):
+        return 0
+    return 2 if ops.conv_wgrad_db_supported(B, H, W, sv.x3.shape[-1], c0, 3, 1) else 1
+
+
 def backward_features(module, p, sv, sink, need_param_grads, need_dx, defer_wgrad=None, defer_below=None):
     wg, acc, g = need_param_grads, sink.acc, sink.g
     groups, gB = sv.groups, sv.gB
     dx = part = None
     reduces = [] if ops.WGRAD_REDUCE_MULTI else None
+    fuse0 = _first_layer_fused(p, sv)
     for li in reversed(range(len(sv.layers))):
         r, below = sv.layers[li], sv.layers[li - 1] if li > 0 else None
         x, in_kw = sv.input_of(li)
         n = r.y.numel() // r.y.shape[-1] // groups
         wname = f"features.{r.ci}.weight"
         cin = p[wname].shape[1]
-        if r.bi is not None:
+        db0 = None
+        if li == 0 and fuse0:
+            dy = g
+            if wg and fuse0 == 2:
+                db0 = sink.take(f"features.{r.ci}.bias")
+            elif wg:
+                ops.bwd_finalize(ops.bwd_reduce(dy, dy, groups=groups), n, dbeta=sink.take(f"features.{r.ci}.bias"), accumulate=acc,
+                                 groups=groups)
+        elif r.bi is not None:
             gam = p[f"features.{r.bi}.weight"]
             dg = sink.take(f"features.{r.bi}.weight") if wg else torch.empty_like(gam)
             db = sink.take(f"features.{r.bi}.bias") if wg else torch.empty_like(gam)
@@ -245,8 +264,8 @@
         if wg:
             dwc = sink.take(wname)
 
-            def launch(x=x, dy=dy, dwc=dwc, stride=r.stride, in_kw=in_kw, red=None):
-                ops.conv_wgrad(x, dy, dwc, 3, stride, **in_kw, accumulate=acc, grp=gB, defer_reduce=red)
+            def launch(x=x, dy=dy, dwc=dwc, stride=r.stride, in_kw=in_kw, red=None, db0=db0):
+                ops.conv_wgrad(x, dy, dwc, 3, stride, **in_kw, accumulate=acc, grp=gB, defer_reduce=red, db=db0)
             if defer_wgrad is not None and (defer_below is None or li < defer_below):
                 ev = torch.cuda.Event()
                 ev.record()
@@ -261,6 +280,8 @@
                 g, part = ops.conv_dgrad_bwdstats(dy, sv.wd[wname], cin, 3, **below.epi("epi_"), grp=gB)
             else:
                 g = ops.conv_fwd(dy, sv.wd[wname], cin, 3, 1)[0]
+        elif li == 1 and fuse0:
+            g = ops.conv_s2_dgrad(dy, sv.ws2[wname], x.shape[1], x.shape[2], cin, act=dict(y=below.y, slope_const=LRELU))
         else:
             epi = below.epi() if below is not None and (below.bi is not None or wg) else None
             out = ops.conv_s2_dgrad(dy, sv.ws2[wname], x.shape[1], x.shape[2], cin, epi=epi, grp=gB)
diff --git a/srgan-st_amd/srganst/ops.py b/srgan-st_amd/srganst/ops.py
--- a/srgan-st_amd/srganst/ops.py
+++ b/srgan-st_amd/srganst/ops.py
@@ -248,14 +248,30 @@
     return mean, rstd, scale, shift
 
 
+D0_FUSE = 2
+
+
+def conv_wgrad_db_supported(B, H, W, cin, cout, ksize=3, stride=1):
+    return D0_FUSE >= 2 and bool(_abi.lib().sst_conv_wgrad_db_supported(B, H, W, cin, cout, ksize, stride))
+
+
 def conv_wgrad(x, dy, dw_out, ksize=3, stride=1, in_scale=None, in_shift=None, in_slope=None, in_slope_const=0.0,
-               in_act=ACT_NONE, accumulate=False, grp=0, defer_reduce=None):
+               in_act=ACT_NONE, accumulate=False, grp=0, defer_reduce=None, db=None):
     B, H, W, cin = x.shape
     cout = dy.shape[-1]
     ho, wo = conv_out_hw(H, W, ksize, stride)
     assert tuple(dy.shape) == (B, ho, wo, cout) and tuple(dw_out.shape) == (cout, cin, ksize, ksize)
     nch = _abi.lib().sst_conv_wgrad_chunks2(B, H, W, cin, cout, ksize, stride, 1)
     slab = _f32(nch * ksize * ksize * cout * cin, like=x)
+    if db is not None:
+        assert tuple(db.shape) == (cout,) and db.is_contiguous()
+        if in_scale is None and in_act == ACT_NONE and conv_wgrad_db_supported(B, H, W, cin, cout, ksize, stride):
+            dbslab = _f32(nch * cout, like=x)
+            args = (ptr(x), ptr(dy), ptr(slab), ptr(dw_out), ptr(dbslab), ptr(db), B, H, W, cin, cout, int(bool(accumulate)))
+            _launch(_abi.lib().sst_conv_wgrad_db, args, "sst_conv_wgrad_db", 2.0 * B * ho * wo * cout * cin * ksize * ksize,
+                    lambda: _wgrad_name(B, H, W, cin, cout, ksize, stride, 1) + "+c3m_reduce_kernel", (x, dy, slab, dw_out, dbslab, db))
+            return dw_out
+        bwd_finalize(bwd_reduce(dy, dy), B * ho * wo, dbeta=db, accumulate=accumulate)
     pend = 0
     if defer_reduce is not None and TRACE is None:
         pend = _abi.lib().sst_conv_wgrad_pending_reduce(B, H, W, cin, cout, ksize, stride, int(in_scale is not None), int(in_act))
@@ -477,8 +493,24 @@
             lambda: f"conv_pipe_kernel<1, {tw}, 1>")
 
 
-def conv_s2_dgrad(dy, wp, H, W, cin, epi=None, grp=0):
+def conv_s2_dgrad_act_supported(B, H, W, cin, cout):
+    return D0_FUSE >= 1 and _pipe_on() and bool(_abi.lib().sst_conv_s2_dgrad_pipe_act_supported(B, H, W, cin, cout))
+
+
+def conv_s2_dgrad(dy, wp, H, W, cin, epi=None, grp=0, act=None):
     B, ho, wo, cout = dy.shape
+    if act is not None:
+        assert epi is None
+        if not conv_s2_dgrad_act_supported(B, H, W, cin, cout):
+            return bwd_apply(conv_s2_dgrad(dy, wp, H, W, cin), y=act["y"], slope_const=act["slope_const"], act=1)
+        assert tuple(act["y"].shape) == (B, H, W, cin) and act["y"].is_contiguous()
+        dx = _f32(B, H, W, cin, like=dy)
+        tw, nws, _, name = _s2_dgrad_route(B, H, W, cin, cout, False, 0)
+        ws = _f32(nws, like=dy) if nws else None
+        _launch(_abi.lib().sst_conv_s2_dgrad_pipe_act,
+                (ptr(dy), ptr(wp), ptr(dx), ptr(ws), ptr(act["y"]), float(act["slope_const"]), B, H, W, cin, cout),
+                "sst_conv_s2_dgrad_pipe_act", 2.0 * B * ho * wo * cout * cin * 9, name, (dy, wp, dx, ws, act["y"]))
+        return dx
     dx = _f32(B, H, W, cin, like=dy)
     L = _abi.lib()
     tw, nws, rows, name = _s2_dgrad_route(B, H, W, cin, cout, epi is not None, grp)
```

Measured after the change: 3286 HR images/s (median of 6 runs). No clear change (+0.9%).
